# hanruihua/NeuPAN

Hardware: AMD Instinct MI355X
Metric: MPC plans/sec (node), diff robot, 1k pts, T=10, K=10; ctrl L2 vs ref (higher is better)
Workload: dtype f32; 1 GPU; BASELINE.json configs[1]: batch=256 synthetic scenes/GPU, diff robot, 1000 pts, T=10, K=10 (iter_threshold=0), M=10, fp32 DUNE (MFMA) + fp64 QP; scenes_per_gpu=256, points=1000, T=10, K=10, M=10, batches_in_flight=40, chains=8, issue_threads=8

## Files before the change

neupan_amd/csrc/c_api.hip:

```cpp
#include "handle.h"

#include <algorithm>
#include <cmath>
#include <cstdlib>
#include <cstring>

extern "C" hipError_t npa_launch_encode(const DevParams& P, const float* wpack, int batch, int scene0, int t0,
                                        int n_stride, const float* cur_s, const float* points, const float* vel,
                                        const int* n_points, const int* flags, unsigned* gkeys, const float* trig,
                                        int n_cu, int blocks_per_cu, int key_terms, hipStream_t stream,
                                        hipEvent_t ev_start, hipEvent_t ev_stop);
extern "C" hipError_t npa_launch_trig(const float* cur_s, int batch, int T, float* trig, hipStream_t stream);
extern "C" hipError_t npa_launch_select_geo(const DevParams& P, const float* wpack, int batch, int scene0, int t0,
                                            int n_stride, const float* cur_s, const float* points, const float* vel,
                                            const int* n_points, const int* flags, const float* trig, float* mu_sorted,
                                            float* lam_sorted, float* pts_sorted, float* dist_sorted, int* count,
                                            unsigned* stats, int debug, unsigned* audit, unsigned audit_thresh,
                                            unsigned audit_seed, float margin_scale, int rows_bf16, hipStream_t stream,
                                            hipEvent_t ev_start, hipEvent_t ev_stop);
#ifdef NPA_EXPERIMENTS
#define NPA_VERSION_SUFFIX " +experiments"
#else
#define NPA_VERSION_SUFFIX ""
#endif
extern "C" hipError_t npa_launch_select(const DevParams& P, const float* wpack, int batch, int scene0, int t0,
                                        int n_stride, const float* cur_s, const float* points, const float* vel,
                                        const int* n_points, const int* flags, const unsigned* gkeys,
                                        const float* trig, float* mu_sorted, float* lam_sorted, float* pts_sorted,
                                        float* dist_sorted, int* count, int key_terms, float e0, unsigned* stats,
                                        int debug, hipStream_t stream, hipEvent_t ev_start, hipEvent_t ev_stop);
extern "C" hipError_t npa_launch_qp(const DevParams& P, int batch, int scene0, const float* cur_s_in,
                                    const float* cur_u_in, const float* ref_s, const float* ref_us, const float* mu_sorted,
                                    const float* lam_sorted, const float* pts_sorted, const float* dist_sorted,
                                    const int* count, float* cur_s_out, float* cur_u_out, float* cur_d_out,
                                    float* out_s, float* out_u, float* out_d, float* out_min_distance,
                                    int* out_iters, float* out_nrmp_points, int* flags, float* state,
                                    double* qp_info, double* warm, float* trig_out, float* dbg_abc, float* dbg_f, double* dbg_x,
                                    hipStream_t stream, hipEvent_t ev_start, hipEvent_t ev_stop, const float* theta);
extern "C" int npa_select_geo_group_supported(int E);
extern "C" hipError_t npa_launch_select_geo_group(const DevParams& P, const SelGeoGroup& G, int n, int batch, int t0, int n_stride_max,
                                                  int debug, unsigned audit_thresh, float margin_scale, int rows_bf16,
                                                  hipStream_t stream, hipEvent_t ev_start, hipEvent_t ev_stop);
extern "C" int npa_qp_group_supported(int T, int M);
extern "C" hipError_t npa_launch_qp_group(const DevParams& P, const QpGroup& G, int n, int batch, hipStream_t stream,
                                          hipEvent_t ev_start, hipEvent_t ev_stop);
extern "C" hipError_t npa_launch_nominal(int batch, int T, int kin, double dt, double L, const double* state,
                                         const float* vel, const double* ref_speed, const double* path,
                                         const int* curve_off, const int* curve_len, const int* point_index,
                                         const double* interval, float* nom_s, float* nom_u, float* ref_s,
                                         float* ref_us, hipStream_t stream);
extern "C" hipError_t npa_launch_scan(int batch, int beam_stride, const double* ranges, const double* beam_vel,
                                      const int* n_beams, const npa_scan_params* params, int mode, int out_stride,
                                      float* points, float* velocities, int* count, hipStream_t stream);
extern "C" int npa_ingest_offsets(int batch, int T, int n_stride, int with_vel, size_t* out, int n);
extern "C" hipError_t npa_launch_ingest_unpack(int batch, int T, int n_stride, int with_vel, const void* record,
                                               size_t record_bytes, float* nom_s, float* nom_u, float* ref_s, float* ref_us,
                                               float* points, float* velocities, int* n_points, int* status,
                                               hipStream_t stream);

extern "C" const char* npa_last_error(void) { return g_err.c_str(); }
extern "C" const char* npa_version(void) { return "neupan_amd 0.5.2 (gfx950, hipcc " NPA_HIPCC_VERSION ")" NPA_VERSION_SUFFIX; }
static int kstride(const npa_handle* h) { return h->key_terms == 4 ? 0 : h->P.key_stride; }

static int check_theta_batch(const npa_handle* h, int batch, const char* who) {
  if (h->theta && batch != h->theta_batch)
    return fail(NPA_E_ARG, std::string(who) + ": batch " + std::to_string(batch) + " differs from the " + std::to_string(h->theta_batch) +
                               " rows registered with npa_set_adjust_batch");
  return NPA_OK;
}

extern "C" size_t npa_workspace_bytes(const npa_handle* h, int batch) {
  if (!h || batch < 1) return 0;
  return npa_scratch_layout(batch, h->P.T, mdim(h->P), h->P.E, kstride(h)).total * sizeof(float);
}
extern "C" size_t npa_workspace_qp_info_offset(const npa_handle* h, int batch) {
  if (!h || batch < 1) return 0;
  return npa_scratch_layout(batch, h->P.T, mdim(h->P), h->P.E, kstride(h)).qp_info * sizeof(float);
}
extern "C" int npa_workspace_layout(const npa_handle* h, int batch, size_t* out, int n) {
  if (!h || batch < 1 || !out || n < 1) return fail(NPA_E_ARG, "npa_workspace_layout: bad argument");
  const ScratchLayout L = npa_scratch_layout(batch, h->P.T, mdim(h->P), h->P.E, kstride(h));
  const size_t v[8] = {L.cur_s * 4, L.cur_u * 4, L.cur_d * 4, L.mu * 4, L.lam * 4, L.pts * 4, L.dist * 4, L.count * 4};
  for (int i = 0; i < n && i < 8; ++i) out[i] = v[i];
  return NPA_OK;
}
extern "C" size_t npa_state_bytes(const npa_handle* h, int batch) {
  if (!h || batch < 1) return 0;
  return (size_t)batch * npa_state_floats(h->P.T, mdim(h->P), h->P.E) * sizeof(float);
}

static EventPair* next_event(npa_handle* h, std::vector<EventPair>& pool, size_t& used) {
  if (!h->prof) return nullptr;
  if (used == pool.size()) {
    if (pool.size() >= 8192) return nullptr;
    EventPair p;
    if (hipEventCreate(&p.a) != hipSuccess || hipEventCreate(&p.b) != hipSuccess) return nullptr;
    pool.push_back(p);
  }
  return &pool[used++];
}

extern "C" int npa_profile_enable(npa_handle* h, int enable) {
  if (!h) return fail(NPA_E_ARG, "null handle");
  h->prof = enable != 0;
  h->n_dune = h->n_sel = h->n_qp = 0;
  return NPA_OK;
}

extern "C" int npa_profile_read(npa_handle* h, double* dune_ms_avg, double* select_ms_avg, double* nrmp_ms_avg,
                                int64_t* launches) {
  if (!h) return fail(NPA_E_ARG, "null handle");
  auto avg = [](std::vector<EventPair>& pool, size_t used, double* out) -> hipError_t {
    double tot = 0;
    for (size_t i = 0; i < used; ++i) {
      hipError_t e = hipEventSynchronize(pool[i].b);
      if (e != hipSuccess) return e;
      float ms = 0;
      e = hipEventElapsedTime(&ms, pool[i].a, pool[i].b);
      if (e != hipSuccess) return e;
      tot += ms;
    }
    if (out) *out = used ? tot / used : 0.0;
    return hipSuccess;
  };
  HIP_TRY(avg(h->ev_dune, h->n_dune, dune_ms_avg));
  HIP_TRY(avg(h->ev_sel, h->n_sel, select_ms_avg));
  HIP_TRY(avg(h->ev_qp, h->n_qp, nrmp_ms_avg));
  if (launches) *launches = (int64_t)h->n_qp;
  h->n_dune = h->n_sel = h->n_qp = 0;
  return NPA_OK;
}

extern "C" int npa_dune_stage(npa_handle* h, int batch, int n_stride, const float* nom_s, const float* points,
                              const float* velocities, const int32_t* n_points, float* mu_sorted, float* lam_sorted,
                              float* pts_sorted, float* dist_sorted, int32_t* count, void* stream) {
  if (!h || batch < 1 || n_stride < 1 || !nom_s || !points || !mu_sorted || !lam_sorted || !pts_sorted ||
      !dist_sorted || !count)
    return fail(NPA_E_ARG, "npa_dune_stage: bad argument");
  if (h->P.M <= 0) return fail(NPA_E_ARG, "npa_dune_stage: planner has no obstacle stage (nrmp_max_num or dune_max_num is 0)");
  {
    int nmax = n_stride < h->P.dune_max_num ? n_stride : h->P.dune_max_num;
    if (nmax > h->P.key_stride) return fail(NPA_E_UNSUPPORTED, "more than 32768 points per scene after decimation");
  }
  const bool geo = h->key_terms == 4;
  const size_t key_bytes = geo ? 0 : (size_t)batch * (h->P.T + 1) * h->P.key_stride * sizeof(unsigned);
  const size_t trig_bytes = ((size_t)batch * (h->P.T + 1) * 2 * sizeof(float) + 63) / 64 * 64;
  const size_t need = key_bytes + trig_bytes + 64;
  if (need > h->stage_cand_bytes) {
    HIP_TRY(hipStreamSynchronize((hipStream_t)stream));
    if (h->stage_cand) HIP_TRY(hipFree(h->stage_cand));
    h->stage_cand = nullptr; h->stage_cand_bytes = 0;
    HIP_TRY(hipMalloc(&h->stage_cand, need));
    h->stage_cand_bytes = need;
  }
  float* trig = reinterpret_cast<float*>(reinterpret_cast<char*>(h->stage_cand) + key_bytes);
  HIP_TRY(npa_launch_trig(nom_s, batch, h->P.T, trig, (hipStream_t)stream));
  if (!geo)
    HIP_TRY(npa_launch_encode(h->P, h->wpack, batch, 0, 0, n_stride, nom_s, points, velocities, n_points, nullptr,
                              (unsigned*)h->stage_cand, trig, h->n_cu, 5, h->key_terms, (hipStream_t)stream,
                              nullptr, nullptr));
  if (geo && !h->select_v1)
    HIP_TRY(npa_launch_select_geo(h->P, h->wpack, batch, 0, 0, n_stride, nom_s, points, velocities, n_points, nullptr, trig,
                                  mu_sorted, lam_sorted, pts_sorted, dist_sorted, count, h->sel_stats_dev, h->sel_debug,
                                  h->rows_bf16 ? nullptr : h->audit_dev, h->audit_thresh, h->launch_seq++, h->margin_scale,
                                  h->rows_bf16 ? 1 : (h->cal.keys_bf16 ? 2 : 0), (hipStream_t)stream, nullptr, nullptr));
  else
    HIP_TRY(npa_launch_select(h->P, h->wpack, batch, 0, 0, n_stride, nom_s, points, velocities, n_points, nullptr,
                              (const unsigned*)h->stage_cand, trig, mu_sorted, lam_sorted, pts_sorted, dist_sorted, count,
                              h->key_terms, h->key_e0, h->sel_stats_dev, h->sel_debug, (hipStream_t)stream, nullptr, nullptr));
  return NPA_OK;
}

extern "C" int npa_nrmp_stage(npa_handle* h, int batch, const float* nom_s, const float* nom_u, const float* ref_s,
                              const float* ref_us, const float* mu_sorted, const float* lam_sorted,
                              const float* pts_sorted, const int32_t* count, float* out_s, float* out_u,
                              float* out_d, double* qp_info, double* x64, void* stream) {
  if (!h || batch < 1 || !nom_s || !nom_u || !ref_s || !ref_us || !out_s || !out_u)
    return fail(NPA_E_ARG, "npa_nrmp_stage: bad argument");
  if (h->P.M > 0 && (!mu_sorted || !lam_sorted || !pts_sorted || !count || !out_d))
    return fail(NPA_E_ARG, "npa_nrmp_stage: obstacle arrays required when nrmp_max_num > 0");
  if (int rc = check_theta_batch(h, batch, "npa_nrmp_stage")) return rc;
  HIP_TRY(npa_launch_qp(h->P, batch, 0, nom_s, nom_u, ref_s, ref_us, mu_sorted, lam_sorted, pts_sorted, nullptr, count,
                        out_s, out_u, out_d, nullptr, nullptr, nullptr, nullptr, nullptr, nullptr, nullptr, nullptr,
                        qp_info, nullptr, nullptr, nullptr, nullptr, x64, (hipStream_t)stream, nullptr, nullptr, h->theta));
  return NPA_OK;
}

extern "C" int npa_nrmp_params(npa_handle* h, int batch, const float* nom_s, const float* nom_u, const float* mu_sorted,
                               const float* lam_sorted, const float* pts_sorted, const int32_t* count, float* out_abc,
                               float* out_f, void* stream) {
  if (!h || batch < 1 || !nom_s || !nom_u || !out_abc) return fail(NPA_E_ARG, "npa_nrmp_params: bad argument");
  if (h->P.M > 0 && (!mu_sorted || !lam_sorted || !pts_sorted || !count || !out_f))
    return fail(NPA_E_ARG, "npa_nrmp_params: obstacle arrays required when nrmp_max_num > 0");
  HIP_TRY(npa_launch_qp(h->P, batch, 0, nom_s, nom_u, nom_s, nom_u, mu_sorted, lam_sorted, pts_sorted, nullptr, count,
                        nullptr, nullptr, nullptr, nullptr, nullptr, nullptr, nullptr, nullptr, nullptr, nullptr, nullptr,
                        nullptr, nullptr, nullptr, out_abc, h->P.M > 0 ? out_f : nullptr, nullptr, (hipStream_t)stream, nullptr, nullptr,
                        nullptr));
  return NPA_OK;
}

extern "C" hipError_t npa_launch_qp_backward(const DevParams& P, int batch, const float* nom_s, const float* nom_u,
                                             const float* ref_s, const float* ref_us, const float* mu_sorted,
                                             const float* lam_sorted, const float* pts_sorted, const int* count,
                                             float* out_s, float* out_u, float* out_d, const float* grad_s,
                                             const float* grad_u, const float* grad_d, float* grad_theta,
                                             float* grad_nom_s, double* qp_info, hipStream_t stream, const float* theta);
extern "C" int npa_nrmp_backward(npa_handle* h, int batch, const float* nom_s, const float* nom_u, const float* ref_s,
                                 const float* ref_us, const float* mu_sorted, const float* lam_sorted,
                                 const float* pts_sorted, const int32_t* count, float* out_s, float* out_u, float* out_d,
                                 const float* grad_s, const float* grad_u, const float* grad_d, float* grad_theta,
                                 float* grad_nom_s, double* qp_info, void* stream) {
  if (!h || batch < 1 || !nom_s || !nom_u || !ref_s || !ref_us || !out_s || !out_u || !grad_s || !grad_u || !grad_theta)
    return fail(NPA_E_ARG, "npa_nrmp_backward: bad argument");
  if (h->P.M > 0 && (!mu_sorted || !lam_sorted || !pts_sorted || !count || !out_d))
    return fail(NPA_E_ARG, "npa_nrmp_backward: obstacle arrays required when nrmp_max_num > 0");
  if (int rc = check_theta_batch(h, batch, "npa_nrmp_backward")) return rc;
  HIP_TRY(npa_launch_qp_backward(h->P, batch, nom_s, nom_u, ref_s, ref_us, mu_sorted, lam_sorted, pts_sorted, count,
                                 out_s, out_u, out_d, grad_s, grad_u, grad_d, grad_theta, grad_nom_s, qp_info, (hipStream_t)stream, h->theta));
  return NPA_OK;
}

__global__ void stage_kernel(float* __restrict__ cur_s, const float* __restrict__ nom_s, size_t ns,
                             float* __restrict__ cur_u, const float* __restrict__ nom_u, size_t nu,
                             int* __restrict__ flags, size_t nflag, int* __restrict__ count, size_t ncount,
                             int* __restrict__ state, size_t nstate, float* __restrict__ trig, int T) {
  const size_t stride = (size_t)gridDim.x * blockDim.x;
  for (size_t i = (size_t)blockIdx.x * blockDim.x + threadIdx.x;; i += stride) {
    bool any = false;
    if (i < ns) { cur_s[i] = nom_s[i]; any = true; }
    if (i < ncount) {
      const size_t b = i / (size_t)(T + 1), t = i - b * (size_t)(T + 1);
      float c, sn;
      npa_trig(nom_s[b * 3 * (size_t)(T + 1) + 2 * (size_t)(T + 1) + t], c, sn);
      trig[2 * i] = c; trig[2 * i + 1] = sn;
    }
    if (i < nu) { cur_u[i] = nom_u[i]; any = true; }
    if (i < nflag) { flags[i] = 0; any = true; }
    if (i < ncount) { count[i] = 0; any = true; }
    if (i < nstate) { state[i] = 0; any = true; }
    if (!any) break;
  }
}

__global__ void stage_group_kernel(StageGroup G, size_t ns, size_t nu, size_t nflag, size_t ncount, size_t nstate, int T) {
  const StageCall& q = G.c[blockIdx.y];
  float* __restrict__ cur_s = q.cur_s; const float* __restrict__ nom_s = q.nom_s; float* __restrict__ cur_u = q.cur_u;
  const float* __restrict__ nom_u = q.nom_u; int* __restrict__ flags = q.flags; int* __restrict__ count = q.count;
  int* __restrict__ state = q.state; float* __restrict__ trig = q.trig;
  const size_t stride = (size_t)gridDim.x * blockDim.x;
  for (size_t i = (size_t)blockIdx.x * blockDim.x + threadIdx.x;; i += stride) {
    bool any = false;
    if (i < ns) { cur_s[i] = nom_s[i]; any = true; }
    if (i < ncount) {
      const size_t b = i / (size_t)(T + 1), t = i - b * (size_t)(T + 1);
      float c, sn;
      npa_trig(nom_s[b * 3 * (size_t)(T + 1) + 2 * (size_t)(T + 1) + t], c, sn);
      trig[2 * i] = c; trig[2 * i + 1] = sn;
    }
    if (i < nu) { cur_u[i] = nom_u[i]; any = true; }
    if (i < nflag) { flags[i] = 0; any = true; }
    if (i < ncount) { count[i] = 0; any = true; }
    if (i < nstate) { state[i] = 0; any = true; }
    if (!any) break;
  }
}

static void key_policy(npa_handle* h, int batch, int n_stride) {
  if (!h->cal.key_auto) return;
  const DevParams& P = h->P;
  const unsigned now = *(volatile unsigned*)h->sel_stats_host;
  if (h->key_terms == 3) {
    if (--h->hold > 0) return;
    h->key_terms = 1; h->key_err = h->cal.err_mode[0]; h->key_e0 = h->cal.e0_mode[0];
    h->stats_mark = now; h->tiles_window = 0; h->calls_window = 0;
  } else if (h->calls_window >= 8) {
    const unsigned redone = now - h->stats_mark;
    if ((unsigned long long)redone * 12ull > h->tiles_window) {
      h->key_terms = 3; h->key_err = h->cal.err_mode[1]; h->key_e0 = h->cal.e0_mode[1]; h->hold = 256;
      return;
    }
    h->stats_mark = now; h->tiles_window = 0; h->calls_window = 0;
  }
  const int n_use = n_stride < P.dune_max_num ? n_stride : P.dune_max_num;
  h->tiles_window += (unsigned long long)batch * ((n_use + 31) / 32) * ((P.T + 1) + (size_t)(P.K - 1) * P.T);
  ++h->calls_window;
}

static int forward_begin_impl(npa_handle* h, int batch, int n_stride, const float* nom_s, const float* nom_u,
                              const float* ref_s, const float* ref_us, const float* points,
                              const float* velocities, const int32_t* n_points, float* out_s, float* out_u,
                              float* out_d, float* out_min_distance, int32_t* out_iters, float* out_nrmp_points,
                              void* workspace, size_t workspace_bytes, void* state, size_t state_bytes,
                              void* stream_, int flags, bool launch_stage) {
  if (!h || batch < 1 || !nom_s || !nom_u || !ref_s || !ref_us || !out_s || !out_u || !workspace || !state)
    return fail(NPA_E_ARG, "npa_forward_begin: null argument");
  const DevParams& P = h->P;
  if (P.M > 0 && !out_d) return fail(NPA_E_ARG, "npa_forward_begin: out_d required when nrmp_max_num > 0");
  if (workspace_bytes < npa_workspace_bytes(h, batch)) return fail(NPA_E_ARG, "workspace too small");
  if (state_bytes < npa_state_bytes(h, batch)) return fail(NPA_E_ARG, "state buffer too small");
  if (points && n_stride < 1) return fail(NPA_E_ARG, "n_stride < 1");
  if (points && (n_stride < P.dune_max_num ? n_stride : P.dune_max_num) > P.key_stride)
    return fail(NPA_E_UNSUPPORTED, "more than 32768 points per scene after decimation");
  std::lock_guard<std::mutex> lock(h->mu);
  PendingCall* pc = &h->pc;
  if (pc->active) return fail(NPA_E_ARG, "npa_forward_begin: previous forward on this handle not ended");
  if (int rc = check_theta_batch(h, batch, "npa_forward_begin")) return rc;
  hipStream_t stream = (hipStream_t)stream_;
  const int T = P.T;
  const bool reset_state = (flags & NPA_FWD_RESET_STATE) != 0;
  const ScratchLayout L = npa_scratch_layout(batch, T, mdim(P), P.E, kstride(h));
  float* ws = (float*)workspace;
  pc->batch = batch; pc->n_stride = n_stride; pc->ref_s = ref_s; pc->ref_us = ref_us; pc->points = points;
  pc->velocities = velocities; pc->n_points = n_points; pc->out_s = out_s; pc->out_u = out_u; pc->out_d = out_d;
  pc->out_md = out_min_distance; pc->out_iters = out_iters; pc->out_np = out_nrmp_points; pc->ws = ws;
  pc->state = (float*)state; pc->stream = stream;
  pc->dune = P.M > 0 && points != nullptr;
  pc->nom_s = nom_s; pc->nom_u = nom_u; pc->reset_state = reset_state;
  pc->theta = h->theta;
  if (pc->dune) key_policy(h, batch, n_stride);
  if (launch_stage) {
    const size_t ns = (size_t)batch * 3 * (T + 1), nu2 = (size_t)batch * 2 * T;
    const size_t nflag = (size_t)batch * 4, ncount = (size_t)batch * (T + 1);
    const size_t nstate = reset_state ? npa_state_bytes(h, batch) / 4 : 0;
    const size_t work = std::max(std::max(ns, nu2), std::max(std::max(nflag, ncount), nstate));
    const int threads = 256;
    const int blocks = (int)std::min<size_t>((work + threads - 1) / threads, 512);
    hipLaunchKernelGGL(stage_kernel, dim3(blocks), dim3(threads), 0, stream, ws + L.cur_s, nom_s, ns, ws + L.cur_u, nom_u, nu2,
                       (int*)(ws + L.flags), nflag, (int*)(ws + L.count), ncount, (int*)state, nstate, ws + L.trig, T);
    HIP_TRY(hipGetLastError());
  }
  pc->active = true;
  return NPA_OK;
}

extern "C" int npa_forward_begin(npa_handle* h, int batch, int n_stride, const float* nom_s, const float* nom_u,
                                 const float* ref_s, const float* ref_us, const float* points,
                                 const float* velocities, const int32_t* n_points, float* out_s, float* out_u,
                                 float* out_d, float* out_min_distance, int32_t* out_iters, float* out_nrmp_points,
                                 void* workspace, size_t workspace_bytes, void* state, size_t state_bytes,
                                 void* stream_, int flags) {
  return forward_begin_impl(h, batch, n_stride, nom_s, nom_u, ref_s, ref_us, points, velocities, n_points, out_s, out_u, out_d,
                            out_min_distance, out_iters, out_nrmp_points, workspace, workspace_bytes, state, state_bytes, stream_,
                            flags, true);
}

extern "C" int npa_group_mergeable(int n, const npa_forward_call* calls) {
  if (n < 2 || n > NPA_GROUP_MAX || !calls) return 0;
  static const bool off = getenv("NPA_GROUP_MERGE") != nullptr && atoi(getenv("NPA_GROUP_MERGE")) == 0;
  if (off) return 0;
  const npa_handle* h0 = calls[0].h;
  if (!h0) return 0;
  const DevParams& P = h0->P;
  const bool dune0 = P.M > 0 && calls[0].points != nullptr;
  if (dune0 && !(h0->key_terms == 4 && !h0->select_v1 && !h0->rows_bf16 && npa_select_geo_group_supported(P.E))) return 0;
  if (!npa_qp_group_supported(P.T, P.M) || h0->qp_generic || h0->cal.key_auto) return 0;
  if (calls[0].iter_num < 1 || calls[0].iter_num > P.K) return 0;
  for (int c = 0; c < n; ++c) {
    const npa_handle* h = calls[c].h;
    if (!h || calls[c].stream != calls[0].stream || calls[c].batch != calls[0].batch || calls[c].iter_num != calls[0].iter_num ||
        h->device != h0->device || memcmp(&h->P, &P, sizeof(DevParams)) != 0 || h->key_terms != h0->key_terms ||
        h->select_v1 != h0->select_v1 || h->rows_bf16 != h0->rows_bf16 || h->cal.keys_bf16 != h0->cal.keys_bf16 ||
        h->sel_debug != h0->sel_debug || h->audit_thresh != h0->audit_thresh || h->margin_scale != h0->margin_scale ||
        h->qp_generic != h0->qp_generic || h->qp_warm != h0->qp_warm || h->cal.key_auto ||
        (P.M > 0 && calls[c].points != nullptr) != dune0 || (calls[c].out_d == nullptr) != (calls[0].out_d == nullptr))
      return 0;
  }
  return 1;
}

extern "C" int npa_forward_group_merged(int n, const npa_forward_call* calls) { return npa_group_mergeable(n, calls); }

struct GroupLock {
  std::mutex* m[NPA_GROUP_MAX];
  int n = 0;
  GroupLock(int cnt, const npa_forward_call* calls) {
    for (int c = 0; c < cnt && n < NPA_GROUP_MAX; ++c)
      if (calls[c].h) m[n++] = &calls[c].h->mu;
    std::sort(m, m + n);
    n = (int)(std::unique(m, m + n) - m);
    for (int i = 0; i < n; ++i) m[i]->lock();
  }
  ~GroupLock() { for (int i = n - 1; i >= 0; --i) m[i]->unlock(); }
  GroupLock(const GroupLock&) = delete;
  GroupLock& operator=(const GroupLock&) = delete;
};

extern "C" int npa_group_begin_merged(int n, const npa_forward_call* calls, int flags, int* begun) {
  *begun = 0;
  for (int c = 0; c < n; ++c) {
    const npa_forward_call& a = calls[c];
    const int rc = forward_begin_impl(a.h, a.batch, a.n_stride, a.nom_s, a.nom_u, a.ref_s, a.ref_us, a.points, a.velocities,
                                      a.n_points, a.out_s, a.out_u, a.out_d, a.out_min_distance, a.out_iters, a.out_nrmp_points,
                                      a.workspace, a.workspace_bytes, a.state, a.state_bytes, a.stream, flags, false);
    if (rc != NPA_OK) return rc;
    *begun = c + 1;
  }
  GroupLock group_lock(n, calls);
  npa_handle* h0 = calls[0].h;
  const DevParams& P = h0->P;
  const int T = P.T, batch = calls[0].batch;
  const ScratchLayout L = npa_scratch_layout(batch, T, mdim(P), P.E, kstride(h0));
  StageGroup G;
  memset(&G, 0, sizeof(G));
  for (int c = 0; c < n; ++c) {
    const PendingCall& pc = calls[c].h->pc;
    G.c[c] = StageCall{pc.ws + L.cur_s, pc.nom_s, pc.ws + L.cur_u, pc.nom_u, (int*)(pc.ws + L.flags), (int*)(pc.ws + L.count),
                       (int*)pc.state, pc.ws + L.trig};
  }
  const size_t ns = (size_t)batch * 3 * (T + 1), nu2 = (size_t)batch * 2 * T;
  const size_t nflag = (size_t)batch * 4, ncount = (size_t)batch * (T + 1);
  const size_t nstate = h0->pc.reset_state ? npa_state_bytes(h0, batch) / 4 : 0;
  const size_t work = std::max(std::max(ns, nu2), std::max(std::max(nflag, ncount), nstate));
  const int threads = 256;
  const int blocks = (int)std::min<size_t>((work + threads - 1) / threads, 512);
  hipLaunchKernelGGL(stage_group_kernel, dim3(blocks, n), dim3(threads), 0, h0->pc.stream, G, ns, nu2, nflag, ncount, nstate, T);
  HIP_TRY(hipGetLastError());
  return NPA_OK;
}

static std::atomic<unsigned long long> g_merged_launches{0};
extern "C" unsigned long long npa_dbg_group_merged_launches(void) { return g_merged_launches.load(); }

extern "C" int npa_group_iter_merged(int n, const npa_forward_call* calls, int k) {
  GroupLock group_lock(n, calls);
  npa_handle* h0 = calls[0].h;
  const DevParams& P = h0->P;
  if (k < 0 || k >= P.K) return fail(NPA_E_ARG, "npa_forward_batch_group: iteration index out of range");
  const int T = P.T, batch = calls[0].batch;
  const ScratchLayout L = npa_scratch_layout(batch, T, mdim(P), P.E, kstride(h0));
  hipStream_t stream = h0->pc.stream;
  for (int c = 0; c < n; ++c)
    if (!calls[c].h->pc.active) return fail(NPA_E_ARG, "npa_forward_batch_group: a call of the group is not in progress");
  if (h0->pc.dune) {
    SelGeoGroup G;
    memset(&G, 0, sizeof(G));
    int n_stride_max = 1;
    for (int c = 0; c < n; ++c) {
      npa_handle* h = calls[c].h;
      const PendingCall& pc = h->pc;
      float* ws = pc.ws;
      G.c[c] = SelGeoCall{h->wpack, ws + L.cur_s, pc.points, pc.velocities, pc.n_points, (const int*)(ws + L.flags),
                          ws + L.mu, ws + L.lam, ws + L.pts, ws + L.dist, (int*)(ws + L.count), h->sel_stats_dev, ws + L.trig,
                          h->rows_bf16 ? nullptr : h->audit_dev, pc.n_stride, h->launch_seq++};
      if (pc.n_stride > n_stride_max) n_stride_max = pc.n_stride;
    }
    EventPair* evs = next_event(h0, h0->ev_sel, h0->n_sel);
    HIP_TRY(npa_launch_select_geo_group(P, G, n, batch, k == 0 ? 0 : 1, n_stride_max, 0, h0->audit_thresh,
                                        h0->margin_scale, h0->cal.keys_bf16 ? 2 : 0, stream, evs ? evs->a : nullptr,
                                        evs ? evs->b : nullptr));
  }
  QpGroup Q;
  memset(&Q, 0, sizeof(Q));
  for (int c = 0; c < n; ++c) {
    npa_handle* h = calls[c].h;
    const PendingCall& pc = h->pc;
    float* ws = pc.ws;
    float *cur_s = ws + L.cur_s, *cur_u = ws + L.cur_u;
    Q.c[c] = QpCall{cur_s, cur_u, pc.ref_s, pc.ref_us, ws + L.mu, ws + L.lam, ws + L.pts, ws + L.dist, (const int*)(ws + L.count),
                    cur_s, cur_u, ws + L.cur_d, pc.out_s, pc.out_u, pc.out_d, pc.out_md, pc.out_iters, pc.out_np,
                    (int*)(ws + L.flags), pc.state, (double*)(ws + L.qp_info), h->qp_warm ? (double*)(ws + L.warm) : nullptr,
                    pc.dune ? ws + L.trig : nullptr, pc.theta};
  }
  EventPair* ev = next_event(h0, h0->ev_qp, h0->n_qp);
  HIP_TRY(npa_launch_qp_group(P, Q, n, batch, stream, ev ? ev->a : nullptr, ev ? ev->b : nullptr));
  g_merged_launches.fetch_add(1);
  return NPA_OK;
}

extern "C" int npa_forward_iter(npa_handle* h, int k) {
  if (!h) return fail(NPA_E_ARG, "npa_forward_iter: null handle");
  std::lock_guard<std::mutex> lock(h->mu);
  PendingCall* pc = &h->pc;
  if (!pc->active) return fail(NPA_E_ARG, "npa_forward_iter: no forward in progress on this handle");
  const DevParams& P = h->P;
  if (k < 0 || k >= P.K) return fail(NPA_E_ARG, "npa_forward_iter: iteration index out of range");
  const int T = P.T, batch = pc->batch;
  const bool geo = h->key_terms == 4;
  const ScratchLayout L = npa_scratch_layout(batch, T, mdim(P), P.E, kstride(h));
  float* ws = pc->ws;
  float *cur_s = ws + L.cur_s, *cur_u = ws + L.cur_u, *cur_d = ws + L.cur_d;
  float *mu = ws + L.mu, *lam = ws + L.lam, *pts = ws + L.pts, *dist = ws + L.dist;
  int* count = (int*)(ws + L.count);
  int* flags = (int*)(ws + L.flags);
  double* qp_info = (double*)(ws + L.qp_info);
  unsigned* gkeys = (unsigned*)(ws + L.keys);
  hipStream_t stream = pc->stream;
  if (pc->dune) {
    const int t0 = k == 0 ? 0 : 1;
    if (!geo) {
      EventPair* ev = next_event(h, h->ev_dune, h->n_dune);
      HIP_TRY(npa_launch_encode(P, h->wpack, batch, 0, t0, pc->n_stride, cur_s, pc->points, pc->velocities,
                                pc->n_points, flags, gkeys, ws + L.trig, h->n_cu, 5, h->key_terms, stream,
                                ev ? ev->a : nullptr, ev ? ev->b : nullptr));
    }
    EventPair* evs = next_event(h, h->ev_sel, h->n_sel);
    if (geo && !h->select_v1)
      HIP_TRY(npa_launch_select_geo(P, h->wpack, batch, 0, t0, pc->n_stride, cur_s, pc->points, pc->velocities, pc->n_points,
                                    flags, ws + L.trig, mu, lam, pts, dist, count, h->sel_stats_dev, 0,
                                    h->rows_bf16 ? nullptr : h->audit_dev, h->audit_thresh, h->launch_seq++, h->margin_scale,
                                    h->rows_bf16 ? 1 : (h->cal.keys_bf16 ? 2 : 0), stream, evs ? evs->a : nullptr, evs ? evs->b : nullptr));
    else
      HIP_TRY(npa_launch_select(P, h->wpack, batch, 0, t0, pc->n_stride, cur_s, pc->points, pc->velocities,
                                pc->n_points, flags, gkeys, ws + L.trig, mu, lam, pts, dist, count, h->key_terms, h->key_e0,
                                h->sel_stats_dev, 0, stream, evs ? evs->a : nullptr, evs ? evs->b : nullptr));
  }
  EventPair* ev = next_event(h, h->ev_qp, h->n_qp);
  HIP_TRY(npa_launch_qp(P, batch, 0, cur_s, cur_u, pc->ref_s, pc->ref_us, mu, lam, pts, dist, count, cur_s, cur_u,
                        cur_d, pc->out_s, pc->out_u, pc->out_d, pc->out_md, pc->out_iters, pc->out_np, flags,
                        pc->state, qp_info, h->qp_warm ? (double*)(ws + L.warm) : nullptr, pc->dune ? ws + L.trig : nullptr,
                        nullptr, nullptr, nullptr, stream,
                        ev ? ev->a : nullptr, ev ? ev->b : nullptr, pc->theta));
  if (h->cal.key_auto && pc->dune && k == P.K - 1)
    HIP_TRY(hipMemcpyAsync(h->sel_stats_host, h->sel_stats_dev, sizeof(unsigned), hipMemcpyDeviceToHost, stream));
  return NPA_OK;
}

extern "C" int npa_forward_end(npa_handle* h) {
  if (!h) return fail(NPA_E_ARG, "npa_forward_end: null handle");
  std::lock_guard<std::mutex> lock(h->mu);
  PendingCall* pc = &h->pc;
  if (!pc->active) return fail(NPA_E_ARG, "npa_forward_end: no forward in progress on this handle");
  pc->active = false;
  return NPA_OK;
}

extern "C" int npa_dbg_select_stats(npa_handle* h, unsigned out[4]) {
  if (!h || !out || !h->sel_stats_dev) return NPA_E_ARG;
  HIP_TRY(hipDeviceSynchronize());
  HIP_TRY(hipMemcpy(out, h->sel_stats_dev, 4 * sizeof(unsigned), hipMemcpyDeviceToHost));
  return NPA_OK;
}

extern "C" int npa_forward_batch_flags(npa_handle* h, int batch, int n_stride, const float* nom_s, const float* nom_u,
                                       const float* ref_s, const float* ref_us, const float* points,
                                       const float* velocities, const int32_t* n_points, float* out_s, float* out_u,
                                       float* out_d, float* out_min_distance, int32_t* out_iters, float* out_nrmp_points,
                                       void* workspace, size_t workspace_bytes, void* state, size_t state_bytes,
                                       void* stream_, int flags) {
  if (!h) return fail(NPA_E_ARG, "npa_forward_batch: null handle");
  int rc = npa_forward_begin(h, batch, n_stride, nom_s, nom_u, ref_s, ref_us, points, velocities, n_points, out_s,
                             out_u, out_d, out_min_distance, out_iters, out_nrmp_points, workspace, workspace_bytes,
                             state, state_bytes, stream_, flags);
  if (rc != NPA_OK) return rc;
  for (int k = 0; k < h->P.K; ++k) {
    rc = npa_forward_iter(h, k);
    if (rc != NPA_OK) { npa_forward_end(h); return rc; }
  }
  return npa_forward_end(h);
}

extern "C" int npa_forward_batch(npa_handle* h, int batch, int n_stride, const float* nom_s, const float* nom_u,
                                 const float* ref_s, const float* ref_us, const float* points,
                                 const float* velocities, const int32_t* n_points, float* out_s, float* out_u,
                                 float* out_d, float* out_min_distance, int32_t* out_iters, float* out_nrmp_points,
                                 void* workspace, size_t workspace_bytes, void* state, size_t state_bytes,
                                 void* stream_) {
  return npa_forward_batch_flags(h, batch, n_stride, nom_s, nom_u, ref_s, ref_us, points, velocities, n_points, out_s, out_u,
                                 out_d, out_min_distance, out_iters, out_nrmp_points, workspace, workspace_bytes, state,
                                 state_bytes, stream_, 0);
}

extern "C" int npa_nominal_ref_states(int batch, int receding, int kinematics, double step_time, double wheelbase,
                                      const double* state, const float* cur_vel, const double* ref_speed,
                                      const double* path, const int32_t* curve_off, const int32_t* curve_len,
                                      const int32_t* point_index, const double* interval, float* nom_s, float* nom_u,
                                      float* ref_s, float* ref_us, void* stream) {
  if (batch < 1 || !state || !ref_speed || !path || !curve_off || !curve_len || !point_index || !interval || !nom_s ||
      !nom_u || !ref_s || !ref_us)
    return fail(NPA_E_ARG, "npa_nominal_ref_states: bad argument");
  if (receding < 1 || receding > NPA_MAX_T) return fail(NPA_E_UNSUPPORTED, "receding outside [1,NPA_MAX_T]");
  if (kinematics < 0 || kinematics > 2) return fail(NPA_E_ARG, "unknown kinematics");
  if (kinematics == NPA_KIN_ACKER && !(wheelbase > 0)) return fail(NPA_E_ARG, "acker needs wheelbase > 0");
  HIP_TRY(npa_launch_nominal(batch, receding, kinematics, step_time, wheelbase, state, cur_vel, ref_speed, path,
                             curve_off, curve_len, point_index, interval, nom_s, nom_u, ref_s, ref_us,
                             (hipStream_t)stream));
  return NPA_OK;
}

extern "C" hipError_t npa_launch_progress(int batch, const double* state, const double* path, const int* curve_off,
                                          const int* curve_len, int* point_index, double close_threshold, int ind_range,
                                          double arrive_threshold, int arrive_index_threshold, float* min_dis,
                                          int* arrived, hipStream_t stream);
extern "C" int npa_path_progress(int batch, const double* state, const double* path, const int32_t* curve_off,
                                 const int32_t* curve_len, int32_t* point_index, double close_threshold, int ind_range,
                                 double arrive_threshold, int arrive_index_threshold, float* min_dis, int32_t* arrived,
                                 void* stream) {
  if (batch < 1 || !state || !path || !curve_off || !curve_len || !point_index || !arrived || ind_range < 1)
    return fail(NPA_E_ARG, "npa_path_progress: bad argument");
  HIP_TRY(npa_launch_progress(batch, state, path, curve_off, curve_len, point_index, close_threshold, ind_range,
                              arrive_threshold, arrive_index_threshold, min_dis, arrived, (hipStream_t)stream));
  return NPA_OK;
}

extern "C" int npa_scan_to_points(int batch, int beam_stride, const double* ranges, const double* beam_vel,
                                  const int32_t* n_beams, const npa_scan_params* params, int mode, int out_stride,
                                  float* points, float* velocities, int32_t* count, void* stream) {
  if (batch < 1 || beam_stride < 1 || out_stride < 1 || !ranges || !params || !points || !count)
    return fail(NPA_E_ARG, "npa_scan_to_points: bad argument");
  if (mode != 0 && mode != 1) return fail(NPA_E_ARG, "npa_scan_to_points: mode must be 0 or 1");
  HIP_TRY(npa_launch_scan(batch, beam_stride, ranges, beam_vel, n_beams, params, mode, out_stride, points, velocities,
                          count, (hipStream_t)stream));
  return NPA_OK;
}

extern "C" hipError_t npa_launch_cycle_switch(int batch, int loop, const double* state, const int* curve_arrived,
                                              const int* curve_off, const int* curve_len, const int* robot_first,
                                              int* curve_index, int* cur_off, int* cur_len, int* point_index, int* arrived,
                                              npa_scan_params* params_a, npa_scan_params* params_b, hipStream_t stream);
extern "C" hipError_t npa_launch_cycle_act(int batch, int T, int kin, int first_cycle, int cycle, const float* opt_u,
                                           const float* min_distance, float threshold, const int* arrived, const int* collided,
                                           const float* override_row, const int* n_points, float* cur_vel, float* action,
                                           uint8_t* stop, int* frozen, float* log_actions, uint8_t* log_stop,
                                           float* log_controls, int* log_n_points, hipStream_t stream);
extern "C" hipError_t npa_launch_cycle_commit(int batch, int cycle, const double* state, const double* clearance, int* collided,
                                              double* log_states, double* log_clearance, hipStream_t stream);

extern "C" int npa_cycle_progress(int batch, const double* state, const double* path, const int32_t* curve_off,
                                  const int32_t* curve_len, const int32_t* robot_first, int loop, double close_threshold,
                                  int ind_range, double arrive_threshold, int arrive_index_threshold, int32_t* curve_index,
                                  int32_t* cur_off, int32_t* cur_len, int32_t* point_index, int32_t* curve_arrived,
                                  int32_t* arrived, npa_scan_params* params_a, npa_scan_params* params_b, void* stream) {
  if (batch < 1 || !state || !path || !curve_off || !curve_len || !robot_first || !curve_index || !cur_off || !cur_len ||
      !point_index || !curve_arrived || !arrived || !params_a || !params_b || ind_range < 1)
    return fail(NPA_E_ARG, "npa_cycle_progress: bad argument");
  HIP_TRY(npa_launch_progress(batch, state, path, cur_off, cur_len, point_index, close_threshold, ind_range, arrive_threshold,
                              arrive_index_threshold, nullptr, curve_arrived, (hipStream_t)stream));
  HIP_TRY(npa_launch_cycle_switch(batch, loop, state, curve_arrived, curve_off, curve_len, robot_first, curve_index, cur_off,
                                  cur_len, point_index, arrived, params_a, params_b, (hipStream_t)stream));
  return NPA_OK;
}

extern "C" int npa_cycle_act(int batch, int receding, int kinematics, int first_cycle, int cycle, const float* opt_u,
                             const float* min_distance, float collision_threshold, const int32_t* arrived,
                             const int32_t* collided, const float* override_row, const int32_t* n_points, float* cur_vel,
                             float* action, uint8_t* stop, int32_t* frozen, float* log_actions, uint8_t* log_stop,
                             float* log_controls, int32_t* log_n_points, void* stream) {
  if (batch < 1 || cycle < 0 || !opt_u || !min_distance || !arrived || !collided || !cur_vel || !action || !stop || !frozen)
    return fail(NPA_E_ARG, "npa_cycle_act: bad argument");
  if (receding < 1 || receding > NPA_MAX_T) return fail(NPA_E_ARG, "npa_cycle_act: receding outside [1,NPA_MAX_T]");
  if (kinematics < 0 || kinematics > 2) return fail(NPA_E_ARG, "npa_cycle_act: unknown kinematics");
  HIP_TRY(npa_launch_cycle_act(batch, receding, kinematics, first_cycle, cycle, opt_u, min_distance, collision_threshold, arrived,
                               collided, override_row, n_points, cur_vel, action, stop, frozen, log_actions, log_stop,
                               log_controls, log_n_points, (hipStream_t)stream));
  return NPA_OK;
}

extern "C" int npa_cycle_commit(int batch, int cycle, const double* state, const double* clearance, int32_t* collided,
                                double* log_states, double* log_clearance, void* stream) {
  if (batch < 1 || cycle < 0 || !state || !clearance || !collided) return fail(NPA_E_ARG, "npa_cycle_commit: bad argument");
  HIP_TRY(npa_launch_cycle_commit(batch, cycle, state, clearance, collided, log_states, log_clearance, (hipStream_t)stream));
  return NPA_OK;
}

extern "C" hipError_t npa_launch_cycle_retask(int batch, int T, int cycle, int style, double min_radius, const double* state,
                                              int* arrived, const int* collided, double* path, const int* curve_off,
                                              int* curve_len, const int* robot_first, const int* row_capacity,
                                              const double* goals, int g_stride, const int* n_goals, int* goal_index,
                                              const double* interval, int* curve_index, int* cur_off, int* cur_len,
                                              int* point_index, float* cur_vel, int* status, int* log_goal, hipStream_t stream);

extern "C" int npa_cycle_retask(int batch, int receding, int cycle, int style, double min_radius, const double* state,
                                int32_t* arrived, const int32_t* collided, double* path, const int32_t* curve_off,
                                int32_t* curve_len, const int32_t* robot_first, const int32_t* row_capacity, const double* goals,
                                int g_stride, const int32_t* n_goals, int32_t* goal_index, const double* interval,
                                int32_t* curve_index, int32_t* cur_off, int32_t* cur_len, int32_t* point_index, float* cur_vel,
                                int32_t* retask_status, int32_t* log_goal, void* stream) {
  const char* what = nullptr;
  if (batch < 1 || cycle < 0 || !state || !arrived || !collided || !path || !curve_off || !curve_len || !robot_first ||
      !row_capacity || !goals || !n_goals || !goal_index || !interval || !curve_index || !cur_off || !cur_len || !point_index ||
      !cur_vel || !retask_status)
    what = "npa_cycle_retask: bad argument";
  else if (receding < 1 || receding > NPA_MAX_T) what = "npa_cycle_retask: receding outside [1,NPA_MAX_T]";
  else if (style != NPA_CURVE_LINE && style != NPA_CURVE_DUBINS) what = "npa_cycle_retask: style outside 0..1";
  else if (style == NPA_CURVE_DUBINS && (!(min_radius > 0.0) || !std::isfinite(min_radius)))
    what = "npa_cycle_retask: dubins needs min_radius > 0";
  else if (g_stride < 1) what = "npa_cycle_retask: g_stride < 1";
  if (what) return fail(NPA_E_ARG, what);
  HIP_TRY(npa_launch_cycle_retask(batch, receding, cycle, style, min_radius, state, arrived, collided, path, curve_off, curve_len,
                                  robot_first, row_capacity, goals, g_stride, n_goals, goal_index, interval, curve_index, cur_off,
                                  cur_len, point_index, cur_vel, retask_status, log_goal, (hipStream_t)stream));
  return NPA_OK;
}

static int ingest_args_ok(int batch, int receding, int n_stride) {
  return batch >= 1 && receding >= 1 && receding <= NPA_MAX_T && n_stride >= 1;
}

extern "C" int npa_ingest_layout(int batch, int receding, int n_stride, int with_velocities, size_t* out, int n) {
  if (!ingest_args_ok(batch, receding, n_stride) || !out || n < 1 || n > 8)
    return fail(NPA_E_ARG, "npa_ingest_layout: bad argument");
  if (npa_ingest_offsets(batch, receding, n_stride, with_velocities != 0, out, n) != 0)
    return fail(NPA_E_ARG, "npa_ingest_layout: the cloud section would not fit int32 word offsets");
  return NPA_OK;
}

extern "C" int npa_ingest_unpack(int batch, int receding, int n_stride, int with_velocities, const void* record,
                                 size_t record_bytes, float* nom_s, float* nom_u, float* ref_s, float* ref_us, float* points,
                                 float* velocities, int32_t* n_points, int32_t* status, void* stream) {
  if (!ingest_args_ok(batch, receding, n_stride) || !record || !nom_s || !nom_u || !ref_s || !ref_us || !points ||
      !n_points || !status || (with_velocities && !velocities))
    return fail(NPA_E_ARG, "npa_ingest_unpack: bad argument");
  const void* ptrs[] = {record, nom_s, nom_u, ref_s, ref_us, points, velocities, n_points, status};
  for (const void* p : ptrs)
    if (((uintptr_t)p & 3) != 0) return fail(NPA_E_ARG, "npa_ingest_unpack: pointers must be 4-byte aligned");
  size_t off[8];
  if (npa_ingest_offsets(batch, receding, n_stride, with_velocities != 0, off, 8) != 0)
    return fail(NPA_E_ARG, "npa_ingest_unpack: the cloud section would not fit int32 word offsets");
  if (record_bytes < off[6] || record_bytes > off[7] || (record_bytes & 3) != 0)
    return fail(NPA_E_ARG, "npa_ingest_unpack: record_bytes must be a multiple of 4 between the cloud section's offset (" +
                               std::to_string(off[6]) + ") and the layout's total (" + std::to_string(off[7]) + "), got " +
                               std::to_string(record_bytes));
  HIP_TRY(npa_launch_ingest_unpack(batch, receding, n_stride, with_velocities != 0, record, record_bytes, nom_s, nom_u, ref_s,
                                   ref_us, points, velocities, n_points, status, (hipStream_t)stream));
  return NPA_OK;
}

extern "C" hipError_t npa_launch_clearance(const DevParams& P, int batch, int n_stride, const float* traj, const float* points,
                                           const float* velocities, const int* n_points, float threshold, float* clearance,
                                           int* nearest, float* min_clearance, int* first_violation, hipStream_t stream);
extern "C" int npa_plan_clearance(npa_handle* h, int batch, int n_stride, const float* traj_s, const float* points,
                                  const float* velocities, const int32_t* n_points, float threshold, float* clearance,
                                  int32_t* nearest, float* min_clearance, int32_t* first_violation, void* stream) {
  if (!h || batch <= 0 || n_stride <= 0 || !traj_s || !points || !clearance || !nearest)
    return fail(NPA_E_ARG, "npa_plan_clearance: bad argument");
  const void* ptrs[] = {traj_s, points, velocities, n_points, clearance, nearest, min_clearance, first_violation};
  for (const void* p : ptrs)
    if (((uintptr_t)p & 3) != 0) return fail(NPA_E_ARG, "npa_plan_clearance: pointers must be 4-byte aligned");
  if (!h->geo_valid)
    return fail(NPA_E_UNSUPPORTED, "npa_plan_clearance: the robot polygon's rows are not consecutive counter-clockwise edges "
                                   "(no vertices could be derived from G, h)");
  HIP_TRY(npa_launch_clearance(h->P, batch, n_stride, traj_s, points, velocities, n_points, threshold, clearance, nearest,
                               min_clearance, first_violation, (hipStream_t)stream));
  return NPA_OK;
}

extern "C" hipError_t npa_launch_labels(int E, const double* G, const double* h, long long n, const double* points,
                                        float* mu, float* dist, hipStream_t stream);
extern "C" int npa_dune_labels(int edge_num, const double* G, const double* h, int64_t n, const double* points,
                               float* mu, float* dist, void* stream) {
  if (!G || !h || n < 0 || (n > 0 && (!points || !mu || !dist))) return fail(NPA_E_ARG, "npa_dune_labels: bad argument");
  if (edge_num < 3 || edge_num > NPA_MAX_E) return fail(NPA_E_UNSUPPORTED, "edge_num outside [3,NPA_MAX_E]");
  HIP_TRY(npa_launch_labels(edge_num, G, h, (long long)n, points, mu, dist, (hipStream_t)stream));
  return NPA_OK;
}
```

neupan_amd/csrc/create.hip:

```cpp
#include "handle.h"
#include "pack_image.h"

#include <algorithm>
#include <cmath>
#include <cstdio>
#include <cstdlib>
#include <cstring>
#include <map>

extern "C" hipError_t npa_launch_key_calib(const DevParams& P, const float* wpack, int key_terms, int nside, float half,
                                           unsigned* out, hipStream_t stream);
extern "C" hipError_t npa_launch_geo_table(const DevParams& P, float* wpack, float* nodes, int n_cu, hipStream_t stream);
extern "C" hipError_t npa_launch_ktab_calib(const DevParams& P, const float* wpack, int nside, float half, float inner, float cx, float cy,
                                            unsigned* out, int n_cu, hipStream_t stream);
extern "C" hipError_t npa_launch_geo_calib(const DevParams& P, const float* wpack, int nside, float half, float inner,
                                           float shift, unsigned* out, int n_cu, hipStream_t stream);
extern "C" hipError_t npa_launch_k16_calib(const DevParams& P, const float* wpack, int nside, float half, float inner, unsigned* out,
                                           int n_cu, hipStream_t stream);
extern "C" size_t npa_qp_shmem_bytes(int T, int M);

static std::mutex g_pack_mu;
static std::map<std::string, std::weak_ptr<SharedPack>> g_packs;
static long long g_pack_calibrations = 0, g_pack_hits = 0;

struct CalibKnobDef { const char* name; void (*parse)(const char* v, CalibKnobs& k); };
static Precision parse_precision(const char* v) {
  return !strcmp(v, "bf16") ? Precision::bf16 : (!strcmp(v, "fp32") ? Precision::fp32 : Precision::invalid);
}
static const CalibKnobDef kCalibKnobs[] = {
    {"NPA_DUNE_FP32KEYS", [](const char*, CalibKnobs& k) { k.forced_mode = 0; }},
    {"NPA_KEY_TERMS", [](const char* v, CalibKnobs& k) { const int t = atoi(v); if (k.forced_mode != 0 && (t == 1 || t == 3 || t == 4)) k.forced_mode = t; }},
    {"NPA_KEY_SAFETY", [](const char* v, CalibKnobs& k) { const double s = atof(v); if (s >= 1.0 && s <= 1e3) k.key_safety = s; }},
    {"NPA_GEO_GRID", [](const char* v, CalibKnobs& k) { const int n = atoi(v); if (n >= 64 && n <= 8192) k.geo_grid = n / 8 * 8; }},
    {"NPA_GEO_NOCHECK", [](const char*, CalibKnobs& k) { k.geo_nocheck = true; }},
    {"NPA_GEO_TABLE", [](const char* v, CalibKnobs& k) { k.geo_table = atoi(v) != 0; }},
    {"NPA_KTAB_SAFETY", [](const char* v, CalibKnobs& k) { const double s = atof(v); if (s >= 1.0 && s <= 100.0) k.ktab_safety = s; }},
    {"NPA_KEYS_PRECISION", [](const char* v, CalibKnobs& k) { k.keys_precision = parse_precision(v); }},
    {"NPA_K16_SAFETY", [](const char* v, CalibKnobs& k) { const double s = atof(v); if (s >= 1.0 && s <= 100.0) k.k16_safety = s; }},
    {"NPA_ROWS_PRECISION", [](const char* v, CalibKnobs& k) { k.rows_precision = parse_precision(v); }},
};

struct Knobs {
  CalibKnobs calib;
  std::string calib_key;
  bool sel_debug = false, qp_cold = false, qp_generic = false, skip_selftest = false, pack_cache = true;
  double audit_rate = 1.0 / 64.0;
  float margin_scale = 1.f;
};

static Knobs read_knobs() {
  Knobs k;
  for (const CalibKnobDef& d : kCalibKnobs) {
    const char* v = getenv(d.name);
    k.calib_key.push_back('|');
    if (v) { k.calib_key.append(v); d.parse(v, k.calib); } else k.calib_key.push_back('\x01');
  }
  k.sel_debug = getenv("NPA_SEL_DEBUG") != nullptr;
  k.qp_cold = getenv("NPA_QP_COLD") != nullptr;
  k.qp_generic = getenv("NPA_QP_GENERIC") != nullptr;
  k.skip_selftest = getenv("NPA_SKIP_SELFTEST") != nullptr;
  if (const char* env = getenv("NPA_PACK_CACHE")) k.pack_cache = atoi(env) != 0;
  if (const char* env = getenv("NPA_AUDIT_RATE")) { double v = atof(env); if (v >= 0.0 && v <= 1.0) k.audit_rate = v; }
  if (const char* env = getenv("NPA_GEO_MARGIN_SCALE")) { double v = atof(env); if (v > 0.0 && v <= 100.0) k.margin_scale = (float)v; }
  return k;
}

#ifdef NPA_EXPERIMENTS
static void read_experiment_knobs(npa_handle* h) { h->select_v1 = getenv("NPA_SELECT_V1") != nullptr; }
#endif


template <class T>
struct DevScratch {
  T* p = nullptr;
  hipError_t alloc_zeroed(size_t n) {
    hipError_t e = hipMalloc(&p, n * sizeof(T));
    return e == hipSuccess ? hipMemset(p, 0, n * sizeof(T)) : e;
  }
  ~DevScratch() { if (p) (void)hipFree(p); }
};

static void set_calibrated(DevParams& P, const Calibration& c) { P.geo_rcal = c.geo_rcal; P.geo_far = c.geo_far; P.geo_tab = c.geo_tab; }

static void use_key_mode(npa_handle* h) { h->key_terms = h->cal.key_terms; h->key_err = h->cal.key_err; h->key_e0 = h->cal.key_e0; }
static void apply_calibration(npa_handle* h, const Calibration& c) {
  h->cal = c;
  set_calibrated(h->P, c);
  use_key_mode(h);
}

static constexpr int kBandsPadded = (NPA_GEO_BANDS + 3) & ~3;
static const float kCalibHalves[3] = {8.f, 32.f, 128.f};

static void band_margins(const float* raw, const bool* seen, double safety, float floor, float* margin, float* near) {
  for (int bnd = 0; bnd < NPA_GEO_BANDS; ++bnd) {
    float m = -1.f;
    for (int q = std::max(bnd - 1, 0); q <= std::min(bnd + 1, NPA_GEO_BANDS - 1); ++q)
      if (seen[q]) m = std::max(m, raw[q]);
    near[bnd] = m;
    margin[bnd] = (m < 0.f || !(m < 1e30f)) ? INFINITY : std::max((float)(safety * m), floor);
  }
}

static void residual_margins(const unsigned* bits, double safety, float floor, float (&margin)[kBandsPadded], float& worst_err,
                             float& worst_margin) {
  float raw[NPA_GEO_BANDS], near[NPA_GEO_BANDS];
  bool seen[NPA_GEO_BANDS];
  for (int bnd = 0; bnd < NPA_GEO_BANDS; ++bnd) { memcpy(&raw[bnd], &bits[bnd], 4); seen[bnd] = bits[bnd] != 0u; }
  for (int bnd = 0; bnd < kBandsPadded; ++bnd) margin[bnd] = INFINITY;
  band_margins(raw, seen, safety, floor, margin, near);
  worst_err = 0.f; worst_margin = 0.f;
  for (int bnd = 0; bnd <= npa_geo_band(8.0f) && bnd < NPA_GEO_BANDS; ++bnd)
    if (near[bnd] >= 0.f) { worst_err = std::max(worst_err, near[bnd]); worst_margin = std::max(worst_margin, margin[bnd]); }
}

static hipError_t calibrate_network_keys(const DevParams& P, const float* wpack, const CalibKnobs& k, int forced, Calibration& c) {
  const int modes[2] = {1, 3};
  const float floor_e0[2] = {1e-4f, 2e-5f}, cap_e0[2] = {5e-2f, 1e-3f};
  bool ok[2] = {false, false};
  const double sf = k.key_safety > 0 ? k.key_safety : 5.0;
  DevScratch<unsigned> dmax;
  hipError_t e = hipMalloc(&dmax.p, sizeof(unsigned));
  for (int m = 0; m < 2 && e == hipSuccess; ++m) {
    if (forced > 0 && forced != modes[m]) continue;
    unsigned bits = 0;
    e = hipMemset(dmax.p, 0, sizeof(unsigned));
    if (e == hipSuccess) e = npa_launch_key_calib(P, wpack, modes[m], 1024, 25.0f, dmax.p, nullptr);
    if (e == hipSuccess) e = hipMemcpy(&bits, dmax.p, sizeof(unsigned), hipMemcpyDeviceToHost);
    if (e != hipSuccess) break;
    float err;
    memcpy(&err, &bits, sizeof(err));
    c.err_mode[m] = err;
    c.e0_mode[m] = std::max((float)(sf * err), floor_e0[m]);
    ok[m] = c.e0_mode[m] <= cap_e0[m] || forced == modes[m];
  }
  if (e != hipSuccess) return e;
  const int pick = ok[0] ? 0 : (ok[1] ? 1 : -1);
  c.key_terms = 0; c.key_err = 0.f; c.key_e0 = 0.f;
  if (pick >= 0) { c.key_terms = modes[pick]; c.key_err = c.err_mode[pick]; c.key_e0 = c.e0_mode[pick]; }
  c.key_auto = forced < 0 && ok[0] && ok[1];
  return hipSuccess;
}

static hipError_t calibrate_geo_keys(const DevParams& P0, float* wpack, int n_cu, const CalibKnobs& k, Calibration& c) {
  DevParams P = P0;
  set_calibrated(P, c);
  const float* halves = kCalibHalves;
  const int nside = k.geo_grid;
  const int forced = k.forced_mode;
  unsigned bits[2 * NPA_GEO_BANDS], bits2[2 * NPA_GEO_BANDS];
  {
    DevScratch<unsigned> tab, tab2;
    hipError_t e = tab.alloc_zeroed(2 * NPA_GEO_BANDS);
    for (int gI = 0; gI < 3 && e == hipSuccess; ++gI)
      e = npa_launch_geo_calib(P, wpack, nside, halves[gI], gI == 0 ? 0.f : 0.97f * halves[gI - 1], 0.f, tab.p, n_cu, nullptr);
    if (e == hipSuccess) e = tab2.alloc_zeroed(2 * NPA_GEO_BANDS);
    for (int gI = 0; gI < 3 && e == hipSuccess; ++gI)
      e = npa_launch_geo_calib(P, wpack, nside, halves[gI], gI == 0 ? 0.f : 0.97f * halves[gI - 1], 0.5f, tab2.p, n_cu, nullptr);
    if (e == hipSuccess) e = hipMemcpy(bits, tab.p, sizeof(bits), hipMemcpyDeviceToHost);
    if (e == hipSuccess) e = hipMemcpy(bits2, tab2.p, sizeof(bits2), hipMemcpyDeviceToHost);
    if (e != hipSuccess) return e;
  }
  const double sf = k.key_safety > 0 ? k.key_safety : 1.5;
  float raw[NPA_GEO_BANDS], mg[NPA_GEO_BANDS], near[NPA_GEO_BANDS];
  bool seen[NPA_GEO_BANDS];
  float refine = 0.f, slope = 0.f;
  {
    float pred[NPA_GEO_BANDS], cen[NPA_GEO_BANDS];
    for (int bnd = 0; bnd < NPA_GEO_BANDS; ++bnd) {
      float f0, f1, c0;
      memcpy(&f0, &bits[bnd], 4); memcpy(&f1, &bits[NPA_GEO_BANDS + bnd], 4); memcpy(&c0, &bits2[bnd], 4);
      pred[bnd] = f0 + f1; cen[bnd] = c0;
    }
    for (int bnd = 0; bnd < NPA_GEO_BANDS; ++bnd) {
      if (bits2[bnd] == 0u) continue;
      float pr = 0.f;
      for (int q = std::max(bnd - 1, 0); q <= std::min(bnd + 1, NPA_GEO_BANDS - 1); ++q) pr = std::max(pr, pred[q]);
      pr = std::max(pr, 1e-3f);
      if (!(cen[bnd] < 1e30f)) { refine = INFINITY; continue; }
      refine = std::max(refine, cen[bnd] / pr);
    }
    const float h0 = 2.0f * halves[0] / (float)(nside - 1);
    for (int bnd = 0; bnd <= npa_geo_band(6.0f); ++bnd) {
      float f1;
      memcpy(&f1, &bits[NPA_GEO_BANDS + bnd], 4);
      if (f1 < 1e30f) slope = std::max(slope, f1 / h0);
    }
  }
  c.geo_refine = refine; c.geo_slope = slope;
  for (int bnd = 0; bnd < NPA_GEO_BANDS; ++bnd) {
    float f0, f1, c0, c1;
    memcpy(&f0, &bits[bnd], 4); memcpy(&f1, &bits[NPA_GEO_BANDS + bnd], 4);
    memcpy(&c0, &bits2[bnd], 4); memcpy(&c1, &bits2[NPA_GEO_BANDS + bnd], 4);
    seen[bnd] = bits[bnd] != 0u || bits[NPA_GEO_BANDS + bnd] != 0u || bits2[bnd] != 0u;
    raw[bnd] = std::max(f0, c0) + std::max(f1, c1);
  }
  band_margins(raw, seen, sf, 1e-4f, mg, near);
  float worst_err = 0.f, worst_margin = 0.f;
  for (int bnd = npa_geo_band(0.25f); bnd <= npa_geo_band(8.0f) && bnd < NPA_GEO_BANDS; ++bnd) {
    worst_margin = std::max(worst_margin, mg[bnd]);
    float f0;
    memcpy(&f0, &bits[bnd], 4);
    worst_err = std::max(worst_err, f0);
  }
  c.geo_err = worst_err; c.geo_margin = worst_margin;
  const bool resolved = refine <= 1.25f || k.geo_nocheck;
  if (!((worst_margin <= 0.15f && resolved) || forced == 4)) return hipSuccess;
  hipError_t e = hipMemcpy(wpack + WP_GEO, mg, sizeof(mg), hipMemcpyHostToDevice);
  c.geo_rcal = halves[2];
  double rmax = 0;
  for (int v = 0; v < P.E; ++v) rmax = std::max(rmax, std::sqrt((double)P.pvx[v] * P.pvx[v] + (double)P.pvy[v] * P.pvy[v]));
  c.geo_far = (float)std::max(1.0, (double)halves[2] - rmax);
  c.key_terms = 4; c.key_err = worst_err; c.key_e0 = worst_margin;
  return e;
}

static hipError_t calibrate_key_table(const DevParams& P0, float* wpack, int n_cu, const float* tabh, const CalibKnobs& k, Calibration& c) {
  DevParams P = P0;
  set_calibrated(P, c);
  unsigned kb[NPA_GEO_BANDS];
  {
    DevScratch<float> nodes;
    DevScratch<unsigned> tabk;
    hipError_t e = hipMalloc(&nodes.p, (size_t)NPA_TAB_LEVELS * (NPA_TAB_N + 1) * (NPA_TAB_N + 1) * sizeof(float));
    if (e == hipSuccess) e = npa_launch_geo_table(P, wpack, nodes.p, n_cu, nullptr);
    if (e == hipSuccess) e = tabk.alloc_zeroed(NPA_GEO_BANDS);
    const float th0 = tabh[2];
    const float khalves[NPA_TAB_LEVELS] = {th0, 4.f * th0, 16.f * th0, 64.f * th0};
    for (int gI = 0; gI < NPA_TAB_LEVELS && e == hipSuccess; ++gI)
      e = npa_launch_ktab_calib(P, wpack, k.geo_grid, khalves[gI], gI == 0 ? 0.f : 0.97f * khalves[gI - 1], tabh[0], tabh[1], tabk.p,
                                n_cu, nullptr);
    if (e == hipSuccess) e = hipMemcpy(kb, tabk.p, sizeof(kb), hipMemcpyDeviceToHost);
    if (e != hipSuccess) return e;
  }
  float mk[kBandsPadded];
  residual_margins(kb, k.ktab_safety, 1e-4f, mk, c.ktab_err, c.ktab_margin);
  const hipError_t e = hipMemcpy(wpack + WP_KTAB, mk, sizeof(mk), hipMemcpyHostToDevice);
  if (e == hipSuccess) c.geo_tab = 1;
  return e;
}

static hipError_t calibrate_bf16_keys(const DevParams& P0, float* wpack, int n_cu, const CalibKnobs& k, Calibration& c) {
  DevParams P = P0;
  set_calibrated(P, c);
  const float* halves = kCalibHalves;
  unsigned bits[NPA_GEO_BANDS];
  {
    DevScratch<unsigned> tab;
    hipError_t e = tab.alloc_zeroed(NPA_GEO_BANDS);
    for (int gI = 0; gI < 3 && e == hipSuccess; ++gI)
      e = npa_launch_k16_calib(P, wpack, 1024, halves[gI], gI == 0 ? 0.f : 0.97f * halves[gI - 1], tab.p, n_cu, nullptr);
    if (e == hipSuccess) e = hipMemcpy(bits, tab.p, sizeof(bits), hipMemcpyDeviceToHost);
    if (e != hipSuccess) return e;
  }
  float mg[kBandsPadded];
  residual_margins(bits, k.k16_safety, 1e-5f, mg, c.k16_err, c.k16_margin);
  const hipError_t e = hipMemcpy(wpack + WP_K16, mg, sizeof(mg), hipMemcpyHostToDevice);
  c.keys_bf16 = true;
  return e;
}

static hipError_t calibrate_key_mode(const DevParams& P, float* wpack, int n_cu, bool geo_valid, const float* tabh, const CalibKnobs& k,
                                     Calibration& c) {
  const int forced = k.forced_mode;
  hipError_t e = hipSuccess;
  if (geo_valid && (forced < 0 || forced == 4)) {
    e = calibrate_geo_keys(P, wpack, n_cu, k, c);
    if (e == hipSuccess && c.key_terms == 4 && (P.E == 4 || P.E == 8) && k.geo_table) e = calibrate_key_table(P, wpack, n_cu, tabh, k, c);
  }
  if (e == hipSuccess && c.key_terms != 4 && forced != 0 && forced != 4) e = calibrate_network_keys(P, wpack, k, forced, c);
  return e;
}

static int check_precision_tiers(npa_handle* h, const CalibKnobs& k, int key_terms) {
  const bool geo48 = key_terms == 4 && !h->select_v1 && (h->P.E == 4 || h->P.E == 8);
  if (k.rows_precision == Precision::invalid) return fail(NPA_E_ARG, "NPA_ROWS_PRECISION must be fp32 or bf16");
  if (k.rows_precision == Precision::bf16) {
    if (!geo48) return fail(NPA_E_UNSUPPORTED, "NPA_ROWS_PRECISION=bf16 needs geometric keys (select_geo_kernel) and a polygon of 4 or 8 edges");
    h->rows_bf16 = true;
  }
  if (k.keys_precision == Precision::invalid) return fail(NPA_E_ARG, "NPA_KEYS_PRECISION must be fp32 or bf16");
  if (k.keys_precision == Precision::bf16 && !(geo48 && !h->rows_bf16))
    return fail(NPA_E_UNSUPPORTED, "NPA_KEYS_PRECISION=bf16 needs geometric keys, exact rows and a polygon of 4 or 8 edges");
  return NPA_OK;
}

static int hip_status(hipError_t e) { return e == hipSuccess ? NPA_OK : fail(NPA_E_HIP, std::string("npa_create: ") + hipGetErrorString(e)); }

static int acquire_pack(npa_handle* h, const std::vector<float>& image, bool need_w, const Knobs& knobs) {
  const DevParams& P = h->P;
  const CalibKnobs& ck = knobs.calib;
  std::string key(reinterpret_cast<const char*>(image.data()), image.size() * sizeof(float));
  key.append(reinterpret_cast<const char*>(&P.E), sizeof(P.E));
  key.append(reinterpret_cast<const char*>(P.G), sizeof(P.G));
  key.append(reinterpret_cast<const char*>(P.h), sizeof(P.h));
  key.append(reinterpret_cast<const char*>(&h->device), sizeof(h->device));
  key.push_back(need_w ? 'w' : '-');
  key.append(knobs.calib_key);
  std::lock_guard<std::mutex> lock(g_pack_mu);
  if (knobs.pack_cache) {
    auto it = g_packs.find(key);
    if (it != g_packs.end()) {
      h->pack = it->second.lock();
      if (!h->pack) g_packs.erase(it);
    }
  }
  const bool hit = (bool)h->pack;
  if (!hit) {
    h->pack = std::make_shared<SharedPack>();
    h->pack->device = h->device;
    hipError_t e = hipMalloc(&h->pack->wpack, ((size_t)WP_TAB + WP_TAB_FLOATS) * sizeof(float));
    if (e == hipSuccess) e = hipMemcpy(h->pack->wpack, image.data(), WP_TOTAL * sizeof(float), hipMemcpyHostToDevice);
    if (e != hipSuccess) return hip_status(e);
  }
  SharedPack& S = *h->pack;
  h->wpack = S.wpack;
  if (need_w) {
    if (hit) ++g_pack_hits;
    else if (int rc = hip_status(calibrate_key_mode(P, S.wpack, h->n_cu, h->geo_valid, &image[WP_TABH], ck, S.cal))) return rc;
    if (int rc = check_precision_tiers(h, ck, S.cal.key_terms)) return rc;
    if (!hit && ck.keys_precision == Precision::bf16)
      if (int rc = hip_status(calibrate_bf16_keys(P, S.wpack, h->n_cu, ck, S.cal))) return rc;
    apply_calibration(h, S.cal);
  }
  if (!hit) {
    if (need_w) ++g_pack_calibrations;
    if (knobs.pack_cache) g_packs[key] = h->pack;
  }
  return NPA_OK;
}

static int params_from_config(const npa_config* cfg, const npa_dune_weights* w, DevParams& P, bool& need_w, bool& geo_valid) {
  if (cfg->receding < 1 || cfg->receding > NPA_MAX_T) return fail(NPA_E_UNSUPPORTED, "receding outside [1,NPA_MAX_T]");
  if (cfg->nrmp_max_num < 0 || cfg->nrmp_max_num > NPA_MAX_M) return fail(NPA_E_UNSUPPORTED, "nrmp_max_num outside [0,NPA_MAX_M]");
  if (cfg->edge_num < 3 || cfg->edge_num > NPA_MAX_E) return fail(NPA_E_UNSUPPORTED, "edge_num outside [3,NPA_MAX_E]");
  if (cfg->kinematics < 0 || cfg->kinematics > 2) return fail(NPA_E_ARG, "unknown kinematics");
  if (cfg->iter_num < 1) return fail(NPA_E_ARG, "iter_num < 1");
  if (npa_qp_shmem_bytes(cfg->receding, cfg->nrmp_max_num) > 160 * 1024) return fail(NPA_E_UNSUPPORTED, "T*M too large for LDS");
  need_w = cfg->nrmp_max_num > 0 && cfg->dune_max_num > 0;
  if (need_w && !w) return fail(NPA_E_ARG, "DUNE weights required unless nrmp_max_num == 0 or dune_max_num == 0");
  P.T = cfg->receding; P.M = (cfg->dune_max_num > 0) ? cfg->nrmp_max_num : 0; P.E = cfg->edge_num;
  P.kin = cfg->kinematics; P.K = cfg->iter_num; P.dune_max_num = cfg->dune_max_num;
  {
    long long n = cfg->dune_max_num > 0 ? cfg->dune_max_num : 1;
    if (n > NPA_MAX_POINTS) n = NPA_MAX_POINTS;
    P.key_stride = (int)((n + 31) / 32 * 32);
  }
  P.iter_threshold = cfg->iter_threshold;
  P.dt = cfg->step_time; P.dt32 = (float)cfg->step_time; P.L = cfg->wheelbase;
  for (int k = 0; k < 2; ++k) { P.speed_bound[k] = cfg->speed_bound[k]; P.acce_bound[k] = cfg->acce_bound[k]; }
  P.ro_obs = cfg->ro_obs; P.bk = cfg->bk;
  for (int k = 0; k < 3; ++k) P.q_s[k] = cfg->q_s[k];
  P.p_u = cfg->p_u; P.eta = cfg->eta; P.d_max = cfg->d_max; P.d_min = cfg->d_min;
  for (int e = 0; e < NPA_MAX_E; ++e) { P.G[e][0] = cfg->G[e][0]; P.G[e][1] = cfg->G[e][1]; P.h[e] = cfg->h[e]; }
  geo_valid = npa_polygon_geometry(P);
  return NPA_OK;
}

extern "C" int npa_dbg_pack_image(const npa_config* cfg, const npa_dune_weights* w, float* image, size_t image_floats, void* params,
                                  size_t params_bytes, size_t* params_size, int* geo_valid, size_t* offsets, int n_offsets) {
  if (!cfg) return fail(NPA_E_ARG, "npa_dbg_pack_image: null configuration");
  const size_t off[13] = {WP_W1, WP_WL, WP_VEC, WP_W6, WP_B6, WP_BF, WP_WLS, WP_WB16, WP_TABH, WP_W116, WP_WL16, WP_VEC16, WP_TOTAL};
  for (int i = 0; offsets && i < n_offsets && i < 13; ++i) offsets[i] = off[i];
  if (params_size) *params_size = sizeof(DevParams);
  DevParams P;
  memset(&P, 0, sizeof(P));
  bool need_w = false, valid = false;
  if (int rc = params_from_config(cfg, w, P, need_w, valid)) return rc;
  if (geo_valid) *geo_valid = valid ? 1 : 0;
  if (params) memcpy(params, &P, std::min(params_bytes, sizeof(P)));
  if (image) {
    std::vector<float> img;
    npa_build_pack_image(P, valid, need_w ? w : nullptr, img);
    memcpy(image, img.data(), std::min(image_floats, img.size()) * sizeof(float));
  }
  return NPA_OK;
}

static hipError_t audit_block_reset(npa_handle* h) {
  if (!h->audit_dev) return hipSuccess;
  unsigned blk[8] = {0, 0, 0, 0, 0, 0, 0, 0};
  void* mirror = nullptr;
  if (h->audit_host && hipHostGetDevicePointer(&mirror, h->audit_host, 0) != hipSuccess) mirror = nullptr;
  memcpy(&blk[6], &mirror, sizeof(mirror));
  if (h->audit_host) *(volatile unsigned*)h->audit_host = 0;
  return hipMemcpy(h->audit_dev, blk, sizeof(blk), hipMemcpyHostToDevice);
}

static hipError_t alloc_handle_buffers(npa_handle* h) {
  hipError_t e = hipMalloc(&h->sel_stats_dev, 4 * sizeof(unsigned));
  if (e == hipSuccess) e = hipMemset(h->sel_stats_dev, 0, 4 * sizeof(unsigned));
  if (e == hipSuccess) e = hipHostMalloc(&h->sel_stats_host, sizeof(unsigned), hipHostMallocDefault);
  if (e == hipSuccess) *h->sel_stats_host = 0;
  if (e == hipSuccess) e = hipMalloc(&h->audit_dev, 8 * sizeof(unsigned));
  if (e == hipSuccess) e = hipHostMalloc(&h->audit_host, sizeof(unsigned), hipHostMallocMapped);
  if (e == hipSuccess) e = audit_block_reset(h);
  return e;
}

static int npa_self_test(npa_handle* h);

static int create_handle(npa_handle* h, bool need_w, const npa_dune_weights* w) {
  std::vector<float> image;
  npa_build_pack_image(h->P, h->geo_valid, need_w ? w : nullptr, image);
  const Knobs knobs = read_knobs();
  h->knobs = knobs.calib;
  h->sel_debug = knobs.sel_debug; h->qp_warm = !knobs.qp_cold; h->qp_generic = knobs.qp_generic;
#ifdef NPA_EXPERIMENTS
  read_experiment_knobs(h);
#endif
  if (int rc = hip_status(hipGetDevice(&h->device))) return rc;
  hipDeviceProp_t prop;
  if (hipGetDeviceProperties(&prop, h->device) == hipSuccess && prop.multiProcessorCount > 0) h->n_cu = prop.multiProcessorCount;
  if (int rc = acquire_pack(h, image, need_w, knobs)) return rc;
  if (need_w) {
    if (int rc = hip_status(alloc_handle_buffers(h))) return rc;
    h->audit_thresh = knobs.audit_rate >= 1.0 ? 0xFFFFFFFFu : (unsigned)(knobs.audit_rate * 4294967296.0);
    h->margin_scale = knobs.margin_scale;
  }
  return knobs.skip_selftest ? NPA_OK : npa_self_test(h);
}

extern "C" int npa_create(const npa_config* cfg, const npa_dune_weights* w, npa_handle** out) {
  if (!cfg || !out) return fail(NPA_E_ARG, "npa_create: null argument");
  DevParams P;
  memset(&P, 0, sizeof(P));
  bool need_w = false, geo_valid = false;
  if (int rc = params_from_config(cfg, w, P, need_w, geo_valid)) return rc;
  npa_handle* h = new npa_handle();
  memcpy(&h->P, &P, sizeof(P));
  h->geo_valid = geo_valid;
  const int rc = create_handle(h, need_w, w);
  if (rc != NPA_OK) {
    const std::string msg = g_err;
    npa_destroy(h);
    return fail(rc, msg);
  }
  *out = h;
  return NPA_OK;
}

extern "C" int npa_destroy(npa_handle* h) {
  if (!h) return NPA_OK;
  {
    int cur = -1;
    if (hipGetDevice(&cur) == hipSuccess) {
      if (cur != h->device) (void)hipSetDevice(h->device);
      (void)hipDeviceSynchronize();
      if (cur != h->device) (void)hipSetDevice(cur);
    }
    (void)hipGetLastError();
  }
  for (auto& p : h->ev_dune) { hipEventDestroy(p.a); hipEventDestroy(p.b); }
  for (auto& p : h->ev_sel) { hipEventDestroy(p.a); hipEventDestroy(p.b); }
  for (auto& p : h->ev_qp) { hipEventDestroy(p.a); hipEventDestroy(p.b); }
  h->wpack = nullptr;
  {
    std::lock_guard<std::mutex> lk(g_pack_mu);
    h->pack.reset();
  }
  if (h->sel_stats_dev) hipFree(h->sel_stats_dev);
  if (h->sel_stats_host) hipHostFree(h->sel_stats_host);
  if (h->audit_dev) hipFree(h->audit_dev);
  if (h->audit_host) hipHostFree(h->audit_host);
  if (h->stage_cand) hipFree(h->stage_cand);
  delete h;
  return NPA_OK;
}

extern "C" int npa_key_mode(const npa_handle* h, int* key_terms, float* measured_error, float* margin_e0) {
  if (!h) return fail(NPA_E_ARG, "npa_key_mode: null handle");
  if (key_terms) *key_terms = h->key_terms;
  if (measured_error) *measured_error = h->key_err;
  if (margin_e0) *margin_e0 = h->key_e0;
  return NPA_OK;
}

extern "C" int npa_pack_cache_stats(int64_t* calibrations, int64_t* shared_creates, int64_t* alive) {
  std::lock_guard<std::mutex> lk(g_pack_mu);
  if (calibrations) *calibrations = g_pack_calibrations;
  if (shared_creates) *shared_creates = g_pack_hits;
  if (alive) {
    int64_t n = 0;
    for (auto& kv : g_packs) n += kv.second.expired() ? 0 : 1;
    *alive = n;
  }
  return NPA_OK;
}

extern "C" int npa_geo_report(const npa_handle* h, float* out, int n) {
  if (!h || !out || n < 1) return fail(NPA_E_ARG, "npa_geo_report: bad argument");
  const Calibration& c = h->cal;
  const float v[10] = {h->geo_valid ? 1.f : 0.f, c.geo_err, c.geo_margin, c.geo_refine, c.geo_slope, h->P.geo_far,
                       c.keys_bf16 ? c.k16_err : 0.f, c.keys_bf16 ? c.k16_margin : 0.f,
                       h->P.geo_tab ? c.ktab_err : 0.f, h->P.geo_tab ? c.ktab_margin : 0.f};
  for (int i = 0; i < n && i < 10; ++i) out[i] = v[i];
  return NPA_OK;
}

extern "C" int npa_audit_read(npa_handle* h, uint64_t* tiles, uint64_t* points, uint64_t* violations, float* worst_excess, int reset) {
  if (!h) return fail(NPA_E_ARG, "npa_audit_read: null handle");
  unsigned v[4] = {0, 0, 0, 0};
  if (h->audit_dev) {
    int cur = -1;
    HIP_TRY(hipGetDevice(&cur));
    if (cur != h->device) HIP_TRY(hipSetDevice(h->device));
    hipError_t e = hipDeviceSynchronize();
    if (e == hipSuccess) e = hipMemcpy(v, h->audit_dev, sizeof(v), hipMemcpyDeviceToHost);
    if (e == hipSuccess && reset) {
      e = hipMemset(h->audit_dev, 0, sizeof(v));
      if (h->audit_host) *(volatile unsigned*)h->audit_host = 0;
    }
    if (cur != h->device) (void)hipSetDevice(cur);
    HIP_TRY(e);
  }
  if (tiles) *tiles = v[0];
  if (points) *points = v[1];
  if (violations) *violations = v[2];
  if (worst_excess) memcpy(worst_excess, &v[3], 4);
  return NPA_OK;
}

extern "C" int npa_audit_peek(const npa_handle* h, uint64_t* violations) {
  if (!h || !violations) return fail(NPA_E_ARG, "npa_audit_peek: null argument");
  *violations = h->audit_host ? (uint64_t)*(volatile unsigned*)h->audit_host : 0;
  return NPA_OK;
}

extern "C" int npa_selftest_flags(const npa_handle* h, int* flags) {
  if (!h || !flags) return fail(NPA_E_ARG, "npa_selftest_flags: null argument");
  *flags = h->selftest_flags;
  return NPA_OK;
}

static hipError_t switch_to_network_keys(npa_handle* h) {
  const hipError_t e = calibrate_network_keys(h->P, h->wpack, h->knobs, -1, h->cal);
  if (e == hipSuccess) use_key_mode(h);
  return e;
}

extern "C" int npa_use_network_keys(npa_handle* h) {
  if (!h) return fail(NPA_E_ARG, "npa_use_network_keys: null handle");
  std::lock_guard<std::mutex> lock(h->mu);
  if (h->pc.active) return fail(NPA_E_ARG, "npa_use_network_keys: a forward call is in progress on this handle");
  if (h->key_terms != 4) return NPA_OK;
  int cur = -1;
  HIP_TRY(hipGetDevice(&cur));
  if (cur != h->device) HIP_TRY(hipSetDevice(h->device));
  hipError_t e = hipDeviceSynchronize();
  if (e == hipSuccess) e = switch_to_network_keys(h);
  if (e == hipSuccess) e = audit_block_reset(h);
  if (e == hipSuccess) { h->rows_bf16 = false; h->cal.keys_bf16 = false; }
  if (cur != h->device) (void)hipSetDevice(cur);
  HIP_TRY(e);
  h->stats_mark = 0; h->tiles_window = 0; h->calls_window = 0; h->hold = 0;
  return NPA_OK;
}

extern "C" int npa_set_adjust(npa_handle* h, const float q_s[3], float p_u, float eta, float d_max, float d_min) {
  if (!h || !q_s) return fail(NPA_E_ARG, "npa_set_adjust: null argument");
  for (int k = 0; k < 3; ++k) h->P.q_s[k] = q_s[k];
  h->P.p_u = p_u; h->P.eta = eta; h->P.d_max = d_max; h->P.d_min = d_min;
  return NPA_OK;
}

extern "C" int npa_set_adjust_batch(npa_handle* h, const float* theta, int batch) {
  if (!h) return fail(NPA_E_ARG, "npa_set_adjust_batch: null handle");
  if (theta && batch < 1) return fail(NPA_E_ARG, "npa_set_adjust_batch: batch < 1");
  std::lock_guard<std::mutex> lock(h->mu);
  h->theta = theta;
  h->theta_batch = theta ? batch : 0;
  return NPA_OK;
}

static int npa_self_test(npa_handle* h) {
  const DevParams& P = h->P;
  const int B = 2, T = P.T, M = mdim(P), E = P.E, N = 96;
  const bool obs = P.M > 0;
  const int kmax = P.K < 3 ? P.K : 3;
  std::vector<float> nom_s((size_t)B * 3 * (T + 1)), nom_u((size_t)B * 2 * T), ref_s(nom_s.size()), ref_us((size_t)B * T),
      pts((size_t)B * 2 * N);
  float rbody = 2.5f;
  if (h->geo_valid) {
    rbody = 0.f;
    for (int e = 0; e < P.E; ++e) rbody = std::max(rbody, std::sqrt(P.pvx[e] * P.pvx[e] + P.pvy[e] * P.pvy[e]));
  }
  unsigned lcg = 12345u;
  auto rnd = [&]() { lcg = lcg * 1664525u + 1013904223u; return (float)((lcg >> 8) & 0xFFFF) / 65535.0f; };
  for (int b = 0; b < B; ++b) {
    const float th = 0.05f * (float)(b + 1), v = 1.0f + 0.5f * (float)b;
    for (int t = 0; t <= T; ++t) {
      const float d = v * (float)P.dt * (float)t;
      nom_s[(size_t)b * 3 * (T + 1) + t] = d * std::cos(th);
      nom_s[(size_t)b * 3 * (T + 1) + (T + 1) + t] = d * std::sin(th);
      nom_s[(size_t)b * 3 * (T + 1) + 2 * (T + 1) + t] = th;
      ref_s[(size_t)b * 3 * (T + 1) + t] = 1.1f * d;
      ref_s[(size_t)b * 3 * (T + 1) + (T + 1) + t] = 0.f;
      ref_s[(size_t)b * 3 * (T + 1) + 2 * (T + 1) + t] = 0.f;
    }
    for (int t = 0; t < T; ++t) {
      nom_u[(size_t)b * 2 * T + t] = v; nom_u[(size_t)b * 2 * T + T + t] = 0.f;
      ref_us[(size_t)b * T + t] = v;
    }
    const float ring0 = std::max(4.0f, rbody + 1.5f), cx = std::max(5.5f, (rbody + 3.0f) * 0.9f), cy = std::max(2.5f, (rbody + 3.0f) * 0.43f);
    for (int n = 0; n < N; ++n) {
      const float ang = 6.2831853f * rnd(), r = ring0 + 5.0f * rnd();
      pts[(size_t)b * 2 * N + n] = (n < 80) ? r * std::cos(ang) : cx + 0.6f * rnd();
      pts[(size_t)b * 2 * N + N + n] = (n < 80) ? r * std::sin(ang) : cy + 0.6f * rnd();
    }
  }
  const size_t wsb = npa_workspace_bytes(h, B), stb = npa_state_bytes(h, B);
  const size_t n_in = nom_s.size() * 2 + nom_u.size() + ref_us.size() + pts.size();
  const size_t n_out = (size_t)B * 3 * (T + 1) + (size_t)B * 2 * T + (size_t)B * T + B + B + (size_t)B * 2 * M;
  const size_t n_stage = (size_t)B * (T + 1) * M * (E + 5) + (size_t)B * (T + 1);
  char* dev = nullptr;
  const size_t bytes = (n_in + 3 * n_out + 2 * n_stage) * 4 + wsb + stb + 1024;
  HIP_TRY(hipMalloc(&dev, bytes));
  struct Free { char* p; ~Free() { if (p) hipFree(p); } } guard{dev};
  HIP_TRY(hipMemset(dev, 0, bytes));
  float* d_nom_s = (float*)dev;
  float* d_ref_s = d_nom_s + nom_s.size();
  float* d_nom_u = d_ref_s + ref_s.size();
  float* d_ref_us = d_nom_u + nom_u.size();
  float* d_pts = d_ref_us + ref_us.size();
  float* d_out[3];
  d_out[0] = d_pts + pts.size(); d_out[1] = d_out[0] + n_out; d_out[2] = d_out[1] + n_out;
  float* d_stage[2];
  d_stage[0] = d_out[2] + n_out; d_stage[1] = d_stage[0] + n_stage;
  char* d_ws = (char*)(((uintptr_t)(d_stage[1] + n_stage) + 255) & ~(uintptr_t)255);
  char* d_state = (char*)(((uintptr_t)(d_ws + wsb) + 255) & ~(uintptr_t)255);
  HIP_TRY(hipMemcpy(d_nom_s, nom_s.data(), nom_s.size() * 4, hipMemcpyHostToDevice));
  HIP_TRY(hipMemcpy(d_ref_s, ref_s.data(), ref_s.size() * 4, hipMemcpyHostToDevice));
  HIP_TRY(hipMemcpy(d_nom_u, nom_u.data(), nom_u.size() * 4, hipMemcpyHostToDevice));
  HIP_TRY(hipMemcpy(d_ref_us, ref_us.data(), ref_us.size() * 4, hipMemcpyHostToDevice));
  HIP_TRY(hipMemcpy(d_pts, pts.data(), pts.size() * 4, hipMemcpyHostToDevice));
  auto run = [&](float* o) -> int {
    float* os = o; float* ou = os + (size_t)B * 3 * (T + 1); float* od = ou + (size_t)B * 2 * T;
    float* omd = od + (size_t)B * T; int32_t* oit = (int32_t*)(omd + B); float* onp = (float*)(oit + B);
    int rc = npa_forward_begin(h, B, N, d_nom_s, d_nom_u, d_ref_s, d_ref_us, obs ? d_pts : nullptr, nullptr, nullptr, os, ou, od,
                               omd, oit, onp, d_ws, wsb, d_state, stb, nullptr, NPA_FWD_RESET_STATE);
    for (int k = 0; k < kmax && rc == NPA_OK; ++k) rc = npa_forward_iter(h, k);
    const int rc2 = npa_forward_end(h);
    return rc != NPA_OK ? rc : rc2;
  };
  std::vector<float> o0(n_out), o1(n_out), o2(n_out);
  int rc = run(d_out[0]);
  if (rc == NPA_OK) rc = run(d_out[1]);
  const bool warm_was = h->qp_warm;
  h->qp_warm = false;
  if (rc == NPA_OK) rc = run(d_out[2]);
  h->qp_warm = warm_was;
  if (rc != NPA_OK) return rc;
  HIP_TRY(hipDeviceSynchronize());
  HIP_TRY(hipMemcpy(o0.data(), d_out[0], n_out * 4, hipMemcpyDeviceToHost));
  HIP_TRY(hipMemcpy(o1.data(), d_out[1], n_out * 4, hipMemcpyDeviceToHost));
  HIP_TRY(hipMemcpy(o2.data(), d_out[2], n_out * 4, hipMemcpyDeviceToHost));
  const size_t n_su = (size_t)B * 3 * (T + 1) + (size_t)B * 2 * T;
  if (memcmp(o0.data(), o1.data(), n_su * 4) != 0)
    return fail(NPA_E_UNSUPPORTED, "npa_create self-test: two runs of the same forward call differ (non-deterministic kernel: "
                                   "this build / runtime combination is not usable; library built with hipcc " NPA_HIPCC_VERSION ")");
  const float* u0 = o0.data() + (size_t)B * 3 * (T + 1);
  const float* u2 = o2.data() + (size_t)B * 3 * (T + 1);
  float warm_gap = 0.f;
  for (int b = 0; b < B; ++b)
    for (int k = 0; k < 2; ++k)
      for (int t = 0; t < T; ++t) {
        const float a = u0[(size_t)b * 2 * T + k * T + t], c = u2[(size_t)b * 2 * T + k * T + t];
        const double sb = P.speed_bound[k];
        for (const float v : {a, c})
          if (!(v == v) || !(std::fabs(v) < 1e30f) || (std::isfinite(sb) && std::fabs(v) > sb + 1e-4 * (1.0 + sb))) {
            char msg[256];
            snprintf(msg, sizeof(msg), "npa_create self-test: control [%d][%d][%d] = %g (bound %g): the QP kernel misbehaves on this "
                                       "build / runtime (hipcc " NPA_HIPCC_VERSION ")", b, k, t, (double)v, sb);
            return fail(NPA_E_UNSUPPORTED, msg);
          }
        warm_gap = std::max(warm_gap, std::fabs(a - c));
      }
  if (warm_gap > 1e-4f && h->qp_warm) {
    h->qp_warm = false;
    h->selftest_flags |= NPA_SELFTEST_WARM_OFF;
  }
  if (obs) {
    auto stage = [&](float* o) -> int {
      float* mu = o; float* lam = mu + (size_t)B * (T + 1) * M * E; float* pt = lam + (size_t)B * (T + 1) * M * 2;
      float* ds = pt + (size_t)B * (T + 1) * M * 2; int32_t* cn = (int32_t*)(ds + (size_t)B * (T + 1) * M);
      return npa_dune_stage(h, B, N, d_nom_s, d_pts, nullptr, nullptr, mu, lam, pt, ds, cn, nullptr);
    };
    rc = stage(d_stage[0]);
    const bool geo2 = h->key_terms == 4 && !h->select_v1 && h->audit_dev && !h->rows_bf16;
    const unsigned one[4] = {0, 0, 1, 0};
    if (rc == NPA_OK && geo2) HIP_TRY(hipMemcpy(h->audit_dev, one, sizeof(one), hipMemcpyHostToDevice));
    if (rc == NPA_OK) rc = stage(d_stage[1]);
    if (rc != NPA_OK) return rc;
    HIP_TRY(hipDeviceSynchronize());
    std::vector<float> s0(n_stage), s1(n_stage);
    HIP_TRY(hipMemcpy(s0.data(), d_stage[0], n_stage * 4, hipMemcpyDeviceToHost));
    HIP_TRY(hipMemcpy(s1.data(), d_stage[1], n_stage * 4, hipMemcpyDeviceToHost));
    const size_t n_rows = (size_t)B * (T + 1) * M * (E + 5);
    auto same_rows = [&]() {
      bool eq = memcmp(s0.data(), s1.data(), n_rows * 4) == 0;
      for (size_t i = n_rows; i < n_stage && eq; ++i) {
        int c0, c1;
        memcpy(&c0, &s0[i], 4); memcpy(&c1, &s1[i], 4);
        eq = (c0 & 0xFF) == (c1 & 0xFF);
      }
      return eq;
    };
    bool same = same_rows();
    if (!same && geo2) {
      HIP_TRY(audit_block_reset(h));
// ... 22 lines not shown
```

neupan_amd/csrc/handle.h:

```cpp
#pragma once
#include "../../include/neupan_amd.h"
#include "pan_common.h"

#include <cstdint>
#include <memory>
#include <mutex>
#include <string>
#include <vector>

inline thread_local std::string g_err;
inline int fail(int code, const std::string& msg) { g_err = msg; return code; }
#define HIP_TRY(expr)                                                                         \
  do {                                                                                        \
    hipError_t e_ = (expr);                                                                   \
    if (e_ != hipSuccess) return fail(NPA_E_HIP, std::string(#expr) + ": " + hipGetErrorString(e_)); \
  } while (0)

#ifndef NPA_HIPCC_VERSION
#define NPA_HIPCC_VERSION "unknown"
#endif

struct EventPair { hipEvent_t a, b; };

struct PendingCall {
  bool active = false;
  int batch = 0, n_stride = 0;
  const float *ref_s = nullptr, *ref_us = nullptr, *points = nullptr, *velocities = nullptr;
  const int32_t* n_points = nullptr;
  float *out_s = nullptr, *out_u = nullptr, *out_d = nullptr, *out_md = nullptr, *out_np = nullptr;
  int32_t* out_iters = nullptr;
  float* ws = nullptr;
  float* state = nullptr;
  hipStream_t stream = nullptr;
  bool dune = false;
  const float *nom_s = nullptr, *nom_u = nullptr;
  bool reset_state = false;
  const float* theta = nullptr;
};

enum class Precision { fp32, bf16, invalid };
struct CalibKnobs {
  int forced_mode = -1;
  double key_safety = -1.0;
  int geo_grid = 4096;
  bool geo_nocheck = false;
  bool geo_table = true;
  double ktab_safety = 2.0, k16_safety = 2.0;
  Precision keys_precision = Precision::fp32, rows_precision = Precision::fp32;
};

struct Calibration {
  int key_terms = 0;
  float key_err = 0.f, key_e0 = 0.f;
  bool key_auto = false;
  float e0_mode[2] = {0.f, 0.f}, err_mode[2] = {0.f, 0.f};
  float geo_err = 0.f, geo_margin = 0.f, geo_refine = 0.f, geo_slope = 0.f, geo_rcal = 0.f, geo_far = 0.f;
  int geo_tab = 0;
  float ktab_err = 0.f, ktab_margin = 0.f;
  bool keys_bf16 = false;
  float k16_err = 0.f, k16_margin = 0.f;
};

struct SharedPack {
  float* wpack = nullptr;
  int device = 0;
  Calibration cal;
  ~SharedPack() {
    if (!wpack) return;
    int cur = -1;
    const bool sw = hipGetDevice(&cur) == hipSuccess && cur != device;
    if (sw) (void)hipSetDevice(device);
    (void)hipFree(wpack);
    if (sw) (void)hipSetDevice(cur);
  }
};

struct npa_handle {
  std::shared_ptr<SharedPack> pack;
  PendingCall pc;
  std::mutex mu;
  DevParams P;
  const float* theta = nullptr;
  int theta_batch = 0;
  float* wpack = nullptr;
  int device = 0;
  int n_cu = 256;
  float* stage_cand = nullptr;
  size_t stage_cand_bytes = 0;
  Calibration cal;
  CalibKnobs knobs;
  int key_terms = 1;
  float key_e0 = 0.f, key_err = 0.f;
  bool qp_warm = true;
  int sel_debug = 0;
  bool geo_valid = false;
  bool select_v1 = false;
  unsigned* audit_dev = nullptr;
  unsigned* audit_host = nullptr;
  bool rows_bf16 = false;
  int selftest_flags = 0;
  unsigned audit_thresh = 0;
  unsigned launch_seq = 0;
  float margin_scale = 1.f;
  unsigned* sel_stats_dev = nullptr;
  unsigned* sel_stats_host = nullptr;
  unsigned stats_mark = 0;
  unsigned long long tiles_window = 0;
  int calls_window = 0, hold = 0;
  bool prof = false;
  std::vector<EventPair> ev_dune, ev_sel, ev_qp;
  size_t n_dune = 0, n_sel = 0, n_qp = 0;
  bool qp_generic = false;
};

inline int mdim(const DevParams& P) { return P.M > 0 ? P.M : 1; }
```

neupan_amd/csrc/nrmp_qp.hip:

```cpp
#include "pan_common.h"
#include <hip/hip_ext.h>
#include <cstdlib>
#include <type_traits>

#include "nrmp_qp_device.h"

static bool qp_fast_path(int T, int M) { return (T == 10 || T == 20) && M == 10; }

extern "C" size_t npa_qp_shmem_bytes_path(int T, int M, int fast) {
  const bool obs = M > 0;
  size_t nu = 2 * T, ldp = nu + 1, mcd = 8 * T - 4 + 2 * T, mf = obs ? (size_t)T * M : 0, npair = nu * (nu + 1) / 2;
  const size_t mfe = (mf + 1) & ~(size_t)1;
  const bool regrows = fast && M > 0 && M % 2 == 0 && T * M / 2 <= QP_THREADS && 5 * T - 2 <= QP_THREADS;
  const size_t rows = (regrows ? 3 : 6) * mcd + (regrows ? 5 : 9) * mfe;
  const bool slim = fast && T > 16;
  const size_t mats = slim ? nu * (nu + 1) / 2 : (fast ? nu * (nu + 1) / 2 + nu * ldp : (size_t)T * 2 * ldp + 2 * nu * ldp);
  const size_t phi = fast ? 0 : (size_t)T * 3 * ldp;
  size_t d = rows + phi + mats + 4 * (T * 3) + T * QP_ABC_LD + (((size_t)T * QP_ST_LD + 1) & ~(size_t)1) + nu + T + (nu + T) + nu + T + nu +
             (fast ? 2 * (size_t)T : 0);
  size_t bytes = d * sizeof(double) + (fast ? 0 : 2 * ((npair + 7) & ~(size_t)7));
  return (bytes + 15) & ~(size_t)15;
}

extern "C" size_t npa_qp_shmem_bytes(int T, int M) { return npa_qp_shmem_bytes_path(T, M, 0); }

extern "C" hipError_t npa_launch_qp(const DevParams& P, int batch, int scene0, const float* cur_s_in,
                                    const float* cur_u_in, const float* ref_s, const float* ref_us,
                                    const float* mu_sorted, const float* lam_sorted, const float* pts_sorted,
                                    const float* dist_sorted, const int* count, float* cur_s_out, float* cur_u_out,
                                    float* cur_d_out, float* out_s, float* out_u, float* out_d,
                                    float* out_min_distance, int* out_iters, float* out_nrmp_points, int* flags,
                                    float* state, double* qp_info, double* warm, float* trig_out, float* dbg_abc,
                                    float* dbg_f, double* dbg_x,
                                    hipStream_t stream, hipEvent_t ev_start, hipEvent_t ev_stop, const float* theta) {
  static const bool force_generic = getenv("NPA_QP_GENERIC") != nullptr;
  const bool fast = qp_fast_path(P.T, P.M) && !force_generic;
  const size_t shmem = npa_qp_shmem_bytes_path(P.T, P.M, fast ? 1 : 0);
  const int nblocks = batch;
  static NpaDeviceOnce attr_set;
  int dev_ = 0;
  if (attr_set.need(&dev_)) {
    hipFuncSetAttribute(reinterpret_cast<const void*>(nrmp_qp_kernel<0, 0>), hipFuncAttributeMaxDynamicSharedMemorySize, 160 * 1024);
    hipFuncSetAttribute(reinterpret_cast<const void*>(nrmp_qp_kernel<10, 10>), hipFuncAttributeMaxDynamicSharedMemorySize, 160 * 1024);
    hipFuncSetAttribute(reinterpret_cast<const void*>(nrmp_qp_kernel<20, 10, false, true>), hipFuncAttributeMaxDynamicSharedMemorySize, 160 * 1024);
    attr_set.done(dev_);
  }
#define QP_LAUNCH(...)                                                                                           \
  hipExtLaunchKernelGGL((nrmp_qp_kernel<__VA_ARGS__>), dim3(nblocks), dim3(QP_THREADS), shmem, stream, ev_start, ev_stop, 0, \
                        P, cur_s_in, cur_u_in, ref_s, ref_us, mu_sorted, lam_sorted, pts_sorted, dist_sorted, count,  \
                        cur_s_out, cur_u_out, cur_d_out, out_s, out_u, out_d, out_min_distance, out_iters,            \
                        out_nrmp_points, flags, state, qp_info, warm, scene0, batch,                                 \
                        QpBackward{nullptr, nullptr, nullptr, nullptr, nullptr, dbg_abc, dbg_f, dbg_x}, trig_out, theta)
  if (fast && P.T == 10) QP_LAUNCH(10, 10);
  else if (fast && P.T == 20) QP_LAUNCH(20, 10, false, true);
  else QP_LAUNCH(0, 0);
#undef QP_LAUNCH
  return hipGetLastError();
}

extern "C" int npa_qp_group_supported(int T, int M) {
  static const bool force_generic = getenv("NPA_QP_GENERIC") != nullptr;
  return !force_generic && M == 10 && (T == 10 || T == 20) ? 1 : 0;
}
extern "C" hipError_t npa_launch_qp_group(const DevParams& P, const QpGroup& G, int n, int batch, hipStream_t stream,
                                          hipEvent_t ev_start, hipEvent_t ev_stop) {
  if (n < 1 || n > NPA_GROUP_MAX || !npa_qp_group_supported(P.T, P.M)) return hipErrorInvalidValue;
  const size_t shmem = npa_qp_shmem_bytes_path(P.T, P.M, 1);
  static NpaDeviceOnce attr_set;
  int dev_ = 0;
  if (attr_set.need(&dev_)) {
    hipFuncSetAttribute(reinterpret_cast<const void*>(nrmp_qp_group_kernel<10, 10>), hipFuncAttributeMaxDynamicSharedMemorySize, 160 * 1024);
    hipFuncSetAttribute(reinterpret_cast<const void*>(nrmp_qp_group_kernel<20, 10, true>), hipFuncAttributeMaxDynamicSharedMemorySize, 160 * 1024);
    attr_set.done(dev_);
  }
  if (P.T == 10)
    hipExtLaunchKernelGGL((nrmp_qp_group_kernel<10, 10>), dim3(batch, n), dim3(QP_THREADS), shmem, stream, ev_start, ev_stop, 0, P, G, batch);
  else
    hipExtLaunchKernelGGL((nrmp_qp_group_kernel<20, 10, true>), dim3(batch, n), dim3(QP_THREADS), shmem, stream, ev_start, ev_stop, 0, P, G, batch);
  return hipGetLastError();
}

extern "C" hipError_t npa_launch_qp_backward(const DevParams& P, int batch, const float* nom_s, const float* nom_u,
                                             const float* ref_s, const float* ref_us, const float* mu_sorted,
                                             const float* lam_sorted, const float* pts_sorted, const int* count,
                                             float* out_s, float* out_u, float* out_d, const float* grad_s,
                                             const float* grad_u, const float* grad_d, float* grad_theta,
                                             float* grad_nom_s, double* qp_info, hipStream_t stream, const float* theta) {
  static const bool force_generic = getenv("NPA_QP_GENERIC") != nullptr;
  const bool fast = qp_fast_path(P.T, P.M) && !force_generic;
  const size_t wave_bytes = npa_qp_shmem_bytes_path(P.T, P.M, fast ? 1 : 0);
  static NpaDeviceOnce attr_set;
  int dev_ = 0;
  if (attr_set.need(&dev_)) {
    hipFuncSetAttribute(reinterpret_cast<const void*>(nrmp_qp_kernel<0, 0, true>), hipFuncAttributeMaxDynamicSharedMemorySize, 160 * 1024);
    hipFuncSetAttribute(reinterpret_cast<const void*>(nrmp_qp_kernel<10, 10, true>), hipFuncAttributeMaxDynamicSharedMemorySize, 160 * 1024);
    hipFuncSetAttribute(reinterpret_cast<const void*>(nrmp_qp_kernel<20, 10, true, true>), hipFuncAttributeMaxDynamicSharedMemorySize, 160 * 1024);
    attr_set.done(dev_);
  }
#define QPB_LAUNCH(...)                                                                                                \
  hipLaunchKernelGGL((nrmp_qp_kernel<__VA_ARGS__>), dim3(batch), dim3(QP_THREADS), wave_bytes, stream, P, nom_s, nom_u, ref_s, \
                     ref_us, mu_sorted, lam_sorted, pts_sorted, (const float*)nullptr, count, out_s, out_u, out_d,        \
                     (float*)nullptr, (float*)nullptr, (float*)nullptr, (float*)nullptr, (int*)nullptr, (float*)nullptr,  \
                     (int*)nullptr, (float*)nullptr, qp_info, (double*)nullptr, 0, batch,                                 \
                     QpBackward{grad_s, grad_u, grad_d, grad_theta, grad_nom_s, nullptr, nullptr, nullptr}, (float*)nullptr, theta)
  if (fast && P.T == 10) QPB_LAUNCH(10, 10, true);
  else if (fast && P.T == 20) QPB_LAUNCH(20, 10, true, true);
  else QPB_LAUNCH(0, 0, true);
#undef QPB_LAUNCH
  return hipGetLastError();
}
```

neupan_amd/csrc/nrmp_qp_body.inc:

```
  double* sm = sm_all;
  if (flags && flags[b * 4 + 0]) return;
  static_assert(!ASET_T, "the active-set launch is retired (DESIGN.md 3.3): ASET_T only keeps the kernels' names");
  if (flags && flags[b * 4 + 3]) {
    if (lane == 0) flags[b * 4 + 3] = 0;
    return;
  }
  __builtin_amdgcn_s_setprio(3);

  PROF_DECL
  const int T = TT > 0 ? TT : P.T, M = (TT > 0 && MM > 0) ? MM : P.M, E = P.E, nu = 2 * T;
  constexpr int NU = TT > 0 ? 2 * TT : 1, T3 = TT > 0 ? 3 * TT : 1;
  const bool obs = M > 0;
  const int mcu = 8 * T - 4;
  const int mf = obs ? T * M : 0;
  const int ldp = nu + 1, ldk = nu + 1;
  const int npair = nu * (nu + 1) / 2;
  const double ro = P.ro_obs, iro = uni64(1.0 / ro);
  float qs0 = P.q_s[0], qs1 = P.q_s[1], qs2 = P.q_s[2], p_u = P.p_u, eta = P.eta, d_max = P.d_max, d_min = P.d_min;
  if (theta) {
    const float* trow = theta + (size_t)b * 8;
    qs0 = uni32(trow[0]); qs1 = uni32(trow[1]); qs2 = uni32(trow[2]); p_u = uni32(trow[3]);
    eta = uni32(trow[4]); d_max = uni32(trow[5]); d_min = uni32(trow[6]);
  }
  const double dmin0 = uni64(fmax((double)d_min, 0.0)), dmaxv = uni64((double)d_max);
  constexpr bool REGROWS = TT > 0 && MM > 0 && (MM % 2) == 0 && TT * MM / 2 <= QP_THREADS && 5 * TT - 2 <= QP_THREADS;
  constexpr bool SCAN = TT > 0 && (TT <= 16 || (SCANW && TT <= 32));
  static_assert(TT == 0 || SCAN, "a fixed horizon without SCAN was the stored-Phi fast path, retired (DESIGN.md 3.3)");
  constexpr bool WIDE = TT > 16;
  constexpr bool SLIM = WIDE && SCAN;
  constexpr int LZERO = NU * (NU - 1) / 2, LDUMP = LZERO + 1;
  constexpr bool DPPB = SCAN && NU > 16 && NU <= 20 && !BWD;
  constexpr int D0 = DPPB ? NU - 16 : 0;
  const int va = DPPB ? (lane < NU ? lane : (lane < 32 ? lane - 16 : 0)) : lane;
  const bool von = DPPB ? lane < 32 : lane < nu;
  const double row0 = lane < 16 ? 1.0 : 0.0;

  const int mcd = mcu + 2 * T;
  const int mcr = REGROWS ? 0 : mcd;
  double* lc = sm;
  double* wc = lc + mcd;
  double* dlc = wc + mcr;
  double* dwc = dlc + mcr;
  double* r2 = dwc + mcd;
  double* iwc = r2 + mcr;
  double* ld_ = lc + mcu; double* wd = wc + mcu; double* dld = dlc + mcu; double* dwd = dwc + mcu;
  double* r2d = r2 + mcu; double* iwd = iwc + mcu;
  const int mfe = (mf + 1) & ~1;
  const int mfr = REGROWS ? 0 : mfe;
  double* fa0 = iwc + mcd;
  double* fa1 = fa0 + mfe;
  double* ff = fa1 + mfe;
  double* lf = ff + mfr;
  double* wf = lf + mfe;
  double* dlf = wf + mfr;
  double* dwf = dlf + mfr;
  double* r3 = dwf + mfe;
  double* iwf = r3 + mfr;
  double* Phi = iwf + mfe;
  double* Ytg = Phi + (SCAN ? 0 : (size_t)T * 3 * ldp);
  double* Hm = Ytg + (TT > 0 ? 0 : (size_t)T * 2 * ldp);
  double* Km = SLIM ? Hm : Hm + (TT > 0 ? (size_t)nu * (nu + 1) / 2 : (size_t)nu * ldk);
  double* cv = SLIM ? Hm + (size_t)nu * (nu + 1) / 2 : Km + (size_t)nu * ldk;
  double* lin = cv + T * 3;
  double* s3 = lin + T * 3;
  double* q3 = s3 + T * 3;
  double* Yt = TT > 0 ? s3 : Ytg;
  double* Abc = q3 + T * 3;
  double* St = Abc + T * QP_ABC_LD;
  double* xu = St + ((T * QP_ST_LD + 1) & ~1);
  double* xd = xu + nu;
  double* xbest = xd + T;
  double* dxu = xbest + nu + T;
  double* dxd = dxu + nu;
  double* invd = dxd + T;
  double* cpre = invd + nu;
  unsigned char* pa = reinterpret_cast<unsigned char*>(TT > 0 ? Km : invd + nu);
  unsigned char* pc = pa + ((npair + 7) & ~7);

  double2 Rwc = make_double2(1.0, 1.0), Rdlc = make_double2(0.0, 0.0), Rr2 = make_double2(0.0, 0.0);
  double2 Rwf = make_double2(1.0, 1.0), Rdlf = make_double2(0.0, 0.0), Rr3 = make_double2(0.0, 0.0), Rff = make_double2(0.0, 0.0);
#define LD_WC(p) (REGROWS ? Rwc : ld2(wc + 2 * (p)))
#define LD_DLC(p) (REGROWS ? Rdlc : ld2(dlc + 2 * (p)))
#define LD_R2(p) (REGROWS ? Rr2 : ld2(r2 + 2 * (p)))
#define LD_WF(h) (REGROWS ? Rwf : ld2(wf + 2 * (h)))
#define LD_DLF(h) (REGROWS ? Rdlf : ld2(dlf + 2 * (h)))
#define LD_R3(h) (REGROWS ? Rr3 : ld2(r3 + 2 * (h)))
#define LD_FF(h) (REGROWS ? Rff : ld2(ff + 2 * (h)))
#define ST_ROW(REG, arr, q, a, b_) do { if constexpr (REGROWS) REG = make_double2((a), (b_)); else st2((arr) + 2 * (q), (a), (b_)); } while (0)

  const float* s_in = cur_s_in + (size_t)b * 3 * (T + 1);
  const float* u_in = cur_u_in + (size_t)b * 2 * T;
  const float* rs = ref_s + (size_t)b * 3 * (T + 1);
  const float* rus = ref_us + (size_t)b * T;

  for (int t = lane; t < T; t += QP_THREADS) {
    float phi = s_in[2 * (T + 1) + t], v = u_in[t], psi = u_in[T + t];
    const float dt32 = P.dt32;
    double* o = Abc + t * QP_ABC_LD;
    float A02 = 0.f, A12 = 0.f, B00, B01 = 0.f, B10, B11 = 0.f, B20 = 0.f, B21 = 0.f, C0, C1, C2 = 0.f;
    if (P.kin == 2) {
      double sp = sin((double)psi), cp = cos((double)psi);
      B00 = (float)(cp * P.dt); B10 = (float)(sp * P.dt);
      B01 = __fmul_rn(__fmul_rn(-v, (float)sp), dt32);
      B11 = __fmul_rn(__fmul_rn(v, (float)cp), dt32);
      C0 = __fmul_rn(__fmul_rn(__fmul_rn(psi, v), (float)sp), dt32);
      C1 = __fmul_rn(__fmul_rn(__fmul_rn(-psi, v), (float)cp), dt32);
    } else {
      double sp = sin((double)phi), cp = cos((double)phi);
      A02 = __fmul_rn(__fmul_rn(-v, dt32), (float)sp);
      A12 = __fmul_rn(__fmul_rn(v, dt32), (float)cp);
      B00 = (float)(cp * P.dt); B10 = (float)(sp * P.dt);
      C0 = __fmul_rn(__fmul_rn(__fmul_rn(phi, v), (float)sp), dt32);
      C1 = __fmul_rn(__fmul_rn(__fmul_rn(-phi, v), (float)cp), dt32);
      if (P.kin == 0) {
        B21 = dt32;
      } else {
        double cps = cos((double)psi); cps = cps * cps;
        float den = (float)(P.L * cps);
        B20 = (float)(tan((double)psi) * P.dt / P.L);
        B21 = __fdiv_rn(__fmul_rn(v, dt32), den);
        C2 = __fdiv_rn(__fmul_rn(__fmul_rn(-psi, v), dt32), den);
      }
    }
    o[0] = A02; o[1] = A12;
    o[2] = B00; o[3] = B01; o[4] = B10; o[5] = B11; o[6] = B20; o[7] = B21;
    o[8] = C0; o[9] = C1; o[10] = C2;
  }
  for (int p = lane; p < (SCAN ? 0 : npair); p += QP_THREADS) {
    int a = (int)((sqrtf(8.0f * (float)p + 1.0f) - 1.0f) * 0.5f);
    while ((a + 1) * (a + 2) / 2 <= p) ++a;
    while (a * (a + 1) / 2 > p) --a;
    pa[p] = (unsigned char)a; pc[p] = (unsigned char)(p - a * (a + 1) / 2);
  }
  const double sb0 = isfinite(P.speed_bound[0]) ? P.speed_bound[0] : 0.0, sb1 = isfinite(P.speed_bound[1]) ? P.speed_bound[1] : 0.0;
  const double ab0 = isfinite(P.acce_bound[0]) ? P.acce_bound[0] : 0.0, ab1 = isfinite(P.acce_bound[1]) ? P.acce_bound[1] : 0.0;
  const double sf0 = isfinite(P.speed_bound[0]) ? 1.0 : 0.0, sf1 = isfinite(P.speed_bound[1]) ? 1.0 : 0.0;
  const double af0 = isfinite(P.acce_bound[0]) ? 1.0 : 0.0, af1 = isfinite(P.acce_bound[1]) ? 1.0 : 0.0;
  const int npu = mcu >> 1, npc = npu + (obs ? T : 0);
#define PAIR_C0(p) qp_pair((p), T, npu, sb0, sb1, ab0, ab1, sf0, sf1, af0, af1, dmaxv, dmin0)
  const PairC my_pair = PAIR_C0(REGROWS && lane < npc ? lane : 0);
#define PAIR_C(p) (REGROWS ? my_pair : PAIR_C0(p))
  constexpr bool HPAIR = TT > 0 && MM > 0 && (MM % 2) == 0;
  LSYNC();

  if constexpr (SCAN) {
    const bool on = lane < TT;
    const double* o = Abc + (on ? lane : 0) * QP_ABC_LD;
    const double a0 = on ? o[0] : 0.0, a1 = on ? o[1] : 0.0, c0 = on ? o[8] : 0.0, c1 = on ? o[9] : 0.0, c2 = on ? o[10] : 0.0;
    const double th0 = s_in[2 * (T + 1)];
    const double thi = scan_prefix<WIDE>(c2), the = th0 + (thi - c2);
    const double x = (double)s_in[0] + scan_prefix<WIDE>(fma(a0, the, c0));
    const double y = (double)s_in[T + 1] + scan_prefix<WIDE>(fma(a1, the, c1));
    const double p0 = scan_prefix<WIDE>(a0), p1 = scan_prefix<WIDE>(a1);
    if (on) {
      cv[lane * 3 + 0] = x; cv[lane * 3 + 1] = y; cv[lane * 3 + 2] = th0 + thi;
      st2(cpre + 2 * lane, p0, p1);
    }
    LSYNC();
  } else
  for (int t = 0; t < T; ++t) {
    const double* o = Abc + t * QP_ABC_LD;
    double* Pt = Phi + (size_t)t * 3 * ldp;
    const double* Pp = Pt - 3 * ldp;
    for (int c = lane; c < nu; c += QP_THREADS) {
      double p0 = 0, p1 = 0, p2 = 0;
      if (t > 0) { p0 = Pp[c]; p1 = Pp[ldp + c]; p2 = Pp[2 * ldp + c]; }
      double n0 = p0 + o[0] * p2, n1 = p1 + o[1] * p2, n2 = p2;
      if (c == 2 * t) { n0 += o[2]; n1 += o[4]; n2 += o[6]; }
      if (c == 2 * t + 1) { n0 += o[3]; n1 += o[5]; n2 += o[7]; }
      Pt[c] = n0; Pt[ldp + c] = n1; Pt[2 * ldp + c] = n2;
    }
    if (lane == 0) {
      double c0, c1, c2;
      if (t == 0) { c0 = s_in[0]; c1 = s_in[T + 1]; c2 = s_in[2 * (T + 1)]; }
      else { c0 = cv[(t - 1) * 3]; c1 = cv[(t - 1) * 3 + 1]; c2 = cv[(t - 1) * 3 + 2]; }
      cv[t * 3 + 0] = c0 + o[0] * c2 + o[8];
      cv[t * 3 + 1] = c1 + o[1] * c2 + o[9];
      cv[t * 3 + 2] = c2 + o[10];
    }
    LSYNC();
  }

  const double m2 = (P.kin == 2) ? 0.0 : 1.0;
  const double W0 = uni64(2.0 * (double)qs0 * (double)qs0 + P.bk);
  const double W1 = uni64(2.0 * (double)qs1 * (double)qs1 + P.bk);
  const double W2 = uni64(2.0 * m2 * (double)qs2 * (double)qs2 + P.bk);
  const double pu = uni64((double)p_u);
  if constexpr (SCAN) {
    for (int q = lane; q < npair; q += QP_THREADS) Hm[q] = 0.0;
  } else
  for (int p = lane; p < npair; p += QP_THREADS) {
    int a = pa[p], c = pc[p];
    double acc = 0;
    for (int t = a >> 1; t < T; ++t) {
      const double* Pt = Phi + (size_t)t * 3 * ldp;
      acc += W0 * Pt[a] * Pt[c] + W1 * Pt[ldp + a] * Pt[ldp + c] + W2 * Pt[2 * ldp + a] * Pt[2 * ldp + c];
    }
    if (a == c && !(a & 1)) acc += 2.0 * pu * pu;
    Hm[a * ldk + c] = acc;
    Hm[c * ldk + a] = acc;
  }
  if constexpr (TT > 0 && !SLIM) {
    LSYNC();
    for (int q = lane; q < nu * ldk; q += QP_THREADS) Km[q] = 0.0;
  }
  double hdiag = 0;
  const double hoff = 0;
  for (int q = lane; q < 3 * T; q += QP_THREADS) {
    int t = q / 3, k = q - 3 * t;
    const float qsk = k == 0 ? qs0 : (k == 1 ? qs1 : qs2);
    double qk = qsk, mk = (k == 2) ? m2 : 1.0, c = cv[q];
    double r = (double)__fmul_rn(qsk, rs[k * (T + 1) + t + 1]);
    lin[q] = 2.0 * mk * qk * (qk * c - r) + P.bk * (c - (double)s_in[k * (T + 1) + t + 1]);
  }

  auto hinge_row = [&](int i) -> double {
    int t = i / M, j = i - t * M;
    size_t row = ((size_t)b * (T + 1) + (t + 1)) * M + j;
    double a0 = 0, a1 = 0, fb = 0;
    const int cnt_t = count[(size_t)b * (T + 1) + t + 1];
    const float l0 = lam_sorted[row * 2], l1 = lam_sorted[row * 2 + 1];
    const float px = pts_sorted[row * 2], py = pts_sorted[row * 2 + 1];
    float muv[NPA_MAX_E];
#pragma unroll
    for (int e = 0; e < NPA_MAX_E; ++e) muv[e] = mu_sorted[row * E + (e < E ? e : 0)];
    if (cnt_t > 0) {
      float tmp = fmaf(l1, py, __fmul_rn(l0, px));
      float mh = 0.f;
#pragma unroll
      for (int e = 0; e < NPA_MAX_E; ++e) mh = e < E ? fmaf(muv[e], P.h[e], mh) : mh;
      a0 = l0; a1 = l1; fb = (double)__fadd_rn(tmp, mh);
    }
    fa0[i] = a0; fa1[i] = a1;
    if (bw.dbg_f) {
      float* o = bw.dbg_f + ((size_t)b * mf + i) * 3;
      o[0] = (float)a0; o[1] = (float)a1; o[2] = (float)fb;
    }
    return fb - (a0 * cv[t * 3] + a1 * cv[t * 3 + 1]);
  };
  if constexpr (REGROWS) {
    if (lane < mf / 2) { const double f0 = hinge_row(2 * lane), f1 = hinge_row(2 * lane + 1); Rff = make_double2(f0, f1); }
  } else {
    for (int i = lane; i < mf; i += QP_THREADS) ff[i] = hinge_row(i);
  }
  if (bw.dbg_abc) {
    for (int q = lane; q < T * 11; q += QP_THREADS) bw.dbg_abc[(size_t)b * T * 11 + q] = (float)Abc[(q / 11) * QP_ABC_LD + (q % 11)];
    return;
  }

  const double d0 = uni64(0.5 * (dmin0 + dmaxv));
  double cmax = fmax(fabs(dmaxv), fabs(dmin0));
  double m_act = 0;
  for (int p = lane; p < npu; p += QP_THREADS) {
    const PairC c = PAIR_C(p);
    if (c.actf != 0.0) { cmax = fmax(cmax, fabs(c.bp)); m_act += 2.0; }
  }
  bool cold_alt = BWD;
  QP_COLD_INIT();
  double gmax = obs ? (double)eta : 0.0;
  if constexpr (SCAN) {
    const bool on = lane < TT;
    const int t = on ? lane : 0;
    const double q0 = on ? lin[3 * t] : 0.0, q1 = on ? lin[3 * t + 1] : 0.0, q2 = on ? lin[3 * t + 2] : 0.0;
    const double l0 = scan_suffix<WIDE>(q0, row0), l1 = scan_suffix<WIDE>(q1, row0);
    const double2 an = ld2(Abc + (t + 1 < TT ? t + 1 : t) * QP_ABC_LD);
    const double l2 = scan_suffix<WIDE>(on ? q2 + an.x * scan_next<WIDE>(l0, lane) + an.y * scan_next<WIDE>(l1, lane) : 0.0, row0);
    const double* o = Abc + t * QP_ABC_LD;
    const double2 b0 = ld2(o + 2), b1 = ld2(o + 4), b2 = ld2(o + 6);
    if (on) {
      const double g0 = b0.x * l0 + b1.x * l1 + b2.x * l2 - 2.0 * pu * (double)__fmul_rn(p_u, rus[t]);
      const double g1 = b0.y * l0 + b1.y * l1 + b2.y * l2;
      gmax = fmax(gmax, fmax(fabs(g0), fabs(g1)));
    }
  } else
  for (int a = lane; a < nu; a += QP_THREADS) {
    double acc = 0;
    for (int t = a >> 1; t < T; ++t) {
      const double* Pt = Phi + (size_t)t * 3 * ldp;
      acc += Pt[a] * lin[t * 3] + Pt[ldp + a] * lin[t * 3 + 1] + Pt[2 * ldp + a] * lin[t * 3 + 2];
    }
    if (!(a & 1)) acc += -2.0 * pu * (double)__fmul_rn(p_u, rus[a >> 1]);
    gmax = fmax(gmax, fabs(acc));
  }
  const double iscale_d = uni64(1.0 / (1.0 + wave_reduce<OpMax>(gmax))), iscale_p = uni64(1.0 / (1.0 + wave_reduce<OpMax>(cmax)));
  const double m_tot = fmax(wave_reduce<OpSum>(m_act) + (double)mf + (obs ? 2.0 * T : 0.0), 1.0);
  const double inv_m = uni64(1.0 / m_tot);
  const double pub = (von && !(va & 1)) ? -2.0 * pu * (double)__fmul_rn(p_u, rus[va >> 1]) : 0.0;
  LSYNC();
  if constexpr (SCAN) hdiag = (lane < NU && !(lane & 1)) ? 2.0 * pu * pu : 0.0;

  double best_merit = 1e300, last_mu = 0;
  int best_it = 0, stall = 0, status = 0, it = 0;

  auto phi_mul = [&](const double* v, double* out3) __attribute__((always_inline)) {
    if constexpr (SCAN) {
      const bool on = lane < TT;
      const int t = on ? lane : 0;
      const double2 vt = ld2(v + 2 * t);
      const double* o = Abc + t * QP_ABC_LD;
      const double2 a01 = ld2(o), b0 = ld2(o + 2), b1 = ld2(o + 4), b2 = ld2(o + 6);
      const double bu2 = on ? b2.x * vt.x + b2.y * vt.y : 0.0;
      const double th = scan_prefix<WIDE>(bu2), thx = th - bu2;
      const double i0 = on ? fma(a01.x, thx, b0.x * vt.x + b0.y * vt.y) : 0.0;
      const double i1 = on ? fma(a01.y, thx, b1.x * vt.x + b1.y * vt.y) : 0.0;
      double x = i0, y = i1;
      scan_prefix2<WIDE>(x, y);
      if (on) { out3[3 * t] = x; out3[3 * t + 1] = y; out3[3 * t + 2] = th; }
      return;
    }
// ... 574 lines not shown
              if (j0 + j < MM / 2) {
                z0 += w2[j].x * p0[j].x; z1 += w2[j].x * p1[j].x; zs += w2[j].x;
                z0 += w2[j].y * p0[j].y; z1 += w2[j].y * p1[j].y; zs += w2[j].y;
              }
            if constexpr (HB < MM / 2) __builtin_amdgcn_sched_barrier(0);
          }
        } else {
#pragma unroll 5
          for (int j = 0; j < M; ++j) { int i = t * M + j; double w = dwf[i]; z0 += w * fa0[i]; z1 += w * fa1[i]; zs += w; }
        }
        double rd = 0;
        const double* S = St + t * QP_ST_LD;
        if (obs) rd = -S[7] - (dwd[2 * t] - dwd[2 * t + 1]) + zs;
        double e = rd * S[6];
        rdr = rd;
        pq0 = -(z0 - S[3] * e);
        pq1 = -(z1 - S[4] * e);
        q3[t * 3 + 0] = pq0; q3[t * 3 + 1] = pq1; q3[t * 3 + 2] = 0.0;
      }
      double rr;
      PROF(5);
      LSYNC();
      PROF_C(2);
      rr = phi_tmul(q3);
      if (von) rr += -r1u - ct_mul(dwc, va);
      PROF_C(3);
      if constexpr (TT > 0) {
        const int lr = DPPB ? va : (lane < NU ? lane : 0);
        rr *= myinv;
        if constexpr (NU <= 20) {
          if constexpr (WV >= 3) {
            {
              double Lrow[NU];
#pragma unroll
              for (int k = 0; k < NU; ++k) Lrow[k] = Km[lr * ldk + k];
              __builtin_amdgcn_sched_barrier(0);
#pragma unroll
              for (int k = 0; k < NU; ++k) rr = fma(-Lrow[k], readlane_f64(rr, k), rr);
            }
            __builtin_amdgcn_sched_barrier(0);
            {
              double Lcol[NU];
#pragma unroll
              for (int k = 0; k < NU; ++k) Lcol[k] = Km[k * ldk + lr];
              __builtin_amdgcn_sched_barrier(0);
#pragma unroll
              for (int k = NU - 1; k >= 0; --k) rr = fma(-Lcol[k], readlane_f64(rr, k), rr);
            }
          } else {
            double Lrow[NU], Lcol[NU];
#pragma unroll
            for (int k = 0; k < NU; ++k) Lrow[k] = Km[lr * ldk + k];
            __builtin_amdgcn_sched_barrier(0);
#pragma unroll
            for (int k = 0; k < NU; ++k) Lcol[k] = Km[k * ldk + lr];
            if constexpr (DPPB) {
              static_for<0, NU>([&](auto K) __attribute__((always_inline)) {
                constexpr int k = decltype(K)::value;
                if constexpr (k < D0) rr = fma(-Lrow[k], readlane_f64(rr, k), rr);
                else subst_rowbcast<(k & 15), k == NU - 1>(rr, Lrow[k]);
              });
              static_for<0, NU>([&](auto K) __attribute__((always_inline)) {
                constexpr int k = NU - 1 - decltype(K)::value;
                if constexpr (k >= 16) rr = fma(-Lcol[k], readlane_f64(rr, k), rr);
                else subst_rowbcast<k, false>(rr, Lcol[k]);
              });
              asm volatile("" : "+v"(rr));
            } else {
#pragma unroll
            for (int k = 0; k < NU; ++k) rr = fma(-Lrow[k], readlane_f64(rr, k), rr);
#pragma unroll
            for (int k = NU - 1; k >= 0; --k) rr = fma(-Lcol[k], readlane_f64(rr, k), rr);
            }
          }
        } else if constexpr (SLIM) {
          int lq = lr;
          asm volatile("" : "+v"(lq));
          const int rbase = lq * (lq - 1) / 2;
#pragma unroll
          for (int k = 0; k < NU - 1; ++k) rr = fma(-Km[k < lq ? rbase + k : LZERO], readlane_f64(rr, k), rr);
          asm volatile("" : "+v"(lq));
#pragma unroll
          for (int k = NU - 1; k >= 1; --k) rr = fma(-Km[lq < k ? k * (k - 1) / 2 + lq : LZERO], readlane_f64(rr, k), rr);
        }
        rr *= myinv;
      } else {
        for (int k = 0; k < nu; ++k) {
          double yk = readlane_f64(rr * myinv, k);
          if (lane == k) rr = yk;
          if (lane > k && lane < nu) rr = fma(-Km[(size_t)lane * ldk + k], yk, rr);
        }
        for (int k = nu - 1; k >= 0; --k) {
          double xk = readlane_f64(rr * myinv, k);
          if (lane == k) rr = xk;
          if (lane < k) rr = fma(-Km[(size_t)k * ldk + lane], xk, rr);
        }
      }
      if (lane < nu) dxu[lane] = rr;
      LSYNC();
      PROF(6); PROF_C(4);
      phi_mul(dxu, s3);
      LSYNC();
      for (int t = lane; t < T && obs; t += QP_THREADS)
        dxd[t] = (rdr + St[t * QP_ST_LD + 3] * s3[t * 3] + St[t * QP_ST_LD + 4] * s3[t * 3 + 1]) * St[t * QP_ST_LD + 6];
      LSYNC();
      PROF_C(5);
      double amax = 1.0, gap_aff = 0;
      double ainv = 1.0;
      auto ratio = [&](double l, double dl, double w, double dw) { ainv = fmax(fmax(ainv, -dl * rough_rcp(l)), -dw * rough_rcp(w)); };
      auto ratio_iw = [&](double l, double dl, double iwv, double dw) { ainv = fmax(fmax(ainv, -dl * rough_rcp(l)), -dw * iwv); };
      if constexpr (HPAIR) {
        for (int h = lane; h < mf / 2; h += QP_THREADS) {
          const int t = h / (MM / 2), i = 2 * h;
          const double2 l = ld2(lf + i), w = LD_WF(h), a0 = ld2(fa0 + i), a1 = ld2(fa1 + i), iw = ld2(iwf + i), tw = ld2(dwf + i), r = LD_R3(h);
          const double sx = s3[t * 3], sy = s3[t * 3 + 1], d = dxd[t];
          const double Fx = a0.x * sx + a1.x * sy - d, Fy = a0.y * sx + a1.y * sy - d;
          const double dlx = -(tw.x + l.x * Fx * iw.x), dly = -(tw.y + l.y * Fy * iw.y);
          const double dwx = Fx + dlx * iro + r.x, dwy = Fy + dly * iro + r.y;
          ratio(l.x, dlx, w.x, dwx); ratio(l.y, dly, w.y, dwy);
          ST_ROW(Rdlf, dlf, h, dlx, dly); st2(dwf + i, dwx, dwy);
        }
      } else {
        for (int i = lane; i < mf; i += QP_THREADS) {
          int t = i / M;
          double l = lf[i], w = wf[i];
          double Fdx = fa0[i] * s3[t * 3] + fa1[i] * s3[t * 3 + 1] - dxd[t];
          double dl = -(dwf[i] + l * Fdx * iwf[i]);
          double dw = Fdx + dl * iro + r3[i];
          ratio(l, dl, w, dw);
          dlf[i] = dl; dwf[i] = dw;
        }
      }
      for (int p = lane; p < npc; p += QP_THREADS) {
        const PairC c = PAIR_C(p);
        const int i = 2 * p;
        const double2 l = ld2(lc + i), w = LD_WC(p), iw = ld2(iwc + i), tw = ld2(dwc + i), r = LD_R2(p);
        const double Cdx = fma(-c.sb, dxu[c.ib], dxu[c.ia]);
        const double dlx = tw.x + l.x * Cdx * iw.x, dly = tw.y - l.y * Cdx * iw.y;
        const double dwx = (-r.x - Cdx) * c.actf, dwy = (Cdx - r.y) * c.actf;
        ratio_iw(l.x, dlx, iw.x, dwx); ratio_iw(l.y, dly, iw.y, dwy);
        ST_ROW(Rdlc, dlc, p, dlx, dly); st2(dwc + i, dwx, dwy);
      }
      PROF_C(6);
      amax = rough_rcp(wave_reduce<OpMax>(ainv));
      if (pass == 0) {
        if constexpr (HPAIR) {
          for (int h = lane; h < mf / 2; h += QP_THREADS) {
            const double2 l = ld2(lf + 2 * h), w = LD_WF(h), dl = LD_DLF(h), dw = ld2(dwf + 2 * h);
            gap_aff += (l.x + amax * dl.x) * (w.x + amax * dw.x) + (l.y + amax * dl.y) * (w.y + amax * dw.y);
          }
        } else {
          for (int i = lane; i < mf; i += QP_THREADS) gap_aff += (lf[i] + amax * dlf[i]) * (wf[i] + amax * dwf[i]);
        }
        for (int p = lane; p < npc; p += QP_THREADS) {
          const double2 l = ld2(lc + 2 * p), w = LD_WC(p), dl = LD_DLC(p), dw = ld2(dwc + 2 * p);
          gap_aff += (l.x + amax * dl.x) * (w.x + amax * dw.x) + (l.y + amax * dl.y) * (w.y + amax * dw.y);
        }
        double mu_aff = wave_reduce<OpSum>(gap_aff) * inv_m;
        double sg = mu_aff * fast_rcp(mu);
        sigma_mu = fmax(fmax(sg * sg * sg * mu, QP_SIGMA_MU_MIN), (BWD ? 0.0 : QP_SIGMA_MU_RES) * rmax);
        corr_w = amax >= QP_CORRECTOR_MIN_AFF ? 1.0 : 0.0;
      } else {
        alpha = fmin(1.0, fmin(fmax(QP_STEP_ETA, 1.0 - mu), 1.0 - QP_STEP_CAP) * amax);
        for (int tr = 0; tr < QP_CENTRAL_TRIES && alpha < QP_CENTRAL_ALPHA; ++tr) {
          double psum = 0.0, pmin = 1e300;
          if constexpr (HPAIR) {
            for (int h = lane; h < mf / 2; h += QP_THREADS) {
              const double2 l = ld2(lf + 2 * h), w = LD_WF(h), dl = LD_DLF(h), dw = ld2(dwf + 2 * h);
              const double px = (l.x + alpha * dl.x) * (w.x + alpha * dw.x), py = (l.y + alpha * dl.y) * (w.y + alpha * dw.y);
              psum += px + py; pmin = fmin(pmin, fmin(px, py));
            }
          } else {
            for (int i = lane; i < mf; i += QP_THREADS) {
              const double pr = (lf[i] + alpha * dlf[i]) * (wf[i] + alpha * dwf[i]);
              psum += pr; pmin = fmin(pmin, pr);
            }
          }
          for (int p = lane; p < npc; p += QP_THREADS) {
            const PairC c = PAIR_C(p);
            const double2 l = ld2(lc + 2 * p), w = LD_WC(p), dl = LD_DLC(p), dw = ld2(dwc + 2 * p);
            const double px = (l.x + alpha * dl.x) * (w.x + alpha * dw.x), py = (l.y + alpha * dl.y) * (w.y + alpha * dw.y);
            if (c.actf != 0.0) { psum += px + py; pmin = fmin(pmin, fmin(px, py)); }
          }
          wave_reduce2<OpSum, OpMin>(psum, pmin);
          if (pmin >= QP_CENTRAL_GAMMA * psum * inv_m) break;
          alpha *= QP_CENTRAL_SHRINK;
        }
      }
      LSYNC();
      PROF(7); PROF_C(7);
    }
    if constexpr (BWD) {
      if (adj) {
        double g0 = 0, g1 = 0, g2 = 0, gp = 0, ge = 0, gmx = 0, gmn = 0;
        for (int q = lane; q < 3 * T; q += QP_THREADS) {
          int k = q % 3;
          double v = s3[q] * lin[q];
          g0 += k == 0 ? v : 0.0; g1 += k == 1 ? v : 0.0; g2 += k == 2 ? v : 0.0;
        }
        for (int t = lane; t < T; t += QP_THREADS) {
          double refu = (double)__fmul_rn(p_u, rus[t]) / (p_u != 0.f ? (double)p_u : 1.0);
          gp += dxu[2 * t] * (xu[2 * t] - refu);
          if (obs) {
            ge += dxd[t];
            if constexpr (!REGROWS) { gmx += dld[2 * t]; gmn += dld[2 * t + 1]; }
          }
        }
        if constexpr (REGROWS) {
          if (obs && lane >= npu && lane < npc) { gmx = Rdlc.x; gmn = Rdlc.y; }
        }
        if (bw.grad_nom_s) {
          float* gn = bw.grad_nom_s + (size_t)b * 3 * (T + 1);
          for (int q = lane; q < 3 * (T + 1); q += QP_THREADS) {
            int k = q / (T + 1), t = q - k * (T + 1);
            gn[q] = (t == 0) ? 0.f : (float)((double)P.bk * s3[(t - 1) * 3 + k]);
          }
        }
        g0 = wave_reduce<OpSum>(g0); g1 = wave_reduce<OpSum>(g1); g2 = wave_reduce<OpSum>(g2);
        gp = wave_reduce<OpSum>(gp); ge = wave_reduce<OpSum>(ge);
        gmx = wave_reduce<OpSum>(gmx); gmn = wave_reduce<OpSum>(gmn);
        if (lane == 0) {
          float* gt = bw.grad_theta + (size_t)b * 8;
          gt[0] = (float)(-4.0 * (double)qs0 * g0);
          gt[1] = (float)(-4.0 * (double)qs1 * g1);
          gt[2] = (float)(-4.0 * m2 * (double)qs2 * g2);
          gt[3] = (float)(-4.0 * pu * gp);
          gt[4] = (float)ge;
          gt[5] = (float)gmx;
          gt[6] = (d_min > 0.f) ? (float)(-gmn) : 0.f;
          gt[7] = (float)status;
        }
        break;
      }
    }
    for (int a = lane; a < nu; a += QP_THREADS) xu[a] += alpha * dxu[a];
    for (int t = lane; t < T && obs; t += QP_THREADS) xd[t] += alpha * dxd[t];
    if constexpr (HPAIR) {
      for (int h = lane; h < mf / 2; h += QP_THREADS) {
        const double2 l = ld2(lf + 2 * h), w = LD_WF(h), dl = LD_DLF(h), dw = ld2(dwf + 2 * h);
        st2(lf + 2 * h, l.x + alpha * dl.x, l.y + alpha * dl.y); ST_ROW(Rwf, wf, h, w.x + alpha * dw.x, w.y + alpha * dw.y);
      }
    } else {
      for (int i = lane; i < mf; i += QP_THREADS) { lf[i] += alpha * dlf[i]; wf[i] += alpha * dwf[i]; }
    }
    for (int p = lane; p < npc; p += QP_THREADS) {
      const double2 l = ld2(lc + 2 * p), w = LD_WC(p), dl = LD_DLC(p), dw = ld2(dwc + 2 * p);
      st2(lc + 2 * p, l.x + alpha * dl.x, l.y + alpha * dl.y); ST_ROW(Rwc, wc, p, w.x + alpha * dw.x, w.y + alpha * dw.y);
    }
    LSYNC();
    PROF(8);
  }
  LSYNC();
  it_total += it;
  if (warm_now) warm_code = 1;
  if (status == 0 && !(best_merit <= QP_RETRY_MERIT)) status = 4;

  if (bw.dbg_x)
    for (int a = lane; a < nu + T; a += QP_THREADS) bw.dbg_x[(size_t)b * (nu + T) + a] = (a < nu || obs) ? xbest[a] : 0.0;
  float* so = cur_s_out + (size_t)b * 3 * (T + 1);
  float* uo = cur_u_out + (size_t)b * 2 * T;
  phi_mul(xbest, s3);
  LSYNC();
  float* stage = reinterpret_cast<float*>(Km);
  for (int q = lane; q < 3 * (T + 1); q += QP_THREADS) {
    int k = q / (T + 1), t = q - k * (T + 1);
    stage[q] = (t == 0) ? s_in[k * (T + 1)] : (float)(s3[(t - 1) * 3 + k] + cv[(t - 1) * 3 + k]);
  }
  LSYNC();
  for (int q = lane; q < 3 * (T + 1); q += QP_THREADS) {
    float fv = stage[q];
    so[q] = fv;
    if (out_s) out_s[(size_t)b * 3 * (T + 1) + q] = fv;
  }
  if (trig_out)
    for (int t = lane; t <= T; t += QP_THREADS) {
      float c, sn;
      npa_trig(stage[2 * (T + 1) + t], c, sn);
      trig_out[((size_t)b * (T + 1) + t) * 2] = c;
      trig_out[((size_t)b * (T + 1) + t) * 2 + 1] = sn;
    }
  for (int q = lane; q < 2 * T; q += QP_THREADS) {
    int k = q / T, t = q - k * T;
    float fv = (float)xbest[2 * t + k];
    uo[q] = fv;
    if (out_u) out_u[(size_t)b * 2 * T + q] = fv;
  }
  if (obs)
    for (int t = lane; t < T; t += QP_THREADS) {
      float fv = (float)xbest[nu + t];
      if (cur_d_out) cur_d_out[(size_t)b * T + t] = fv;
      if (out_d) out_d[(size_t)b * T + t] = fv;
    }
  if (wrm) {
    for (int a = lane; a < nu + T; a += QP_THREADS) wrm[a] = xbest[a];
    for (int i = lane; i < mf; i += QP_THREADS) wrm[nu + T + i] = lf[i];
    for (int i = lane; i < mcu; i += QP_THREADS) wrm[nu + T + mf + i] = lc[i];
    for (int i = lane; i < 2 * T && obs; i += QP_THREADS) wrm[nu + T + mf + mcu + i] = ld_[i];
    if (flags && lane == 0) flags[b * 4 + 2] = (status == 0 && best_merit <= 1e-12) ? 1 : 0;
  }
  if (qp_info && lane == 0) {
    double* qi = qp_info + (size_t)b * QP_INFO_STRIDE;
    qi[0] = best_it; qi[1] = best_merit; qi[2] = last_mu; qi[3] = status; qi[4] = it;
    qi[14] = it_total; qi[15] = warm_code;
#ifndef NPA_QP_PROF
    if (P.qp_aset && !(can_warm)) { qi[5] = 0; qi[6] = 0; qi[7] = 0; qi[8] = 0; }
#endif
#ifdef NPA_QP_PROF
    PROF(9);
    for (int i = 0; i < 10; ++i) qi[5 + i] = (double)pacc_[i];
#endif
  }

  const int cnt0 = (obs && count) ? count[(size_t)b * (T + 1)] : 0;
  if (out_min_distance && lane == 0) {
    float mdv = __builtin_inff();
    const bool have_md = obs && cnt0 > 0;
    if (have_md) mdv = dist_sorted[(size_t)b * (T + 1) * M];
    if (state) {
      const int Ms_ = M > 0 ? M : 1;
      int* tail = reinterpret_cast<int*>(state + (size_t)(b + 1) * npa_state_floats(T, Ms_, E)) - 4;
      if (have_md) { tail[2] = 1; tail[3] = __float_as_int(mdv); }
      else if (tail[2]) mdv = __int_as_float(tail[3]);
    }
    out_min_distance[b] = mdv;
  }
  if (out_nrmp_points && obs)
    for (int q = lane; q < 2 * M; q += QP_THREADS) {
      int k = q / M, j = q - k * M;
      out_nrmp_points[(size_t)b * 2 * M + q] = cnt0 > 0 ? pts_sorted[((size_t)b * (T + 1) * M + j) * 2 + k] : 0.f;
    }

  if (state && flags) {
    const int Ms = M > 0 ? M : 1;
    const size_t nsf = npa_state_floats(T, Ms, E);
    float* st = state + (size_t)b * nsf;
    float* ps = st;
    float* pu_ = ps + 3 * (T + 1);
    float* pmu = pu_ + 2 * T;
    float* plam = pmu + (size_t)(T + 1) * Ms * E;
    int* pint = reinterpret_cast<int*>(plam + (size_t)(T + 1) * Ms * 2);
    const int valid = pint[0], prev_n = pint[1];
    const bool have = obs && cnt0 > 0;
    double acc_s = 0, acc_u = 0, acc_mu = 0, acc_lam = 0;
    int eff = 0;
    if (valid) {
      if (!have || prev_n == 0) {
        for (int q = lane; q < 3 * (T + 1); q += QP_THREADS) { double d = (double)stage[q] - (double)ps[q]; acc_s += d * d; }
        for (int q = lane; q < 2 * T; q += QP_THREADS) {
          int k = q / T, t = q - k * T;
          double d = (double)(float)xbest[2 * t + k] - (double)pu_[q];
          acc_u += d * d;
        }
      } else {
        eff = cnt0 < prev_n ? cnt0 : prev_n;
        for (int q = lane; q < (T + 1) * eff; q += QP_THREADS) {
          int t = q / eff, j = q - t * eff;
          size_t row = ((size_t)b * (T + 1) + t) * M + j;
          size_t prow = (size_t)t * M + j;
          float mn[NPA_MAX_E], mo[NPA_MAX_E], ln[2], lo[2];
#pragma unroll
          for (int e = 0; e < NPA_MAX_E; ++e) { const int ee = e < E ? e : 0; mn[e] = mu_sorted[row * E + ee]; mo[e] = pmu[prow * E + ee]; }
#pragma unroll
          for (int k = 0; k < 2; ++k) { ln[k] = lam_sorted[row * 2 + k]; lo[k] = plam[prow * 2 + k]; }
#pragma unroll
          for (int e = 0; e < NPA_MAX_E; ++e) { const double d = (double)mn[e] - (double)mo[e]; acc_mu = e < E ? fma(d, d, acc_mu) : acc_mu; }
#pragma unroll
          for (int k = 0; k < 2; ++k) { const double d = (double)ln[k] - (double)lo[k]; acc_lam = fma(d, d, acc_lam); }
        }
      }
    }
    acc_s = wave_reduce<OpSum>(acc_s); acc_u = wave_reduce<OpSum>(acc_u);
    acc_mu = wave_reduce<OpSum>(acc_mu); acc_lam = wave_reduce<OpSum>(acc_lam);
    for (int q = lane; q < 3 * (T + 1); q += QP_THREADS) ps[q] = stage[q];
    for (int q = lane; q < 2 * T; q += QP_THREADS) { int k = q / T, t = q - k * T; pu_[q] = (float)xbest[2 * t + k]; }
    if (have)
      for (int q = lane; q < (T + 1) * M; q += QP_THREADS) {
        size_t row = (size_t)b * (T + 1) * M + q;
        float mn[NPA_MAX_E];
#pragma unroll
        for (int e = 0; e < NPA_MAX_E; ++e) mn[e] = mu_sorted[row * E + (e < E ? e : 0)];
        const float ln0 = lam_sorted[row * 2], ln1 = lam_sorted[row * 2 + 1];
#pragma unroll
        for (int e = 0; e < NPA_MAX_E; ++e) if (e < E) pmu[(size_t)q * E + e] = mn[e];
        plam[(size_t)q * 2] = ln0; plam[(size_t)q * 2 + 1] = ln1;
      }
    if (lane == 0) {
      pint[0] = 1;
      pint[1] = have ? cnt0 : 0;
      int stop = 0;
      if (valid) {
        float diff;
        if (!have || prev_n == 0) diff = (float)(acc_s + acc_u);
        else {
          float md = (float)sqrt(acc_mu) / (float)eff, ldv = (float)sqrt(acc_lam) / (float)eff;
          diff = md * md + ldv * ldv;
        }
        stop = diff < P.iter_threshold ? 1 : 0;
      }
      flags[b * 4 + 1] += 1;
      if (stop) flags[b * 4 + 0] = 1;
      if (out_iters) out_iters[b] = flags[b * 4 + 1];
    }
  }
```

neupan_amd/csrc/nrmp_qp_device.h:

```cpp
#pragma once
#define QP_THREADS 64
#ifndef NPA_QP_WAVES
#define NPA_QP_WAVES 2
#endif
#define QP_MAX_IT 40
#define QP_ABC_LD 14
#define QP_ST_LD 9
#define QP_WARM_DELTA 0.003
#define QP_STEP_ETA 0.995
#define QP_STEP_CAP 1e-6
#define QP_START_MU 3.0
#ifndef NPA_QP_WIDE_LDS
#define NPA_QP_WIDE_LDS 1
#endif
#ifndef QP_WLDS_CH
#define QP_WLDS_CH 4
#endif
#ifndef QP_CHOL_LOOK
#define QP_CHOL_LOOK 3
#endif
#define QP_RETRY_MERIT 1e-9
#define QP_SIGMA_MU_MIN 1e-15
#define QP_SIGMA_MU_RES 0.01
#define QP_STALL_NEAR_MERIT 1e-6
#define QP_STALL_FAR 8
#define QP_CENTRAL_GAMMA 1e-3
#define QP_CENTRAL_SHRINK 0.7
#define QP_CENTRAL_TRIES 6
#define QP_CENTRAL_ALPHA 0.9
#define QP_CORRECTOR_MIN_AFF 0.1
#define QP_COLD_INIT()                                                                            \
  do {                                                                                            \
    for (int a = lane; a < nu; a += QP_THREADS) { xu[a] = 0.0; xbest[a] = 0.0; }                  \
    for (int t = lane; t < T; t += QP_THREADS) { xd[t] = d0; xbest[nu + t] = d0; dxd[t] = 0.0; }  \
    for (int p = lane; p < npc; p += QP_THREADS) {                                                \
      const PairC c = PAIR_C(p);                                                                  \
      const double cx = p >= npu ? d0 : 0.0;                           \
      const bool on = c.actf != 0.0;                                                              \
      const double w0p = on ? fmax(c.bp - cx, 1.0) : 1.0, w0m = on ? fmax(c.bm + cx, 1.0) : 1.0;  \
      st2(lc + 2 * p, c.actf * (cold_alt ? 1.0 : QP_START_MU * fast_rcp(w0p)), c.actf * (cold_alt ? 1.0 : QP_START_MU * fast_rcp(w0m))); \
      ST_ROW(Rwc, wc, p, w0p, w0m);                                                               \
      ST_ROW(Rdlc, dlc, p, 0.0, 0.0); st2(dwc + 2 * p, 0.0, 0.0);                                 \
    }                                                                                             \
    LSYNC();                                                                                      \
    if constexpr (REGROWS) {                                                                      \
      if (lane < mf / 2) {                                                                        \
         \
        const double hx = -d0 - Rff.x, hy = -d0 - Rff.y;                                          \
        const double l0x = cold_alt ? 1.0 : QP_START_MU * fast_rcp(fmax(hx + iro, 1.0));          \
        const double l0y = cold_alt ? 1.0 : QP_START_MU * fast_rcp(fmax(hy + iro, 1.0));          \
        Rwf = make_double2(fmax(hx + l0x * iro, 1.0), fmax(hy + l0y * iro, 1.0));                 \
        st2(lf + 2 * lane, cold_alt ? 1.0 : QP_START_MU * fast_rcp(Rwf.x), cold_alt ? 1.0 : QP_START_MU * fast_rcp(Rwf.y)); \
      }                                                                                           \
    } else {                                                                                      \
      for (int i = lane; i < mf; i += QP_THREADS) {                                               \
        const double hx = -d0 - ff[i];                                      \
        const double l0x = cold_alt ? 1.0 : QP_START_MU * fast_rcp(fmax(hx + iro, 1.0));          \
        wf[i] = fmax(hx + l0x * iro, 1.0);                                                        \
        lf[i] = cold_alt ? 1.0 : QP_START_MU * fast_rcp(wf[i]);                                   \
      }                                                                                           \
    }                                                                                             \
    LSYNC();                                                                                      \
  } while (0)
#define QP_INFO_STRIDE 16
#ifdef NPA_QP_PROF
#define PROF_DECL unsigned long long pt_ = __builtin_amdgcn_s_memtime(), pacc_[10] = {0, 0, 0, 0, 0, 0, 0, 0, 0, 0};
#define PROF_AT(i) do { unsigned long long n_ = __builtin_amdgcn_s_memtime(); pacc_[i] += n_ - pt_; pt_ = n_; } while (0)
#define PROF(i) do { if (NPA_QP_PROF == 1 || (i) == 0 || (i) == 9) PROF_AT(i); } while (0)
#define PROF_B(i) do { if (NPA_QP_PROF == 2) PROF_AT(i); } while (0)
#define PROF_C(i) do { if (NPA_QP_PROF == 3) PROF_AT(i); } while (0)
#else
#define PROF_DECL
#define PROF(i) do { } while (0)
#define PROF_B(i) do { } while (0)
#define PROF_C(i) do { } while (0)
#endif

__device__ __forceinline__ double readlane_f64(double v, int l) {
  unsigned lo = __builtin_amdgcn_readlane((unsigned)__double2loint(v), l);
  unsigned hi = __builtin_amdgcn_readlane((unsigned)__double2hiint(v), l);
  return __hiloint2double((int)hi, (int)lo);
}
template <int CTRL>
__device__ __forceinline__ double dpp_f64(double v) {
  int lo = __builtin_amdgcn_update_dpp(0, __double2loint(v), CTRL, 0xF, 0xF, false);
  int hi = __builtin_amdgcn_update_dpp(0, __double2hiint(v), CTRL, 0xF, 0xF, false);
  return __hiloint2double(hi, lo);
}
template <int CTRL>
__device__ __forceinline__ double dpp0_f64(double v) {
  int lo = __builtin_amdgcn_update_dpp(0, __double2loint(v), CTRL, 0xF, 0xF, true);
  int hi = __builtin_amdgcn_update_dpp(0, __double2hiint(v), CTRL, 0xF, 0xF, true);
  return __hiloint2double(hi, lo);
}
__device__ __forceinline__ double row_prefix_sum(double v) {
  v += dpp0_f64<0x111>(v); v += dpp0_f64<0x112>(v); v += dpp0_f64<0x114>(v); v += dpp0_f64<0x118>(v);
  return v;
}
__device__ __forceinline__ double row_suffix_sum(double v) {
  v += dpp0_f64<0x101>(v); v += dpp0_f64<0x102>(v); v += dpp0_f64<0x104>(v); v += dpp0_f64<0x108>(v);
  return v;
}
template <bool WIDE>
__device__ __forceinline__ double scan_prefix(double v) {
  v = row_prefix_sum(v);
  if constexpr (WIDE) {
    int lo = __builtin_amdgcn_update_dpp(0, __double2loint(v), 0x142, 0xA, 0xF, false);
    int hi = __builtin_amdgcn_update_dpp(0, __double2hiint(v), 0x142, 0xA, 0xF, false);
    v += __hiloint2double(hi, lo);
  }
  return v;
}
template <bool WIDE>
__device__ __forceinline__ double scan_suffix(double v, double row0) {
  v = row_suffix_sum(v);
  if constexpr (WIDE) {
    const unsigned lo = __builtin_amdgcn_readlane((unsigned)__double2loint(v), 16);
    const unsigned hi = __builtin_amdgcn_readlane((unsigned)__double2hiint(v), 16);
    v = fma(row0, __hiloint2double((int)hi, (int)lo), v);
  }
  return v;
}
template <bool WIDE>
__device__ __forceinline__ double scan_next(double v, int lane) {
  double x = dpp0_f64<0x101>(v);
  if constexpr (WIDE) {
    const unsigned lo = __builtin_amdgcn_readlane((unsigned)__double2loint(v), 16);
    const unsigned hi = __builtin_amdgcn_readlane((unsigned)__double2hiint(v), 16);
    if (lane == 15) x = __hiloint2double((int)hi, (int)lo);
  }
  return x;
}
#define QP_SCAN_STEP2(CT) do { a += dpp0_f64<CT>(a); __builtin_amdgcn_sched_barrier(0); b += dpp0_f64<CT>(b); __builtin_amdgcn_sched_barrier(0); } while (0)
#define QP_SCAN_STEP3(CT) do { a += dpp0_f64<CT>(a); __builtin_amdgcn_sched_barrier(0); b += dpp0_f64<CT>(b); __builtin_amdgcn_sched_barrier(0); \
                               c += dpp0_f64<CT>(c); __builtin_amdgcn_sched_barrier(0); } while (0)
template <bool WIDE>
__device__ __forceinline__ void scan_prefix2(double& a, double& b) {
  __builtin_amdgcn_sched_barrier(0);
  QP_SCAN_STEP2(0x111); QP_SCAN_STEP2(0x112); QP_SCAN_STEP2(0x114); QP_SCAN_STEP2(0x118);
  if constexpr (WIDE) {
    a += __hiloint2double(__builtin_amdgcn_update_dpp(0, __double2hiint(a), 0x142, 0xA, 0xF, false), __builtin_amdgcn_update_dpp(0, __double2loint(a), 0x142, 0xA, 0xF, false));
    b += __hiloint2double(__builtin_amdgcn_update_dpp(0, __double2hiint(b), 0x142, 0xA, 0xF, false), __builtin_amdgcn_update_dpp(0, __double2loint(b), 0x142, 0xA, 0xF, false));
  }
}
template <bool WIDE>
__device__ __forceinline__ void scan_suffix2(double& a, double& b, double row0) {
  __builtin_amdgcn_sched_barrier(0);
  QP_SCAN_STEP2(0x101); QP_SCAN_STEP2(0x102); QP_SCAN_STEP2(0x104); QP_SCAN_STEP2(0x108);
  if constexpr (WIDE) { a = fma(row0, readlane_f64(a, 16), a); b = fma(row0, readlane_f64(b, 16), b); }
}
template <bool WIDE>
__device__ __forceinline__ void scan_suffix3(double& a, double& b, double& c, double row0) {
  __builtin_amdgcn_sched_barrier(0);
  QP_SCAN_STEP3(0x101); QP_SCAN_STEP3(0x102); QP_SCAN_STEP3(0x104); QP_SCAN_STEP3(0x108);
  if constexpr (WIDE) { a = fma(row0, readlane_f64(a, 16), a); b = fma(row0, readlane_f64(b, 16), b); c = fma(row0, readlane_f64(c, 16), c); }
}
template <int N, bool LEAD, bool TAIL>
__device__ __forceinline__ void fmac_rowbcast(double& acc, double& src, double mul) {
  static_assert(N >= 0 && N < 16, "row_newbcast lane");
  if constexpr (LEAD && TAIL)
    asm("s_nop 1\n\tv_fmac_f64_dpp %0, %1, -%2 row_newbcast:%3 row_mask:0xf bank_mask:0xf\n\ts_nop 0" : "+v"(acc), "+v"(src) : "v"(mul), "n"(N));
  else if constexpr (LEAD)
    asm("s_nop 1\n\tv_fmac_f64_dpp %0, %1, -%2 row_newbcast:%3 row_mask:0xf bank_mask:0xf" : "+v"(acc), "+v"(src) : "v"(mul), "n"(N));
  else if constexpr (TAIL)
    asm("v_fmac_f64_dpp %0, %1, -%2 row_newbcast:%3 row_mask:0xf bank_mask:0xf\n\ts_nop 0" : "+v"(acc) : "v"(src), "v"(mul), "n"(N));
  else
    asm("v_fmac_f64_dpp %0, %1, -%2 row_newbcast:%3 row_mask:0xf bank_mask:0xf" : "+v"(acc) : "v"(src), "v"(mul), "n"(N));
}
template <int N, bool TAIL>
__device__ __forceinline__ void subst_rowbcast(double& x, double mul) {
  static_assert(N >= 0 && N < 16, "row_newbcast lane");
  if constexpr (TAIL)
    asm("s_nop 1\n\tv_fmac_f64_dpp %0, %0, -%1 row_newbcast:%2 row_mask:0xf bank_mask:0xf\n\ts_nop 0" : "+v"(x) : "v"(mul), "n"(N));
  else
    asm("s_nop 1\n\tv_fmac_f64_dpp %0, %0, -%1 row_newbcast:%2 row_mask:0xf bank_mask:0xf" : "+v"(x) : "v"(mul), "n"(N));
}
typedef __attribute__((address_space(3))) double lds_f64;
__device__ __forceinline__ unsigned lds_addr(const double* p) { return (unsigned)(size_t)((const lds_f64*)p); }
template <unsigned MASK, int OFF, bool LAST, unsigned RESTORE>
__device__ __forceinline__ void park_store(unsigned addr, double v) {
  if constexpr (LAST)
    asm volatile("s_mov_b64 exec, %2\n\tds_write_b64 %0, %1 offset:%3\n\ts_mov_b64 exec, %4\n\ts_nop 4" : : "v"(addr), "v"(v), "n"(MASK), "n"(OFF), "n"(RESTORE) : "memory");
  else
    asm volatile("s_mov_b64 exec, %2\n\tds_write_b64 %0, %1 offset:%3\n\ts_mov_b64 exec, %4" : : "v"(addr), "v"(v), "n"(MASK), "n"(OFF), "n"(RESTORE) : "memory");
}
template <int C, int N>
__device__ __forceinline__ void park_rows(unsigned lrow, const double (&arow)[N], double myinv) {
  constexpr unsigned ALL = (1u << N) - 1u;
  if constexpr (C + 4 <= N - 1) {
    const double v0 = arow[C] * myinv, v1 = arow[C + 1] * myinv, v2 = arow[C + 2] * myinv, v3 = arow[C + 3] * myinv;
    asm volatile("s_mov_b64 exec, %5\n\tds_write_b64 %0, %1 offset:%9\n\ts_mov_b64 exec, %6\n\tds_write_b64 %0, %2 offset:%10\n\t"
                 "s_mov_b64 exec, %7\n\tds_write_b64 %0, %3 offset:%11\n\ts_mov_b64 exec, %8\n\tds_write_b64 %0, %4 offset:%12\n\ts_mov_b64 exec, %13"
                 : : "v"(lrow), "v"(v0), "v"(v1), "v"(v2), "v"(v3),
                     "n"(ALL & ~((2u << C) - 1u)), "n"(ALL & ~((2u << (C + 1)) - 1u)), "n"(ALL & ~((2u << (C + 2)) - 1u)), "n"(ALL & ~((2u << (C + 3)) - 1u)),
                     "n"(C * 8), "n"(C * 8 + 8), "n"(C * 8 + 16), "n"(C * 8 + 24), "n"(ALL) : "memory");
    park_rows<C + 4, N>(lrow, arow, myinv);
  } else if constexpr (C < N - 1) {
    park_store<ALL & ~((2u << C) - 1u), C * 8, C == N - 2, ALL>(lrow, arow[C] * myinv);
    park_rows<C + 1, N>(lrow, arow, myinv);
  }
}
template <int I, int N, class F>
__device__ __forceinline__ void static_for(F&& f) {
  if constexpr (I < N) { f(std::integral_constant<int, I>{}); static_for<I + 1, N>(f); }
}
__device__ __forceinline__ double uni64(double v) {
  return __hiloint2double(__builtin_amdgcn_readfirstlane(__double2hiint(v)), __builtin_amdgcn_readfirstlane(__double2loint(v)));
}
__device__ __forceinline__ float uni32(float v) { return __int_as_float(__builtin_amdgcn_readfirstlane(__float_as_int(v))); }
struct OpSum { __device__ static double f(double a, double b) { return a + b; } };
struct OpMax { __device__ static double f(double a, double b) { return fmax(a, b); } };
struct OpMin { __device__ static double f(double a, double b) { return fmin(a, b); } };
template <class Op>
__device__ __forceinline__ double wave_reduce(double v) {
  v = Op::f(v, dpp0_f64<0xB1>(v));
  v = Op::f(v, dpp0_f64<0x4E>(v));
  v = Op::f(v, dpp0_f64<0x141>(v));
  v = Op::f(v, dpp0_f64<0x140>(v));
  v = Op::f(v, dpp0_f64<0x142>(v));
  v = Op::f(v, dpp0_f64<0x143>(v));
  return readlane_f64(v, 63);
}
template <class OpA, class OpB>
__device__ __forceinline__ void wave_reduce2(double& a, double& b) {
#define QP_RED_STEP2(CT) do { a = OpA::f(a, dpp0_f64<CT>(a)); __builtin_amdgcn_sched_barrier(0); b = OpB::f(b, dpp0_f64<CT>(b)); __builtin_amdgcn_sched_barrier(0); } while (0)
  __builtin_amdgcn_sched_barrier(0);
  QP_RED_STEP2(0xB1); QP_RED_STEP2(0x4E); QP_RED_STEP2(0x141); QP_RED_STEP2(0x140); QP_RED_STEP2(0x142); QP_RED_STEP2(0x143);
#undef QP_RED_STEP2
  a = readlane_f64(a, 63); b = readlane_f64(b, 63);
}
__device__ __forceinline__ double fast_rcp(double x) {
  double r = __builtin_amdgcn_rcp(x);
  r = fma(fma(-x, r, 1.0), r, r);
  r = fma(fma(-x, r, 1.0), r, r);
  return r;
}
__device__ __forceinline__ double rough_rcp(double x) { return __builtin_amdgcn_rcp(x); }
__device__ __forceinline__ double fast_rsqrt(double x) {
  double y = __builtin_amdgcn_rsq(x);
  y = y * fma(-0.5 * x * y, y, 1.5);
  return y;
}
__device__ __forceinline__ double2 ld2(const double* p) { return *reinterpret_cast<const double2*>(p); }
__device__ __forceinline__ void st2(double* p, double a, double b) { *reinterpret_cast<double2*>(p) = make_double2(a, b); }
#define LSYNC()                                              \
  do {                                                       \
    __builtin_amdgcn_fence(__ATOMIC_SEQ_CST, "wavefront");   \
    __builtin_amdgcn_wave_barrier();                         \
  } while (0)

struct QpBackward {
  const float* grad_s;
  const float* grad_u;
  const float* grad_d;
  float* grad_theta;
  float* grad_nom_s;
  float* dbg_abc;
  float* dbg_f;
  double* dbg_x;
};

struct PairC { int ia, ib; double sb, bp, bm, actf; };
__device__ __forceinline__ PairC qp_pair(int p, int T, int npu, double sb0, double sb1, double ab0, double ab1, double sf0,
                                         double sf1, double af0, double af1, double dmaxv, double dmin0) {
  PairC c;
  const bool is_d = p >= npu, is_rate = p >= 2 * T && !is_d;
  const int q = p - 2 * T;
  const bool odd = ((is_rate ? q : p) & 1) != 0;
  c.ia = is_d ? 2 * T + (p - npu) : (is_rate ? q + 2 : p);
  c.ib = is_rate ? q : 0;
  c.sb = is_rate ? 1.0 : 0.0;
  const double bs = odd ? sb1 : sb0, ba = odd ? ab1 : ab0, fs = odd ? sf1 : sf0, fa = odd ? af1 : af0;
  const double bd = is_rate ? ba : bs;
  c.actf = is_d ? 1.0 : (is_rate ? fa : fs);
  c.bp = is_d ? dmaxv : bd;
  c.bm = is_d ? -dmin0 : bd;
  return c;
}

template <int TT, int MM, bool BWD = false, bool SCANW = false, int WV = NPA_QP_WAVES, bool ASET_T = false>
__global__ __attribute__((amdgpu_flat_work_group_size(QP_THREADS, QP_THREADS), amdgpu_waves_per_eu(WV, 3)))
void nrmp_qp_kernel(
    DevParams P, const float* cur_s_in, const float* cur_u_in, const float* __restrict__ ref_s,
    const float* __restrict__ ref_us, const float* __restrict__ mu_sorted, const float* __restrict__ lam_sorted,
    const float* __restrict__ pts_sorted, const float* __restrict__ dist_sorted, const int* __restrict__ count,
    float* cur_s_out, float* cur_u_out, float* __restrict__ cur_d_out, float* __restrict__ out_s,
    float* __restrict__ out_u, float* __restrict__ out_d, float* __restrict__ out_min_distance,
    int* __restrict__ out_iters, float* __restrict__ out_nrmp_points, int* __restrict__ flags,
    float* __restrict__ state, double* __restrict__ qp_info, double* __restrict__ warm, int scene0, int nscene,
    QpBackward bw, float* __restrict__ trig_out, const float* __restrict__ theta) {
  extern __shared__ __attribute__((aligned(16))) double sm_all[];
  const int lane = threadIdx.x;
  if ((int)blockIdx.x >= nscene) return;
  const int b = blockIdx.x + scene0;
#include "nrmp_qp_body.inc"
}

template <int TT, int MM, bool SCANW = false>
__global__ __attribute__((amdgpu_flat_work_group_size(QP_THREADS, QP_THREADS), amdgpu_waves_per_eu(NPA_QP_WAVES, 3)))
void nrmp_qp_group_kernel(DevParams P, QpGroup G, int nscene) {
  extern __shared__ __attribute__((aligned(16))) double sm_all[];
  constexpr bool BWD = false, ASET_T = false;
  constexpr int WV = NPA_QP_WAVES;
  const int lane = threadIdx.x;
  if ((int)blockIdx.x >= nscene) return;
  const int b = blockIdx.x;
  const QpCall& q = G.c[blockIdx.y];
  const float* cur_s_in = q.cur_s_in; const float* cur_u_in = q.cur_u_in;
  const float* __restrict__ ref_s = q.ref_s; const float* __restrict__ ref_us = q.ref_us;
  const float* __restrict__ mu_sorted = q.mu_sorted; const float* __restrict__ lam_sorted = q.lam_sorted;
  const float* __restrict__ pts_sorted = q.pts_sorted; const float* __restrict__ dist_sorted = q.dist_sorted;
  const int* __restrict__ count = q.count;
  float* cur_s_out = q.cur_s_out; float* cur_u_out = q.cur_u_out; float* __restrict__ cur_d_out = q.cur_d_out;
  float* __restrict__ out_s = q.out_s; float* __restrict__ out_u = q.out_u; float* __restrict__ out_d = q.out_d;
  float* __restrict__ out_min_distance = q.out_min_distance; int* __restrict__ out_iters = q.out_iters;
  float* __restrict__ out_nrmp_points = q.out_nrmp_points; int* __restrict__ flags = q.flags; float* __restrict__ state = q.state;
  double* __restrict__ qp_info = q.qp_info; double* __restrict__ warm = q.warm; float* __restrict__ trig_out = q.trig_out;
  const float* __restrict__ theta = q.theta;
  const QpBackward bw{nullptr, nullptr, nullptr, nullptr, nullptr, nullptr, nullptr, nullptr};
#include "nrmp_qp_body.inc"
}
```

neupan_amd/csrc/pan_common.h:

```cpp
#pragma once
#include <hip/hip_runtime.h>
#include <stdint.h>
#include <atomic>

#define NPA_MAX_T 21
#define NPA_MAX_M 32
#define NPA_MAX_E 8
#define NPA_MAX_POINTS 32768

struct NpaDeviceOnce {
  std::atomic<unsigned long long> mask{0};
  bool need(int* dev_out) {
    int d = 0;
    if (hipGetDevice(&d) != hipSuccess) d = 0;
    *dev_out = d;
    return !(mask.load(std::memory_order_acquire) & (1ull << (d & 63)));
  }
  void done(int d) { mask.fetch_or(1ull << (d & 63), std::memory_order_release); }
};

struct DevParams {
  int T, M, E, kin, K, dune_max_num;
  int key_stride;
  float iter_threshold;
  float dt32;
  double dt, L;
  double speed_bound[2], acce_bound[2];
  double ro_obs, bk;
  float q_s[3], p_u, eta, d_max, d_min;
  float G[NPA_MAX_E][2];
  float h[NPA_MAX_E];
  float pvx[NPA_MAX_E], pvy[NPA_MAX_E], pdx[NPA_MAX_E], pdy[NPA_MAX_E], pil[NPA_MAX_E];
  float geo_rcal;
  float geo_far;
  int geo_rect;
  float rcx, rcy, rhx, rhy;
  int qp_aset;
  int geo_tab;
};

#define NPA_GROUP_MAX 8
struct SelGeoCall {
  const float* wpack; const float* cur_s; const float* points; const float* vel; const int* n_points; const int* flags;
  float* mu_sorted; float* lam_sorted; float* pts_sorted; float* dist_sorted; int* count; unsigned* stats; const float* trig;
  unsigned* audit; int n_stride; unsigned audit_seed;
};
struct SelGeoGroup { SelGeoCall c[NPA_GROUP_MAX]; };
struct QpCall {
  const float* cur_s_in; const float* cur_u_in; const float* ref_s; const float* ref_us; const float* mu_sorted;
  const float* lam_sorted; const float* pts_sorted; const float* dist_sorted; const int* count; float* cur_s_out;
  float* cur_u_out; float* cur_d_out; float* out_s; float* out_u; float* out_d; float* out_min_distance; int* out_iters;
  float* out_nrmp_points; int* flags; float* state; double* qp_info; double* warm; float* trig_out;
  const float* theta;
};
struct QpGroup { QpCall c[NPA_GROUP_MAX]; };
struct StageCall {
  float* cur_s; const float* nom_s; float* cur_u; const float* nom_u; int* flags; int* count; int* state; float* trig;
};
struct StageGroup { StageCall c[NPA_GROUP_MAX]; };

#define NPA_GEO_BANDS 88
#define NPA_GEO_KEY_FAR 0x7F800000u
__host__ __device__ inline int npa_geo_band(float g) {
  union { float f; unsigned u; } v;
  v.f = g + 0.25f;
  if (v.u & 0x80000000u) return 0;
  const int b = (int)(v.u >> 20) - (int)(0x3E800000u >> 20);
  return b < 0 ? 0 : (b >= NPA_GEO_BANDS ? NPA_GEO_BANDS - 1 : b);
}

#define WP_W1 0
#define WP_WL (WP_W1 + 64)
#define WP_VEC (WP_WL + 4 * 16 * 64)
#define WP_W6 (WP_VEC + 11 * 32)
#define WP_B6 (WP_W6 + 8 * 32)
#define WP_BF (WP_B6 + 8)
#define WP_BF_FLOATS (4 * 2 * 2 * 64 * 4)
#define WP_KVEC (WP_BF + WP_BF_FLOATS)
#define WP_KSC (WP_KVEC + 5 * 32)
#define WP_KW1 (WP_KSC + 8)
#define WP_KEY_LDS_FLOATS (WP_BF_FLOATS + 5 * 32 + 8)
#define WP_GEO (WP_KW1 + 64)
#define WP_WLS (((WP_GEO + NPA_GEO_BANDS) + 3) & ~3)
#define WP_WB16 (WP_WLS + 4 * 64 * 16)
#define WP_WB16_FLOATS (4 * 2 * 64 * 4)
#define WP_K16 (WP_WB16 + WP_WB16_FLOATS)
#define WP_KTAB (WP_K16 + ((NPA_GEO_BANDS + 3) & ~3))
#define WP_TABH (WP_KTAB + ((NPA_GEO_BANDS + 3) & ~3))
#define WP_W116 (WP_TABH + 8)
#define WP_WL16 (WP_W116 + 2 * 64)
#define WP_VEC16 (WP_WL16 + 4 * 64 * 16)
#define WP_VEC16_FLOATS (11 * 32 + 8 * 32 + 8)
#define WP_TOTAL (WP_VEC16 + WP_VEC16_FLOATS)
#define NPA_TAB_KEY_FAR 0xFFFFFFFDu
#define NPA_TAB_N 512
#define NPA_TAB_LEVELS 4
#define NPA_TAB_HALF0 2.0f
#define WP_TAB ((WP_TOTAL + 3) & ~3)
#define WP_TAB_FLOATS (NPA_TAB_LEVELS * NPA_TAB_N * NPA_TAB_N * 2)
enum { V_B1 = 0, V_G1, V_BE1, V_B2, V_B3, V_G2, V_BE2, V_B4, V_B5, V_G3, V_BE3 };

__host__ __device__ inline int npa_feat(int r, int hf) { return (r & 3) + 8 * (r >> 2) + 4 * hf; }
__host__ __device__ inline int npa_feat16(int s, int kq) { return 8 * (s >> 1) + 2 * (s & 1) + (kq >> 1) + 4 * (kq & 1); }

__host__ __device__ inline size_t npa_state_floats(int T, int M, int E) {
  return (size_t)3 * (T + 1) + 2 * T + (size_t)(T + 1) * M * E + (size_t)(T + 1) * M * 2 + 4;
}

__device__ inline void npa_trig(float th, float& c, float& s) {
  c = (float)cos((double)th);
  s = (float)sin((double)th);
}

struct ScratchLayout {
  size_t cur_s, cur_u, cur_d, mu, lam, pts, dist, count, flags, warm, qp_info, trig, keys, total;
};
__host__ __device__ inline size_t npa_warm_doubles(int T, int M) {
  return (size_t)2 * T + T + (size_t)T * M + (8 * T - 4) + 2 * T;
}
__host__ __device__ inline ScratchLayout npa_scratch_layout(int B, int T, int M, int E, int key_stride) {
  ScratchLayout L;
  size_t o = 0;
  auto take = [&](size_t n) { size_t r = o; o += (n + 3) & ~(size_t)3; return r; };
  L.cur_s = take((size_t)B * 3 * (T + 1));
  L.cur_u = take((size_t)B * 2 * T);
  L.cur_d = take((size_t)B * T);
  L.mu = take((size_t)B * (T + 1) * M * E);
  L.lam = take((size_t)B * (T + 1) * M * 2);
  L.pts = take((size_t)B * (T + 1) * M * 2);
  L.dist = take((size_t)B * (T + 1) * M);
  L.count = take((size_t)B * (T + 1));
  L.flags = take((size_t)B * 4);
  o = (o + 3) & ~(size_t)3;
  L.warm = take((size_t)B * npa_warm_doubles(T, M) * 2);
  L.qp_info = take((size_t)B * 16 * 2);
  L.trig = take((size_t)B * (T + 1) * 2);
  L.keys = take((size_t)B * (T + 1) * key_stride);
  L.total = o;
  return L;
}
```

Measured before the change: 858,300 plans/s.

## Schedule QP blocks longest-first using previous iteration's iteration counts

Each QP launch now files every scene into one of 32 buckets by its inner iteration count, using atomic counters and lists in new workspace scratch. The next MPC iteration's launch maps block index to scene through a DPP prefix scan over those buckets, so the scenes that took the most iterations are dispatched first and the tail of the grid is shorter. In the grouped kernel, blocks from the different calls are also interleaved by rank. The change adds atomics, a scratch region and a per-block pick cost, and it removes the flags[3] early-exit path and the qp_aset clearing of qp_info.

After: 895,900 plans/s (median of 6 runs). +4.4%, better.

```diff
diff --git a/neupan_amd/csrc/c_api.hip b/neupan_amd/csrc/c_api.hip
--- a/neupan_amd/csrc/c_api.hip
+++ b/neupan_amd/csrc/c_api.hip
@@ -36,7 +36,8 @@
                                     float* out_s, float* out_u, float* out_d, float* out_min_distance,
                                     int* out_iters, float* out_nrmp_points, int* flags, float* state,
                                     double* qp_info, double* warm, float* trig_out, float* dbg_abc, float* dbg_f, double* dbg_x,
-                                    hipStream_t stream, hipEvent_t ev_start, hipEvent_t ev_stop, const float* theta);
+                                    hipStream_t stream, hipEvent_t ev_start, hipEvent_t ev_stop, const float* theta,
+                                    QpSched sched);
 extern "C" int npa_select_geo_group_supported(int E);
 extern "C" hipError_t npa_launch_select_geo_group(const DevParams& P, const SelGeoGroup& G, int n, int batch, int t0, int n_stride_max,
                                                   int debug, unsigned audit_thresh, float margin_scale, int rows_bf16,
@@ -71,17 +72,17 @@
 
 extern "C" size_t npa_workspace_bytes(const npa_handle* h, int batch) {
   if (!h || batch < 1) return 0;
-  return npa_scratch_layout(batch, h->P.T, mdim(h->P), h->P.E, kstride(h)).total * sizeof(float);
+  return npa_scratch_layout(batch, h->P.T, mdim(h->P), h->P.E, kstride(h), h->P.K).total * sizeof(float);
 }
 extern "C" size_t npa_workspace_qp_info_offset(const npa_handle* h, int batch) {
   if (!h || batch < 1) return 0;
-  return npa_scratch_layout(batch, h->P.T, mdim(h->P), h->P.E, kstride(h)).qp_info * sizeof(float);
+  return npa_scratch_layout(batch, h->P.T, mdim(h->P), h->P.E, kstride(h), h->P.K).qp_info * sizeof(float);
 }
 extern "C" int npa_workspace_layout(const npa_handle* h, int batch, size_t* out, int n) {
   if (!h || batch < 1 || !out || n < 1) return fail(NPA_E_ARG, "npa_workspace_layout: bad argument");
-  const ScratchLayout L = npa_scratch_layout(batch, h->P.T, mdim(h->P), h->P.E, kstride(h));
-  const size_t v[8] = {L.cur_s * 4, L.cur_u * 4, L.cur_d * 4, L.mu * 4, L.lam * 4, L.pts * 4, L.dist * 4, L.count * 4};
-  for (int i = 0; i < n && i < 8; ++i) out[i] = v[i];
+  const ScratchLayout L = npa_scratch_layout(batch, h->P.T, mdim(h->P), h->P.E, kstride(h), h->P.K);
+  const size_t v[9] = {L.cur_s * 4, L.cur_u * 4, L.cur_d * 4, L.mu * 4, L.lam * 4, L.pts * 4, L.dist * 4, L.count * 4, L.sched * 4};
+  for (int i = 0; i < n && i < 9; ++i) out[i] = v[i];
   return NPA_OK;
 }
 extern "C" size_t npa_state_bytes(const npa_handle* h, int batch) {
@@ -182,7 +183,8 @@
   if (int rc = check_theta_batch(h, batch, "npa_nrmp_stage")) return rc;
   HIP_TRY(npa_launch_qp(h->P, batch, 0, nom_s, nom_u, ref_s, ref_us, mu_sorted, lam_sorted, pts_sorted, nullptr, count,
                         out_s, out_u, out_d, nullptr, nullptr, nullptr, nullptr, nullptr, nullptr, nullptr, nullptr,
-                        qp_info, nullptr, nullptr, nullptr, nullptr, x64, (hipStream_t)stream, nullptr, nullptr, h->theta));
+                        qp_info, nullptr, nullptr, nullptr, nullptr, x64, (hipStream_t)stream, nullptr, nullptr, h->theta,
+                        QpSched{nullptr, nullptr, nullptr, nullptr, nullptr}));
   return NPA_OK;
 }
 
@@ -195,7 +197,8 @@
   HIP_TRY(npa_launch_qp(h->P, batch, 0, nom_s, nom_u, nom_s, nom_u, mu_sorted, lam_sorted, pts_sorted, nullptr, count,
                         nullptr, nullptr, nullptr, nullptr, nullptr, nullptr, nullptr, nullptr, nullptr, nullptr, nullptr,
                         nullptr, nullptr, nullptr, out_abc, h->P.M > 0 ? out_f : nullptr, nullptr, (hipStream_t)stream, nullptr, nullptr,
-                        nullptr));
+                        nullptr,
+                        QpSched{nullptr, nullptr, nullptr, nullptr, nullptr}));
   return NPA_OK;
 }
 
@@ -223,7 +226,8 @@
 __global__ void stage_kernel(float* __restrict__ cur_s, const float* __restrict__ nom_s, size_t ns,
                              float* __restrict__ cur_u, const float* __restrict__ nom_u, size_t nu,
                              int* __restrict__ flags, size_t nflag, int* __restrict__ count, size_t ncount,
-                             int* __restrict__ state, size_t nstate, float* __restrict__ trig, int T) {
+                             int* __restrict__ state, size_t nstate, float* __restrict__ trig, int T,
+                             int* __restrict__ sched_cnt, size_t nsched) {
   const size_t stride = (size_t)gridDim.x * blockDim.x;
   for (size_t i = (size_t)blockIdx.x * blockDim.x + threadIdx.x;; i += stride) {
     bool any = false;
@@ -238,15 +242,17 @@
     if (i < nflag) { flags[i] = 0; any = true; }
     if (i < ncount) { count[i] = 0; any = true; }
     if (i < nstate) { state[i] = 0; any = true; }
+    if (i < nsched) { sched_cnt[i] = 0; any = true; }
     if (!any) break;
   }
 }
 
-__global__ void stage_group_kernel(StageGroup G, size_t ns, size_t nu, size_t nflag, size_t ncount, size_t nstate, int T) {
+__global__ void stage_group_kernel(StageGroup G, size_t ns, size_t nu, size_t nflag, size_t ncount, size_t nstate, int T,
+                                   size_t nsched) {
   const StageCall& q = G.c[blockIdx.y];
   float* __restrict__ cur_s = q.cur_s; const float* __restrict__ nom_s = q.nom_s; float* __restrict__ cur_u = q.cur_u;
   const float* __restrict__ nom_u = q.nom_u; int* __restrict__ flags = q.flags; int* __restrict__ count = q.count;
-  int* __restrict__ state = q.state; float* __restrict__ trig = q.trig;
+  int* __restrict__ state = q.state; float* __restrict__ trig = q.trig; int* __restrict__ sched_cnt = q.sched_cnt;
   const size_t stride = (size_t)gridDim.x * blockDim.x;
   for (size_t i = (size_t)blockIdx.x * blockDim.x + threadIdx.x;; i += stride) {
     bool any = false;
@@ -261,8 +267,22 @@
     if (i < nflag) { flags[i] = 0; any = true; }
     if (i < ncount) { count[i] = 0; any = true; }
     if (i < nstate) { state[i] = 0; any = true; }
+    if (i < nsched) { sched_cnt[i] = 0; any = true; }
     if (!any) break;
   }
+}
+
+static QpSched sched_ptrs(const npa_handle* h, PendingCall* pc, const ScratchLayout& L) {
+  QpSched s{nullptr, nullptr, nullptr, nullptr, nullptr};
+  const int j = pc->qp_seq++;
+  if (!h->qp_order || j >= h->P.K) return s;
+  int* cnt = (int*)(pc->ws + L.sched);
+  int* list = cnt + npa_sched_cnt_ints(h->P.K);
+  const size_t set = (size_t)NPA_SCHED_NCLS * pc->batch;
+  if (j > 0) { s.in_cnt = cnt + (size_t)(j - 1) * NPA_SCHED_NCLS; s.in_list = list + (size_t)((j - 1) & 1) * set; }
+  s.out_cnt = cnt + (size_t)j * NPA_SCHED_NCLS; s.out_list = list + (size_t)(j & 1) * set;
+  s.ticket = list + 2 * set;
+  return s;
 }
 
 static void key_policy(npa_handle* h, int batch, int n_stride) {
@@ -308,7 +328,7 @@
   hipStream_t stream = (hipStream_t)stream_;
   const int T = P.T;
   const bool reset_state = (flags & NPA_FWD_RESET_STATE) != 0;
-  const ScratchLayout L = npa_scratch_layout(batch, T, mdim(P), P.E, kstride(h));
+  const ScratchLayout L = npa_scratch_layout(batch, T, mdim(P), P.E, kstride(h), h->P.K);
   float* ws = (float*)workspace;
   pc->batch = batch; pc->n_stride = n_stride; pc->ref_s = ref_s; pc->ref_us = ref_us; pc->points = points;
   pc->velocities = velocities; pc->n_points = n_points; pc->out_s = out_s; pc->out_u = out_u; pc->out_d = out_d;
@@ -317,16 +337,19 @@
   pc->dune = P.M > 0 && points != nullptr;
   pc->nom_s = nom_s; pc->nom_u = nom_u; pc->reset_state = reset_state;
   pc->theta = h->theta;
+  pc->qp_seq = 0;
   if (pc->dune) key_policy(h, batch, n_stride);
   if (launch_stage) {
     const size_t ns = (size_t)batch * 3 * (T + 1), nu2 = (size_t)batch * 2 * T;
     const size_t nflag = (size_t)batch * 4, ncount = (size_t)batch * (T + 1);
     const size_t nstate = reset_state ? npa_state_bytes(h, batch) / 4 : 0;
-    const size_t work = std::max(std::max(ns, nu2), std::max(std::max(nflag, ncount), nstate));
+    const size_t nsched = npa_sched_cnt_ints(P.K);
+    const size_t work = std::max(std::max(std::max(ns, nu2), nsched), std::max(std::max(nflag, ncount), nstate));
     const int threads = 256;
     const int blocks = (int)std::min<size_t>((work + threads - 1) / threads, 512);
     hipLaunchKernelGGL(stage_kernel, dim3(blocks), dim3(threads), 0, stream, ws + L.cur_s, nom_s, ns, ws + L.cur_u, nom_u, nu2,
-                       (int*)(ws + L.flags), nflag, (int*)(ws + L.count), ncount, (int*)state, nstate, ws + L.trig, T);
+                       (int*)(ws + L.flags), nflag, (int*)(ws + L.count), ncount, (int*)state, nstate, ws + L.trig, T,
+                       (int*)(ws + L.sched), nsched);
     HIP_TRY(hipGetLastError());
   }
   pc->active = true;
@@ -399,21 +422,23 @@
   npa_handle* h0 = calls[0].h;
   const DevParams& P = h0->P;
   const int T = P.T, batch = calls[0].batch;
-  const ScratchLayout L = npa_scratch_layout(batch, T, mdim(P), P.E, kstride(h0));
+  const ScratchLayout L = npa_scratch_layout(batch, T, mdim(P), P.E, kstride(h0), h0->P.K);
   StageGroup G;
   memset(&G, 0, sizeof(G));
   for (int c = 0; c < n; ++c) {
     const PendingCall& pc = calls[c].h->pc;
     G.c[c] = StageCall{pc.ws + L.cur_s, pc.nom_s, pc.ws + L.cur_u, pc.nom_u, (int*)(pc.ws + L.flags), (int*)(pc.ws + L.count),
-                       (int*)pc.state, pc.ws + L.trig};
+                       (int*)pc.state, pc.ws + L.trig, (int*)(pc.ws + L.sched)};
   }
   const size_t ns = (size_t)batch * 3 * (T + 1), nu2 = (size_t)batch * 2 * T;
   const size_t nflag = (size_t)batch * 4, ncount = (size_t)batch * (T + 1);
   const size_t nstate = h0->pc.reset_state ? npa_state_bytes(h0, batch) / 4 : 0;
-  const size_t work = std::max(std::max(ns, nu2), std::max(std::max(nflag, ncount), nstate));
+  const size_t nsched = npa_sched_cnt_ints(P.K);
+  const size_t work = std::max(std::max(std::max(ns, nu2), nsched), std::max(std::max(nflag, ncount), nstate));
   const int threads = 256;
   const int blocks = (int)std::min<size_t>((work + threads - 1) / threads, 512);
-  hipLaunchKernelGGL(stage_group_kernel, dim3(blocks, n), dim3(threads), 0, h0->pc.stream, G, ns, nu2, nflag, ncount, nstate, T);
+  hipLaunchKernelGGL(stage_group_kernel, dim3(blocks, n), dim3(threads), 0, h0->pc.stream, G, ns, nu2, nflag, ncount, nstate, T,
+                     nsched);
   HIP_TRY(hipGetLastError());
   return NPA_OK;
 }
@@ -427,7 +452,7 @@
   const DevParams& P = h0->P;
   if (k < 0 || k >= P.K) return fail(NPA_E_ARG, "npa_forward_batch_group: iteration index out of range");
   const int T = P.T, batch = calls[0].batch;
-  const ScratchLayout L = npa_scratch_layout(batch, T, mdim(P), P.E, kstride(h0));
+  const ScratchLayout L = npa_scratch_layout(batch, T, mdim(P), P.E, kstride(h0), h0->P.K);
   hipStream_t stream = h0->pc.stream;
   for (int c = 0; c < n; ++c)
     if (!calls[c].h->pc.active) return fail(NPA_E_ARG, "npa_forward_batch_group: a call of the group is not in progress");
@@ -459,7 +484,7 @@
     Q.c[c] = QpCall{cur_s, cur_u, pc.ref_s, pc.ref_us, ws + L.mu, ws + L.lam, ws + L.pts, ws + L.dist, (const int*)(ws + L.count),
                     cur_s, cur_u, ws + L.cur_d, pc.out_s, pc.out_u, pc.out_d, pc.out_md, pc.out_iters, pc.out_np,
                     (int*)(ws + L.flags), pc.state, (double*)(ws + L.qp_info), h->qp_warm ? (double*)(ws + L.warm) : nullptr,
-                    pc.dune ? ws + L.trig : nullptr, pc.theta};
+                    pc.dune ? ws + L.trig : nullptr, pc.theta, sched_ptrs(h, &h->pc, L)};
   }
   EventPair* ev = next_event(h0, h0->ev_qp, h0->n_qp);
   HIP_TRY(npa_launch_qp_group(P, Q, n, batch, stream, ev ? ev->a : nullptr, ev ? ev->b : nullptr));
@@ -476,7 +501,7 @@
   if (k < 0 || k >= P.K) return fail(NPA_E_ARG, "npa_forward_iter: iteration index out of range");
   const int T = P.T, batch = pc->batch;
   const bool geo = h->key_terms == 4;
-  const ScratchLayout L = npa_scratch_layout(batch, T, mdim(P), P.E, kstride(h));
+  const ScratchLayout L = npa_scratch_layout(batch, T, mdim(P), P.E, kstride(h), h->P.K);
   float* ws = pc->ws;
   float *cur_s = ws + L.cur_s, *cur_u = ws + L.cur_u, *cur_d = ws + L.cur_d;
   float *mu = ws + L.mu, *lam = ws + L.lam, *pts = ws + L.pts, *dist = ws + L.dist;
@@ -509,7 +534,7 @@
                         cur_d, pc->out_s, pc->out_u, pc->out_d, pc->out_md, pc->out_iters, pc->out_np, flags,
                         pc->state, qp_info, h->qp_warm ? (double*)(ws + L.warm) : nullptr, pc->dune ? ws + L.trig : nullptr,
                         nullptr, nullptr, nullptr, stream,
-                        ev ? ev->a : nullptr, ev ? ev->b : nullptr, pc->theta));
+                        ev ? ev->a : nullptr, ev ? ev->b : nullptr, pc->theta, sched_ptrs(h, pc, L)));
   if (h->cal.key_auto && pc->dune && k == P.K - 1)
     HIP_TRY(hipMemcpyAsync(h->sel_stats_host, h->sel_stats_dev, sizeof(unsigned), hipMemcpyDeviceToHost, stream));
   return NPA_OK;
diff --git a/neupan_amd/csrc/create.hip b/neupan_amd/csrc/create.hip
--- a/neupan_amd/csrc/create.hip
+++ b/neupan_amd/csrc/create.hip
@@ -44,6 +44,7 @@
   CalibKnobs calib;
   std::string calib_key;
   bool sel_debug = false, qp_cold = false, qp_generic = false, skip_selftest = false, pack_cache = true;
+  bool qp_order = true;
   double audit_rate = 1.0 / 64.0;
   float margin_scale = 1.f;
 };
@@ -58,6 +59,7 @@
   k.sel_debug = getenv("NPA_SEL_DEBUG") != nullptr;
   k.qp_cold = getenv("NPA_QP_COLD") != nullptr;
   k.qp_generic = getenv("NPA_QP_GENERIC") != nullptr;
+  if (const char* env = getenv("NPA_QP_ORDER")) k.qp_order = atoi(env) != 0;
   k.skip_selftest = getenv("NPA_SKIP_SELFTEST") != nullptr;
   if (const char* env = getenv("NPA_PACK_CACHE")) k.pack_cache = atoi(env) != 0;
   if (const char* env = getenv("NPA_AUDIT_RATE")) { double v = atof(env); if (v >= 0.0 && v <= 1.0) k.audit_rate = v; }
@@ -406,6 +408,7 @@
   const Knobs knobs = read_knobs();
   h->knobs = knobs.calib;
   h->sel_debug = knobs.sel_debug; h->qp_warm = !knobs.qp_cold; h->qp_generic = knobs.qp_generic;
+  h->qp_order = knobs.qp_order;
 #ifdef NPA_EXPERIMENTS
   read_experiment_knobs(h);
 #endif
diff --git a/neupan_amd/csrc/handle.h b/neupan_amd/csrc/handle.h
--- a/neupan_amd/csrc/handle.h
+++ b/neupan_amd/csrc/handle.h
@@ -35,6 +35,7 @@
   bool dune = false;
   const float *nom_s = nullptr, *nom_u = nullptr;
   bool reset_state = false;
+  int qp_seq = 0;
   const float* theta = nullptr;
 };
 
@@ -111,6 +112,7 @@
   std::vector<EventPair> ev_dune, ev_sel, ev_qp;
   size_t n_dune = 0, n_sel = 0, n_qp = 0;
   bool qp_generic = false;
+  bool qp_order = true;
 };
 
 inline int mdim(const DevParams& P) { return P.M > 0 ? P.M : 1; }
diff --git a/neupan_amd/csrc/nrmp_qp.hip b/neupan_amd/csrc/nrmp_qp.hip
--- a/neupan_amd/csrc/nrmp_qp.hip
+++ b/neupan_amd/csrc/nrmp_qp.hip
@@ -32,7 +32,9 @@
                                     float* out_min_distance, int* out_iters, float* out_nrmp_points, int* flags,
                                     float* state, double* qp_info, double* warm, float* trig_out, float* dbg_abc,
                                     float* dbg_f, double* dbg_x,
-                                    hipStream_t stream, hipEvent_t ev_start, hipEvent_t ev_stop, const float* theta) {
+                                    hipStream_t stream, hipEvent_t ev_start, hipEvent_t ev_stop, const float* theta,
+                                    QpSched sched) {
+  if (scene0 != 0) sched = QpSched{nullptr, nullptr, nullptr, nullptr, nullptr};
   static const bool force_generic = getenv("NPA_QP_GENERIC") != nullptr;
   const bool fast = qp_fast_path(P.T, P.M) && !force_generic;
   const size_t shmem = npa_qp_shmem_bytes_path(P.T, P.M, fast ? 1 : 0);
@@ -50,7 +52,8 @@
                         P, cur_s_in, cur_u_in, ref_s, ref_us, mu_sorted, lam_sorted, pts_sorted, dist_sorted, count,  \
                         cur_s_out, cur_u_out, cur_d_out, out_s, out_u, out_d, out_min_distance, out_iters,            \
                         out_nrmp_points, flags, state, qp_info, warm, scene0, batch,                                 \
-                        QpBackward{nullptr, nullptr, nullptr, nullptr, nullptr, dbg_abc, dbg_f, dbg_x}, trig_out, theta)
+                        QpBackward{nullptr, nullptr, nullptr, nullptr, nullptr, dbg_abc, dbg_f, dbg_x}, trig_out, theta,   \
+                        sched)
   if (fast && P.T == 10) QP_LAUNCH(10, 10);
   else if (fast && P.T == 20) QP_LAUNCH(20, 10, false, true);
   else QP_LAUNCH(0, 0);
@@ -74,9 +77,9 @@
     attr_set.done(dev_);
   }
   if (P.T == 10)
-    hipExtLaunchKernelGGL((nrmp_qp_group_kernel<10, 10>), dim3(batch, n), dim3(QP_THREADS), shmem, stream, ev_start, ev_stop, 0, P, G, batch);
+    hipExtLaunchKernelGGL((nrmp_qp_group_kernel<10, 10>), dim3(batch, n), dim3(QP_THREADS), shmem, stream, ev_start, ev_stop, 0, P, G, batch, n);
   else
-    hipExtLaunchKernelGGL((nrmp_qp_group_kernel<20, 10, true>), dim3(batch, n), dim3(QP_THREADS), shmem, stream, ev_start, ev_stop, 0, P, G, batch);
+    hipExtLaunchKernelGGL((nrmp_qp_group_kernel<20, 10, true>), dim3(batch, n), dim3(QP_THREADS), shmem, stream, ev_start, ev_stop, 0, P, G, batch, n);
   return hipGetLastError();
 }
 
@@ -102,7 +105,8 @@
                      ref_us, mu_sorted, lam_sorted, pts_sorted, (const float*)nullptr, count, out_s, out_u, out_d,        \
                      (float*)nullptr, (float*)nullptr, (float*)nullptr, (float*)nullptr, (int*)nullptr, (float*)nullptr,  \
                      (int*)nullptr, (float*)nullptr, qp_info, (double*)nullptr, 0, batch,                                 \
-                     QpBackward{grad_s, grad_u, grad_d, grad_theta, grad_nom_s, nullptr, nullptr, nullptr}, (float*)nullptr, theta)
+                     QpBackward{grad_s, grad_u, grad_d, grad_theta, grad_nom_s, nullptr, nullptr, nullptr}, (float*)nullptr, theta, \
+                     QpSched{nullptr, nullptr, nullptr, nullptr, nullptr})
   if (fast && P.T == 10) QPB_LAUNCH(10, 10, true);
   else if (fast && P.T == 20) QPB_LAUNCH(20, 10, true, true);
   else QPB_LAUNCH(0, 0, true);
diff --git a/neupan_amd/csrc/nrmp_qp_body.inc b/neupan_amd/csrc/nrmp_qp_body.inc
--- a/neupan_amd/csrc/nrmp_qp_body.inc
+++ b/neupan_amd/csrc/nrmp_qp_body.inc
@@ -1,10 +1,9 @@
   double* sm = sm_all;
-  if (flags && flags[b * 4 + 0]) return;
+  if (flags && flags[b * 4 + 0]) {
+    if (lane == 0) QP_SCHED_FILE(0);
+    return;
+  }
   static_assert(!ASET_T, "the active-set launch is retired (DESIGN.md 3.3): ASET_T only keeps the kernels' names");
-  if (flags && flags[b * 4 + 3]) {
-    if (lane == 0) flags[b * 4 + 3] = 0;
-    return;
-  }
   __builtin_amdgcn_s_setprio(3);
 
   PROF_DECL
@@ -1185,14 +1184,12 @@
     double* qi = qp_info + (size_t)b * QP_INFO_STRIDE;
     qi[0] = best_it; qi[1] = best_merit; qi[2] = last_mu; qi[3] = status; qi[4] = it;
     qi[14] = it_total; qi[15] = warm_code;
-#ifndef NPA_QP_PROF
-    if (P.qp_aset && !(can_warm)) { qi[5] = 0; qi[6] = 0; qi[7] = 0; qi[8] = 0; }
-#endif
 #ifdef NPA_QP_PROF
     PROF(9);
     for (int i = 0; i < 10; ++i) qi[5 + i] = (double)pacc_[i];
 #endif
   }
+  if (lane == 0) QP_SCHED_FILE(it_total);
 
   const int cnt0 = (obs && count) ? count[(size_t)b * (T + 1)] : 0;
   if (out_min_distance && lane == 0) {
diff --git a/neupan_amd/csrc/nrmp_qp_device.h b/neupan_amd/csrc/nrmp_qp_device.h
--- a/neupan_amd/csrc/nrmp_qp_device.h
+++ b/neupan_amd/csrc/nrmp_qp_device.h
@@ -249,6 +249,32 @@
     __builtin_amdgcn_wave_barrier();                         \
   } while (0)
 
+__device__ __forceinline__ int qp_sched_pick(const int* __restrict__ cnt, const int* __restrict__ list, int rank, int nscene, int lane) {
+  if (!cnt) return rank;
+  const int c0 = cnt[lane & (NPA_SCHED_NCLS - 1)];
+  const int c = lane < NPA_SCHED_NCLS ? c0 : 0;
+  int s = c;
+  s += __builtin_amdgcn_update_dpp(0, s, 0x111, 0xF, 0xF, true);
+  s += __builtin_amdgcn_update_dpp(0, s, 0x112, 0xF, 0xF, true);
+  s += __builtin_amdgcn_update_dpp(0, s, 0x114, 0xF, 0xF, true);
+  s += __builtin_amdgcn_update_dpp(0, s, 0x118, 0xF, 0xF, true);
+  s += __builtin_amdgcn_update_dpp(0, s, 0x142, 0xA, 0xF, false);
+  if (__builtin_amdgcn_readlane(s, NPA_SCHED_NCLS - 1) != nscene) return rank;
+  const unsigned long long over = __builtin_amdgcn_ballot_w64(lane < NPA_SCHED_NCLS && s > rank);
+  const int cls = __builtin_amdgcn_readfirstlane((int)__builtin_ctzll(over | (1ull << (NPA_SCHED_NCLS - 1))));
+  int off = rank - __builtin_amdgcn_readlane(s - c, cls);
+  off = off < 0 ? 0 : (off >= nscene ? nscene - 1 : off);
+  const int b = __builtin_amdgcn_readfirstlane(list[(size_t)cls * nscene + off]);
+  return b < 0 ? 0 : (b >= nscene ? nscene - 1 : b);
+}
+__device__ __forceinline__ void qp_sched_file(int* cnt, int* list, int* ticket, int it_total, int b, int L, int nscene) {
+  if (!cnt) return;
+  const int cls = NPA_SCHED_NCLS - 1 - (it_total < 0 ? 0 : (it_total > NPA_SCHED_NCLS - 1 ? NPA_SCHED_NCLS - 1 : it_total));
+  const int pos = __hip_atomic_fetch_add(&cnt[cls], 1, __ATOMIC_RELAXED, __HIP_MEMORY_SCOPE_AGENT);
+  if ((unsigned)pos < (unsigned)nscene) list[(size_t)cls * nscene + pos] = b;
+  ticket[b] = L;
+}
+
 struct QpBackward {
   const float* grad_s;
   const float* grad_u;
@@ -288,24 +314,33 @@
     float* __restrict__ out_u, float* __restrict__ out_d, float* __restrict__ out_min_distance,
     int* __restrict__ out_iters, float* __restrict__ out_nrmp_points, int* __restrict__ flags,
     float* __restrict__ state, double* __restrict__ qp_info, double* __restrict__ warm, int scene0, int nscene,
-    QpBackward bw, float* __restrict__ trig_out, const float* __restrict__ theta) {
+    QpBackward bw, float* __restrict__ trig_out, const float* __restrict__ theta,
+    QpSched sched) {
   extern __shared__ __attribute__((aligned(16))) double sm_all[];
   const int lane = threadIdx.x;
   if ((int)blockIdx.x >= nscene) return;
-  const int b = blockIdx.x + scene0;
+  int b_ = blockIdx.x;
+  if constexpr (!BWD) b_ = qp_sched_pick(sched.in_cnt, sched.in_list, blockIdx.x, nscene, lane);
+  const int b = b_ + scene0;
+#define QP_SCHED_FILE(IT) do { if constexpr (!BWD) qp_sched_file(sched.out_cnt, sched.out_list, sched.ticket, (IT), b, (int)blockIdx.x, nscene); } while (0)
 #include "nrmp_qp_body.inc"
+#undef QP_SCHED_FILE
 }
 
 template <int TT, int MM, bool SCANW = false>
 __global__ __attribute__((amdgpu_flat_work_group_size(QP_THREADS, QP_THREADS), amdgpu_waves_per_eu(NPA_QP_WAVES, 3)))
-void nrmp_qp_group_kernel(DevParams P, QpGroup G, int nscene) {
+void nrmp_qp_group_kernel(DevParams P, QpGroup G, int nscene, int n) {
   extern __shared__ __attribute__((aligned(16))) double sm_all[];
   constexpr bool BWD = false, ASET_T = false;
   constexpr int WV = NPA_QP_WAVES;
   const int lane = threadIdx.x;
   if ((int)blockIdx.x >= nscene) return;
-  const int b = blockIdx.x;
-  const QpCall& q = G.c[blockIdx.y];
+  const unsigned sched_L = blockIdx.y * (unsigned)nscene + blockIdx.x, sched_rank = sched_L / (unsigned)n;
+  const int sched_call = __builtin_amdgcn_readfirstlane((int)(sched_L - sched_rank * (unsigned)n));
+  const QpCall& q = G.c[sched_call];
+  const int b = qp_sched_pick(q.sched.in_cnt, q.sched.in_list, (int)sched_rank, nscene, lane);
+#define QP_SCHED_FILE(IT) do { const QpSched& so_ = G.c[sched_call].sched; \
+    qp_sched_file(so_.out_cnt, so_.out_list, so_.ticket, (IT), b, (int)(blockIdx.y * (unsigned)nscene + blockIdx.x), nscene); } while (0)
   const float* cur_s_in = q.cur_s_in; const float* cur_u_in = q.cur_u_in;
   const float* __restrict__ ref_s = q.ref_s; const float* __restrict__ ref_us = q.ref_us;
   const float* __restrict__ mu_sorted = q.mu_sorted; const float* __restrict__ lam_sorted = q.lam_sorted;
@@ -319,4 +354,5 @@
   const float* __restrict__ theta = q.theta;
   const QpBackward bw{nullptr, nullptr, nullptr, nullptr, nullptr, nullptr, nullptr, nullptr};
 #include "nrmp_qp_body.inc"
-}
+#undef QP_SCHED_FILE
+}
diff --git a/neupan_amd/csrc/pan_common.h b/neupan_amd/csrc/pan_common.h
--- a/neupan_amd/csrc/pan_common.h
+++ b/neupan_amd/csrc/pan_common.h
@@ -46,16 +46,19 @@
   unsigned* audit; int n_stride; unsigned audit_seed;
 };
 struct SelGeoGroup { SelGeoCall c[NPA_GROUP_MAX]; };
+struct QpSched { const int* in_cnt; const int* in_list; int* out_cnt; int* out_list; int* ticket; };
 struct QpCall {
   const float* cur_s_in; const float* cur_u_in; const float* ref_s; const float* ref_us; const float* mu_sorted;
   const float* lam_sorted; const float* pts_sorted; const float* dist_sorted; const int* count; float* cur_s_out;
   float* cur_u_out; float* cur_d_out; float* out_s; float* out_u; float* out_d; float* out_min_distance; int* out_iters;
   float* out_nrmp_points; int* flags; float* state; double* qp_info; double* warm; float* trig_out;
   const float* theta;
+  QpSched sched;
 };
 struct QpGroup { QpCall c[NPA_GROUP_MAX]; };
 struct StageCall {
   float* cur_s; const float* nom_s; float* cur_u; const float* nom_u; int* flags; int* count; int* state; float* trig;
+  int* sched_cnt;
 };
 struct StageGroup { StageCall c[NPA_GROUP_MAX]; };
 
@@ -112,13 +115,18 @@
   s = (float)sin((double)th);
 }
 
+#define NPA_SCHED_NCLS 32
 struct ScratchLayout {
-  size_t cur_s, cur_u, cur_d, mu, lam, pts, dist, count, flags, warm, qp_info, trig, keys, total;
+  size_t cur_s, cur_u, cur_d, mu, lam, pts, dist, count, flags, warm, qp_info, trig, keys, sched, total;
 };
+__host__ __device__ inline size_t npa_sched_cnt_ints(int K) { return (size_t)(K > 0 ? K : 1) * NPA_SCHED_NCLS; }
+__host__ __device__ inline size_t npa_sched_ints(int B, int K) {
+  return npa_sched_cnt_ints(K) + (size_t)2 * NPA_SCHED_NCLS * B + (size_t)B;
+}
 __host__ __device__ inline size_t npa_warm_doubles(int T, int M) {
   return (size_t)2 * T + T + (size_t)T * M + (8 * T - 4) + 2 * T;
 }
-__host__ __device__ inline ScratchLayout npa_scratch_layout(int B, int T, int M, int E, int key_stride) {
+__host__ __device__ inline ScratchLayout npa_scratch_layout(int B, int T, int M, int E, int key_stride, int K) {
   ScratchLayout L;
   size_t o = 0;
   auto take = [&](size_t n) { size_t r = o; o += (n + 3) & ~(size_t)3; return r; };
@@ -136,6 +144,7 @@
   L.qp_info = take((size_t)B * 16 * 2);
   L.trig = take((size_t)B * (T + 1) * 2);
   L.keys = take((size_t)B * (T + 1) * key_stride);
+  L.sched = take(npa_sched_ints(B, K));
   L.total = o;
   return L;
 }
```
